# YiZhangCUG/liblcg

Hardware: AMD Instinct MI355X
Metric: cg_iterations_per_sec (higher is better)
Workload: dtype f64

## Files before the change

### include/lcg_hip.h

```cpp
#ifndef LCG_HIP_H
#define LCG_HIP_H

#include <stdint.h>

#ifdef __cplusplus
extern "C" {
#endif


typedef struct lcg_para {
    int    max_iterations;
    double epsilon;
    int    abs_diff;
    double restart_epsilon;
    double step;
    double sigma;
    double beta;
    int    maxi_m;
} lcg_para;

typedef struct clcg_para {
    int    max_iterations;
    double epsilon;
    int    abs_diff;
} clcg_para;

typedef enum lcg_solver_enum { LCG_CG = 0, LCG_PCG = 1, LCG_CGS = 2, LCG_BICGSTAB = 3, LCG_BICGSTAB2 = 4, LCG_PG = 5, LCG_SPG = 6 } lcg_solver_enum;
typedef enum clcg_solver_enum { CLCG_BICG = 0, CLCG_BICG_SYM = 1, CLCG_CGS = 2, CLCG_BICGSTAB = 3, CLCG_TFQMR = 4,
                                CLCG_PCG = 5, CLCG_PBICG = 6 } clcg_solver_enum;
enum {
    LCG_SUCCESS = 0, LCG_CONVERGENCE = 0, LCG_STOP = 1, LCG_ALREADY_OPTIMIZIED = 2,
    LCG_UNKNOWN_ERROR = -1024, LCG_INVILAD_VARIABLE_SIZE = -1023, LCG_INVILAD_MAX_ITERATIONS = -1022,
    LCG_INVILAD_EPSILON = -1021, LCG_INVILAD_RESTART_EPSILON = -1020,
    LCG_REACHED_MAX_ITERATIONS = -1019, LCG_NULL_PRECONDITION_MATRIX = -1018, LCG_NAN_VALUE = -1017,
    LCG_INVALID_POINTER = -1016, LCG_INVALID_LAMBDA = -1015, LCG_INVALID_SIGMA = -1014,
    LCG_INVALID_BETA = -1013, LCG_INVALID_MAXIM = -1012, LCG_SIZE_NOT_MATCH = -1011
};
enum {
    CLCG_SUCCESS = 0, CLCG_CONVERGENCE = 0, CLCG_STOP = 1, CLCG_ALREADY_OPTIMIZIED = 2,
    CLCG_UNKNOWN_ERROR = -1024, CLCG_INVILAD_VARIABLE_SIZE = -1023, CLCG_INVILAD_MAX_ITERATIONS = -1022,
    CLCG_INVILAD_EPSILON = -1021, CLCG_REACHED_MAX_ITERATIONS = -1020, CLCG_NAN_VALUE = -1019,
    CLCG_INVALID_POINTER = -1018, CLCG_SIZE_NOT_MATCH = -1017, CLCG_UNKNOWN_SOLVER = -1016
};
enum {
    LCG_HIP_E_RUNTIME = -2000,
    LCG_HIP_E_NO_DEVICE = -2001,
    LCG_HIP_E_COMM = -2002,
    LCG_HIP_E_ARG = -2003
};
enum { LCG_HIP_MEM_HOST = 0, LCG_HIP_MEM_DEVICE = 1 };

typedef void (*lcg_axfunc_ptr)(void *instance, const double *x, double *prod_Ax, const int n_size);
typedef int (*lcg_progress_ptr)(void *instance, const double *m, const double converge,
                                const lcg_para *param, const int n_size, const int k);
typedef void (*clcg_hip_axfunc_ptr)(void *instance, const double *x, double *prod_Ax,
                                    const int n_size, int layout, int conjugate);
typedef int (*clcg_hip_progress_ptr)(void *instance, const double *m, const double converge,
                                     const clcg_para *param, const int n_size, const int k);

typedef void (*clcg_hip_axfunc_c64_ptr)(void *instance, const float *x, float *prod_Ax, const int n_size,
                                        int layout, int conjugate);
typedef int (*clcg_hip_progress_c64_ptr)(void *instance, const float *m, const float converge,
                                         const clcg_para *param, const int n_size, const int k);

int  lcg_hip_init(int device);
int  lcg_hip_set_stream(void *hip_stream);
void *lcg_hip_get_stream(void);
int  lcg_hip_synchronize(void);
int  lcg_hip_memcpy(void *dst, const void *src, uint64_t bytes, int kind);
const char *lcg_hip_last_error(void);
lcg_para  lcg_hip_default_parameters(void);
clcg_para clcg_hip_default_parameters(void);
int    lcg_hip_last_iterations(void);
double lcg_hip_last_residual(void);
int    lcg_hip_set_profiling(int on);
double lcg_hip_last_ax_mean_us(void);
int    lcg_hip_last_ax_calls(void);
int    lcg_hip_last_launches(int *vector_passes, int *scalar_steps, int *rank_reductions, int *products);
int    lcg_hip_last_finisher_steps(void);
int    lcg_hip_trim(void);
enum { LCG_HIP_CG_AUTO = 0, LCG_HIP_CG_CLASSIC = 1, LCG_HIP_CG_ONE_REDUCTION = 2 };
int    lcg_hip_set_cg_schedule(int schedule);
int    lcg_hip_set_placement(int mode);
int    lcg_hip_last_placement(int *timed, int *moved, double *us_as_allocated, double *us_as_placed);
int    lcg_hip_pool_info(int *vectors, int64_t *bytes, int *arena_slots);
int    lcg_hip_pool_add_arena_for_test(uint64_t slot_bytes, int slots);
int    lcg_hip_placement_tune_for_test(uint64_t stream_min_bytes, uint64_t chunk_bytes, int max_chunks, double wall_ms, uint64_t hold_max_bytes,
                                       int force_find_at, int allow_shared);
int    lcg_hip_last_placement_walk(int *chunks, double *wall_ms, int64_t *held_bytes, int *found, const char **ended);

int lcg_hip_solver(lcg_axfunc_ptr Afp, lcg_progress_ptr Pfp, double *m, const double *B,
                   int n_size, const lcg_para *param, void *instance, int solver_id, int mem);
int lcg_hip_solver_preconditioned(lcg_axfunc_ptr Afp, lcg_axfunc_ptr Mfp, lcg_progress_ptr Pfp,
                                  double *m, const double *B, int n_size, const lcg_para *param,
                                  void *instance, int solver_id, int mem);
int lcg_hip_solver_constrained(lcg_axfunc_ptr Afp, lcg_progress_ptr Pfp, double *m, const double *B,
                               const double *low, const double *hig, int n_size, const lcg_para *param,
                               void *instance, int solver_id, int mem);
int lcg_hip_lcg(lcg_axfunc_ptr Afp, lcg_progress_ptr Pfp, double *m, const double *B, int n_size,
                const lcg_para *param, void *instance, double *Gk, double *Dk, double *ADk, int mem);
int lcg_hip_lcgs(lcg_axfunc_ptr Afp, lcg_progress_ptr Pfp, double *m, const double *B, int n_size,
                 const lcg_para *param, void *instance, double *RK, double *R0T, double *PK,
                 double *AX, double *UK, double *QK, double *WK, int mem);
int clcg_hip_solver(clcg_hip_axfunc_ptr Afp, clcg_hip_progress_ptr Pfp, double *m, const double *B,
                    int n_size, const clcg_para *param, void *instance, int solver_id, int mem);
int clcg_hip_solver_preconditioned(clcg_hip_axfunc_ptr Afp, clcg_hip_axfunc_ptr Mfp, clcg_hip_progress_ptr Pfp,
                                   double *m, const double *B, int n_size, const clcg_para *param,
                                   void *instance, int solver_id, int mem);
int clcg_hip_solver_c64(clcg_hip_axfunc_c64_ptr Afp, clcg_hip_progress_c64_ptr Pfp, float *m, const float *B,
                        int n_size, const clcg_para *param, void *instance, int solver_id, int mem);
int clcg_hip_solver_preconditioned_c64(clcg_hip_axfunc_c64_ptr Afp, clcg_hip_axfunc_c64_ptr Mfp, clcg_hip_progress_c64_ptr Pfp,
                                       float *m, const float *B, int n_size, const clcg_para *param, void *instance,
                                       int solver_id, int mem);
int lcg_hip_set_shadow_seed(unsigned seed);
int lcg_hip_set_shadow_vector(const double *rbar0_host, int n_size);

typedef struct lcg_hip_csr *lcg_hip_csr_t;

int lcg_hip_csr_create(lcg_hip_csr_t *A, int n_rows, int n_cols, int64_t nnz, const int *rowptr,
                       const int *col, const double *val, int is_complex, int mem, int adopt);
int lcg_hip_csr_create_c64(lcg_hip_csr_t *A, int n_rows, int n_cols, int64_t nnz, const int *rowptr,
                           const int *col, const float *val, int mem, int adopt);
int lcg_hip_csr_from_coo(lcg_hip_csr_t *A, int n, int64_t nnz, const int *row, const int *col,
                         const double *val, int is_complex, int mem);
int lcg_hip_csr_destroy(lcg_hip_csr_t A);
int lcg_hip_csr_rows(lcg_hip_csr_t A);
int64_t lcg_hip_csr_nnz(lcg_hip_csr_t A);
int lcg_hip_csr_arrays(lcg_hip_csr_t A, const int **rowptr, const int **col, const double **val);
int lcg_hip_csr_set_kernel(lcg_hip_csr_t A, int variant);
int lcg_hip_csr_set_packed(lcg_hip_csr_t A, int mode);
int64_t lcg_hip_csr_packed_runs(lcg_hip_csr_t A, int64_t *blocks_out);
int lcg_hip_csr_set_run_stretches(lcg_hip_csr_t A, int mode);
int64_t lcg_hip_csr_run_stretches(lcg_hip_csr_t A, int64_t *blocks_out);
int64_t lcg_hip_csr_packed_templates(lcg_hip_csr_t A);
int lcg_hip_csr_set_binned(lcg_hip_csr_t A, int mode);
int lcg_hip_csr_set_tiled(lcg_hip_csr_t A, int mode);
const char *lcg_hip_csr_tiled_status(lcg_hip_csr_t A);
int lcg_hip_csr_set_ranges(lcg_hip_csr_t A, int mode);
int lcg_hip_csr_ranges(lcg_hip_csr_t A, int cap, int *first_row);
const char *lcg_hip_csr_binned_status(lcg_hip_csr_t A);
const char *lcg_hip_csr_last_kernel(lcg_hip_csr_t A);
int64_t lcg_hip_csr_last_traffic_model(lcg_hip_csr_t A);
int lcg_hip_csr_plan_info(lcg_hip_csr_t A, double *build_ms, int64_t *extra_bytes);
int lcg_hip_csr_build_jacobi(lcg_hip_csr_t A, double *diag_out);

void lcg_hip_csr_ax(void *instance, const double *x, double *prod_Ax, const int n_size);
void lcg_hip_jacobi_mx(void *instance, const double *x, double *prod_Mx, const int n_size);
void clcg_hip_csr_ax(void *instance, const double *x, double *prod_Ax, const int n_size,
                     int layout, int conjugate);
void clcg_hip_jacobi_mx(void *instance, const double *x, double *prod_Mx, const int n_size,
                        int layout, int conjugate);
void clcg_hip_csr_ax_c64(void *instance, const float *x, float *prod_Ax, const int n_size,
                         int layout, int conjugate);
void clcg_hip_jacobi_mx_c64(void *instance, const float *x, float *prod_Mx, const int n_size,
                            int layout, int conjugate);

int  lcg_hip_csr_build_ic0(lcg_hip_csr_t A);
int  lcg_hip_csr_build_ic0_c64(lcg_hip_csr_t A);
int  lcg_hip_csr_ic0_info(lcg_hip_csr_t A, int *levels_lower, int *levels_upper, int *launches_per_apply,
                          int *zero_pivot, double *build_ms, int64_t *bytes);
int  lcg_hip_csr_ic0_set_sweeps(lcg_hip_csr_t A, int sweeps);
int  lcg_hip_csr_ic0_get_sweeps(lcg_hip_csr_t A, int *sweeps);
int  lcg_hip_csr_ic0_factor(lcg_hip_csr_t A, const int **rowptr, const int **col, const double **val);
int  lcg_hip_ic0_solve(lcg_hip_csr_t A, int which, const double *x, double *y);
int  lcg_hip_ic0_solve_c64(lcg_hip_csr_t A, int which, const float *x, float *y);
void lcg_hip_ic0_mx(void *instance, const double *x, double *prod_Mx, const int n_size);
void clcg_hip_ic0_mx(void *instance, const double *x, double *prod_Mx, const int n_size,
                     int layout, int conjugate);
void clcg_hip_ic0_mx_c64(void *instance, const float *x, float *prod_Mx, const int n_size,
                         int layout, int conjugate);
int  lcg_hip_csr_ic0_schedule_for_test(lcg_hip_csr_t A, int max_merged_rows);

int  lcg_hip_csr_build_ilu0(lcg_hip_csr_t A);
int  lcg_hip_csr_ilu0_info(lcg_hip_csr_t A, int *levels_L, int *levels_U, int *launches_per_apply, int *zero_pivot,
                           double *build_ms, int64_t *bytes);
int  lcg_hip_csr_ilu0_set_sweeps(lcg_hip_csr_t A, int sweeps);
int  lcg_hip_csr_ilu0_get_sweeps(lcg_hip_csr_t A, int *sweeps);
int  lcg_hip_csr_ilu0_factor(lcg_hip_csr_t A, int which, const int **rowptr, const int **col, const double **val);
int  lcg_hip_ilu0_solve(lcg_hip_csr_t A, int which, const double *x, double *y);
void lcg_hip_ilu0_mx(void *instance, const double *x, double *prod_Mx, const int n_size);
void clcg_hip_ilu0_mx(void *instance, const double *x, double *prod_Mx, const int n_size,
                      int layout, int conjugate);
void lcg_hip_csr_ax_ilu0(void *instance, const double *x, double *prod_Ax, const int n_size);
void clcg_hip_csr_ax_ilu0(void *instance, const double *x, double *prod_Ax, const int n_size,
                          int layout, int conjugate);
int  lcg_hip_csr_ilu0_schedule_for_test(lcg_hip_csr_t A, int max_merged_rows);

typedef struct lcg_hip_dense *lcg_hip_dense_t;

int lcg_hip_dense_create(lcg_hip_dense_t *K, int m_rows, int n_cols, const double *val, int64_t ld, int is_complex, int mem);
int lcg_hip_dense_create_rows(lcg_hip_dense_t *K, int m_rows, int n_cols, const double *const *rows, int is_complex);
int lcg_hip_dense_destroy(lcg_hip_dense_t K);
int lcg_hip_dense_rows(lcg_hip_dense_t K);
int lcg_hip_dense_cols(lcg_hip_dense_t K);
int lcg_hip_dense_matvec(lcg_hip_dense_t K, const double *x, double *y, int layout);
int clcg_hip_dense_matvec(lcg_hip_dense_t K, const double *x, double *y, int layout, int conjugate);
int lcg_hip_dense_ata(lcg_hip_dense_t K, const double *x, double *y);
void lcg_hip_dense_ata_ax(void *instance, const double *x, double *prod_Ax, const int n_size);
void lcg_hip_dense_ax(void *instance, const double *x, double *prod_Ax, const int n_size);
void clcg_hip_dense_ax(void *instance, const double *x, double *prod_Ax, const int n_size,
                       int layout, int conjugate);
int lcg_hip_dense_build_jacobi(lcg_hip_dense_t K, int normal, double *diag_out);
void lcg_hip_dense_jacobi_mx(void *instance, const double *x, double *prod_Mx, const int n_size);
void clcg_hip_dense_jacobi_mx(void *instance, const double *x, double *prod_Mx, const int n_size,
                              int layout, int conjugate);
const char *lcg_hip_dense_last_kernel(lcg_hip_dense_t K);
const char *lcg_hip_dense_kernel_name(int index);
int lcg_hip_dense_set_kernel(lcg_hip_dense_t K, int variant);
int lcg_hip_dense_matmat(lcg_hip_dense_t K, int k, const double *X, double *Y, int layout);
int lcg_hip_dense_ata_multi(lcg_hip_dense_t K, int k, const double *X, double *Y);
int lcg_hip_dense_op_multi_dot(lcg_hip_dense_t K, int k, int normal, const double *X, double *Y, const double *U, double *dots);
const char *lcg_hip_dense_multi_last_kernel(lcg_hip_dense_t K);
const char *lcg_hip_dense_multi_kernel_name(int index);
int lcg_hip_dense_lcg_multi (lcg_hip_dense_t K, int k, int normal, double *M, const double *B, const lcg_para *param,
                             int *ret, int *iterations, double *residual, int mem);
int lcg_hip_dense_lpcg_multi(lcg_hip_dense_t K, int k, int normal, double *M, const double *B, const lcg_para *param,
                             int *ret, int *iterations, double *residual, int mem);
int clcg_hip_dense_matmat(lcg_hip_dense_t K, int k, const double *X, double *Y, int layout, int conjugate);
int clcg_hip_dense_op_multi_dot(lcg_hip_dense_t K, int k, const double *X, double *Y, const double *U, double *dots);
const char *clcg_hip_dense_multi_kernel_name(int index);
int clcg_hip_dense_lbicg_sym_multi(lcg_hip_dense_t K, int k, double *M, const double *B, const clcg_para *param,
                                   int *ret, int *iterations, double *residual, int mem);
int clcg_hip_dense_lpcg_multi(lcg_hip_dense_t K, int k, double *M, const double *B, const clcg_para *param,
                              int *ret, int *iterations, double *residual, int mem);

int lcg_hip_spmv(lcg_hip_csr_t A, const double *x, double *y);
int lcg_hip_spmv_op(lcg_hip_csr_t A, const double *x, double *y, int layout, int conjugate);
int lcg_hip_spmv_dot(lcg_hip_csr_t A, const double *x, double *y, const double *u, double *result2);
int lcg_hip_spmm(lcg_hip_csr_t A, int k, const double *X, double *Y);
int lcg_hip_spmm_dot(lcg_hip_csr_t A, int k, const double *X, double *Y, const double *U, double *dots);
int lcg_hip_spmm_dot2(lcg_hip_csr_t A, int k, const double *X, double *Y, const double *U, double *dots2);
int lcg_hip_lcg_multi(lcg_hip_csr_t A, int k, double *M, const double *B, const lcg_para *param,
                      int *ret, int *iterations, double *residual, int mem);
int lcg_hip_lpcg_multi(lcg_hip_csr_t A, int k, double *M, const double *B, const lcg_para *param,
                       int *ret, int *iterations, double *residual, int mem);
int lcg_hip_ic0_solve_multi (lcg_hip_csr_t A, int k, int which, const double *X, double *Y);
int lcg_hip_ilu0_solve_multi(lcg_hip_csr_t A, int k, int which, const double *X, double *Y);
enum { LCG_HIP_M_JACOBI = 0, LCG_HIP_M_IC0 = 1, LCG_HIP_M_ILU0 = 2 };
int lcg_hip_lpcg_multi_m(lcg_hip_csr_t A, int k, int precond, double *M, const double *B, const lcg_para *param,
                         int *ret, int *iterations, double *residual, int mem);
enum { LCG_HIP_M_NONE = -1 };
int lcg_hip_lbicgstab_multi(lcg_hip_csr_t A, int k, int precond, double *M, const double *B, const lcg_para *param,
                            int *ret, int *iterations, double *residual, int mem);
int clcg_hip_spmm(lcg_hip_csr_t A, int k, const double *X, double *Y);
int clcg_hip_spmm_dot(lcg_hip_csr_t A, int k, const double *X, double *Y, const double *U, double *dots);
int clcg_hip_lbicg_sym_multi(lcg_hip_csr_t A, int k, double *M, const double *B, const clcg_para *param,
                             int *ret, int *iterations, double *residual, int mem);
int clcg_hip_lpcg_multi(lcg_hip_csr_t A, int k, double *M, const double *B, const clcg_para *param,
                        int *ret, int *iterations, double *residual, int mem);
int lcg_hip_spmv_c64(lcg_hip_csr_t A, const float *x, float *y, int layout, int conjugate);
int lcg_hip_dot(int n, const double *a, const double *b, double *result);
int lcg_hip_nrm2(int n, const double *a, double *result);
int lcg_hip_axpy(int n, double alpha, const double *x, double *y);
int lcg_hip_scal(int n, double alpha, double *x);
int lcg_hip_set2box(int n, const double *low, const double *hig, double *a);
int lcg_hip_vecmul(int n, const double *a, const double *b, double *c);
int lcg_hip_vecdiv(int n, const double *a, const double *b, double *c);
int clcg_hip_dot(int n, const double *a, const double *b, double *result2);
int clcg_hip_inner(int n, const double *a, const double *b, double *result2);
int clcg_hip_axpy(int n, const double *alpha2, const double *x, double *y);
int clcg_hip_vecdiv(int n, const double *a, const double *b, double *c);

int lcg_hip_csr_generate(lcg_hip_csr_t *A, int64_t n, int npairs, int64_t band, int symmetric,
                         uint64_t seed, double diag_shift, int64_t r0, int64_t r1);
enum { LCG_HIP_GEN_SCRAMBLED = 0, LCG_HIP_GEN_DIAGONALS = 1, LCG_HIP_GEN_ROW_RANDOM_BAND = 2 };
int lcg_hip_csr_generate_ex(lcg_hip_csr_t *A, int64_t n, int npairs, int pattern, int64_t band, int symmetric,
                            uint64_t seed, double diag_shift, int64_t r0, int64_t r1);
int lcg_hip_gen_xtrue(int64_t n, uint64_t seed, int64_t r0, int64_t r1, double *x_dev);
int lcg_hip_csr_laplace2d(lcg_hip_csr_t *A, int nx, int ny, int64_t r0, int64_t r1);

int lcg_hip_comm_unique_id(void *id128);
int lcg_hip_comm_init(int nranks, int rank, const void *id128);
int lcg_hip_comm_destroy(void);
int lcg_hip_comm_rank(void);
int lcg_hip_comm_size(void);
const char *lcg_hip_comm_library(void);
int lcg_hip_csr_distribute(lcg_hip_csr_t A, int64_t n_global, int mode);
int64_t lcg_hip_csr_exchange_volume(lcg_hip_csr_t A);
int lcg_hip_allreduce_sum(double *dev_values, int count);
int lcg_hip_barrier(void);
#define LCG_HIP_P2P_HANDLE_BYTES 64
int lcg_hip_p2p_export(void *handle64);
int lcg_hip_p2p_connect(int nranks, int rank, const void *handles);
int lcg_hip_p2p_selftest(int rounds);
int lcg_hip_p2p_enable(int on);
int lcg_hip_p2p_status(void);
// ... 14 lines not shown
```

### liblcg_amd/_lib.py

```python
from __future__ import annotations

import ctypes as C
import os
import subprocess

HERE = os.path.dirname(os.path.abspath(__file__))
SO_PATH = os.path.join(HERE, "lib", "liblcg_hip.so")
CSRC = os.path.join(HERE, "csrc")

c_int_p = C.POINTER(C.c_int)
c_double_p = C.POINTER(C.c_double)
vp = C.c_void_p


class LcgPara(C.Structure):
    _fields_ = [("max_iterations", C.c_int), ("epsilon", C.c_double), ("abs_diff", C.c_int),
                ("restart_epsilon", C.c_double), ("step", C.c_double), ("sigma", C.c_double),
                ("beta", C.c_double), ("maxi_m", C.c_int)]


class ClcgPara(C.Structure):
    _fields_ = [("max_iterations", C.c_int), ("epsilon", C.c_double), ("abs_diff", C.c_int)]


AXFUNC = C.CFUNCTYPE(None, vp, vp, vp, C.c_int)
PROGRESS = C.CFUNCTYPE(C.c_int, vp, vp, C.c_double, C.POINTER(LcgPara), C.c_int, C.c_int)
CAXFUNC = C.CFUNCTYPE(None, vp, vp, vp, C.c_int, C.c_int, C.c_int)
CPROGRESS = C.CFUNCTYPE(C.c_int, vp, vp, C.c_double, C.POINTER(ClcgPara), C.c_int, C.c_int)
CPROGRESS_C64 = C.CFUNCTYPE(C.c_int, vp, vp, C.c_float, C.POINTER(ClcgPara), C.c_int, C.c_int)

SIGNATURES = {
    "lcg_hip_init": (C.c_int, [C.c_int]),
    "lcg_hip_set_stream": (C.c_int, [vp]),
    "lcg_hip_get_stream": (vp, []),
    "lcg_hip_synchronize": (C.c_int, []),
    "lcg_hip_memcpy": (C.c_int, [vp, vp, C.c_uint64, C.c_int]),
    "lcg_hip_last_error": (C.c_char_p, []),
    "lcg_hip_default_parameters": (LcgPara, []),
    "clcg_hip_default_parameters": (ClcgPara, []),
    "lcg_hip_last_iterations": (C.c_int, []),
    "lcg_hip_last_residual": (C.c_double, []),
    "lcg_hip_set_profiling": (C.c_int, [C.c_int]),
    "lcg_hip_set_cg_schedule": (C.c_int, [C.c_int]),
    "lcg_hip_set_placement": (C.c_int, [C.c_int]),
    "lcg_hip_last_placement": (C.c_int, [C.POINTER(C.c_int), C.POINTER(C.c_int), C.POINTER(C.c_double), C.POINTER(C.c_double)]),
    "lcg_hip_pool_info": (C.c_int, [C.POINTER(C.c_int), C.POINTER(C.c_int64), C.POINTER(C.c_int)]),
    "lcg_hip_pool_add_arena_for_test": (C.c_int, [C.c_uint64, C.c_int]),
    "lcg_hip_placement_tune_for_test": (C.c_int, [C.c_uint64, C.c_uint64, C.c_int, C.c_double, C.c_uint64, C.c_int, C.c_int]),
    "lcg_hip_last_placement_walk": (C.c_int, [C.POINTER(C.c_int), C.POINTER(C.c_double), C.POINTER(C.c_int64), C.POINTER(C.c_int), C.POINTER(C.c_char_p)]),
    "lcg_hip_last_ax_mean_us": (C.c_double, []),
    "lcg_hip_last_ax_calls": (C.c_int, []),
    "lcg_hip_last_launches": (C.c_int, [c_int_p, c_int_p, c_int_p, c_int_p]),
    "lcg_hip_last_finisher_steps": (C.c_int, []),
    "lcg_hip_trim": (C.c_int, []),
    "lcg_hip_solver": (C.c_int, [vp, vp, vp, vp, C.c_int, C.POINTER(LcgPara), vp, C.c_int, C.c_int]),
    "lcg_hip_solver_preconditioned": (C.c_int, [vp, vp, vp, vp, vp, C.c_int, C.POINTER(LcgPara), vp, C.c_int, C.c_int]),
    "lcg_hip_solver_constrained": (C.c_int, [vp, vp, vp, vp, vp, vp, C.c_int, C.POINTER(LcgPara), vp, C.c_int, C.c_int]),
    "lcg_hip_set2box": (C.c_int, [C.c_int, vp, vp, vp]),
    "lcg_hip_lcg": (C.c_int, [vp, vp, vp, vp, C.c_int, C.POINTER(LcgPara), vp, vp, vp, vp, C.c_int]),
    "lcg_hip_lcgs": (C.c_int, [vp, vp, vp, vp, C.c_int, C.POINTER(LcgPara), vp, vp, vp, vp, vp, vp, vp, vp, C.c_int]),
    "clcg_hip_solver": (C.c_int, [vp, vp, vp, vp, C.c_int, C.POINTER(ClcgPara), vp, C.c_int, C.c_int]),
    "clcg_hip_solver_preconditioned": (C.c_int, [vp, vp, vp, vp, vp, C.c_int, C.POINTER(ClcgPara), vp, C.c_int, C.c_int]),
    "clcg_hip_jacobi_mx": (None, [vp, vp, vp, C.c_int, C.c_int, C.c_int]),
    "clcg_hip_solver_c64": (C.c_int, [vp, vp, vp, vp, C.c_int, C.POINTER(ClcgPara), vp, C.c_int, C.c_int]),
    "clcg_hip_solver_preconditioned_c64": (C.c_int, [vp, vp, vp, vp, vp, C.c_int, C.POINTER(ClcgPara), vp, C.c_int, C.c_int]),
    "lcg_hip_csr_create_c64": (C.c_int, [C.POINTER(vp), C.c_int, C.c_int, C.c_int64, vp, vp, vp, C.c_int, C.c_int]),
    "lcg_hip_spmv_c64": (C.c_int, [vp, vp, vp, C.c_int, C.c_int]),
    "clcg_hip_csr_ax_c64": (None, [vp, vp, vp, C.c_int, C.c_int, C.c_int]),
    "clcg_hip_jacobi_mx_c64": (None, [vp, vp, vp, C.c_int, C.c_int, C.c_int]),
    "lcg_hip_set_shadow_seed": (C.c_int, [C.c_uint]),
    "lcg_hip_set_shadow_vector": (C.c_int, [vp, C.c_int]),
    "lcg_hip_csr_create": (C.c_int, [C.POINTER(vp), C.c_int, C.c_int, C.c_int64, vp, vp, vp, C.c_int, C.c_int, C.c_int]),
    "lcg_hip_csr_from_coo": (C.c_int, [C.POINTER(vp), C.c_int, C.c_int64, vp, vp, vp, C.c_int, C.c_int]),
    "lcg_hip_csr_destroy": (C.c_int, [vp]),
    "lcg_hip_csr_rows": (C.c_int, [vp]),
    "lcg_hip_csr_nnz": (C.c_int64, [vp]),
    "lcg_hip_csr_arrays": (C.c_int, [vp, C.POINTER(vp), C.POINTER(vp), C.POINTER(vp)]),
    "lcg_hip_csr_set_kernel": (C.c_int, [vp, C.c_int]),
    "lcg_hip_csr_set_packed": (C.c_int, [vp, C.c_int]),
    "lcg_hip_csr_packed_runs": (C.c_int64, [vp, C.POINTER(C.c_int64)]),
    "lcg_hip_csr_set_run_stretches": (C.c_int, [vp, C.c_int]),
    "lcg_hip_csr_run_stretches": (C.c_int64, [vp, C.POINTER(C.c_int64)]),
    "lcg_hip_csr_packed_templates": (C.c_int64, [vp]),
    "lcg_hip_csr_set_binned": (C.c_int, [vp, C.c_int]),
    "lcg_hip_csr_set_tiled": (C.c_int, [vp, C.c_int]),
    "lcg_hip_csr_set_ranges": (C.c_int, [vp, C.c_int]),
    "lcg_hip_csr_ranges": (C.c_int, [vp, C.c_int, C.POINTER(C.c_int)]),
    "lcg_hip_csr_tiled_status": (C.c_char_p, [vp]),
    "lcg_hip_csr_binned_status": (C.c_char_p, [vp]),
    "lcg_hip_csr_last_kernel": (C.c_char_p, [vp]),
    "lcg_hip_csr_last_traffic_model": (C.c_int64, [vp]),
    "lcg_hip_csr_plan_info": (C.c_int, [vp, C.POINTER(C.c_double), C.POINTER(C.c_int64)]),
    "lcg_hip_csr_build_jacobi": (C.c_int, [vp, vp]),
    "lcg_hip_csr_build_ic0": (C.c_int, [vp]),
    "lcg_hip_csr_ic0_info": (C.c_int, [vp, c_int_p, c_int_p, c_int_p, c_int_p, c_double_p, C.POINTER(C.c_int64)]),
    "lcg_hip_csr_ic0_factor": (C.c_int, [vp, C.POINTER(vp), C.POINTER(vp), C.POINTER(vp)]),
    "lcg_hip_ic0_solve": (C.c_int, [vp, C.c_int, vp, vp]),
    "lcg_hip_ic0_mx": (None, [vp, vp, vp, C.c_int]),
    "clcg_hip_ic0_mx": (None, [vp, vp, vp, C.c_int, C.c_int, C.c_int]),
    "lcg_hip_csr_ic0_schedule_for_test": (C.c_int, [vp, C.c_int]),
    "lcg_hip_csr_ic0_set_sweeps": (C.c_int, [vp, C.c_int]),
    "lcg_hip_csr_ic0_get_sweeps": (C.c_int, [vp, c_int_p]),
    "lcg_hip_csr_build_ic0_c64": (C.c_int, [vp]),
    "lcg_hip_ic0_solve_c64": (C.c_int, [vp, C.c_int, vp, vp]),
    "clcg_hip_ic0_mx_c64": (None, [vp, vp, vp, C.c_int, C.c_int, C.c_int]),
    "lcg_hip_csr_build_ilu0": (C.c_int, [vp]),
    "lcg_hip_csr_ilu0_info": (C.c_int, [vp, c_int_p, c_int_p, c_int_p, c_int_p, c_double_p, C.POINTER(C.c_int64)]),
    "lcg_hip_csr_ilu0_set_sweeps": (C.c_int, [vp, C.c_int]),
    "lcg_hip_csr_ilu0_get_sweeps": (C.c_int, [vp, c_int_p]),
    "lcg_hip_csr_ilu0_factor": (C.c_int, [vp, C.c_int, C.POINTER(vp), C.POINTER(vp), C.POINTER(vp)]),
    "lcg_hip_ilu0_solve": (C.c_int, [vp, C.c_int, vp, vp]),
    "lcg_hip_ilu0_mx": (None, [vp, vp, vp, C.c_int]),
    "clcg_hip_ilu0_mx": (None, [vp, vp, vp, C.c_int, C.c_int, C.c_int]),
    "lcg_hip_csr_ax_ilu0": (None, [vp, vp, vp, C.c_int]),
    "clcg_hip_csr_ax_ilu0": (None, [vp, vp, vp, C.c_int, C.c_int, C.c_int]),
    "lcg_hip_csr_ilu0_schedule_for_test": (C.c_int, [vp, C.c_int]),
    "lcg_hip_dense_create": (C.c_int, [C.POINTER(vp), C.c_int, C.c_int, vp, C.c_int64, C.c_int, C.c_int]),
    "lcg_hip_dense_create_rows": (C.c_int, [C.POINTER(vp), C.c_int, C.c_int, vp, C.c_int]),
    "lcg_hip_dense_destroy": (C.c_int, [vp]),
    "lcg_hip_dense_rows": (C.c_int, [vp]),
    "lcg_hip_dense_cols": (C.c_int, [vp]),
    "lcg_hip_dense_matvec": (C.c_int, [vp, vp, vp, C.c_int]),
    "clcg_hip_dense_matvec": (C.c_int, [vp, vp, vp, C.c_int, C.c_int]),
    "lcg_hip_dense_ata": (C.c_int, [vp, vp, vp]),
    "lcg_hip_dense_ata_ax": (None, [vp, vp, vp, C.c_int]),
    "lcg_hip_dense_ax": (None, [vp, vp, vp, C.c_int]),
    "clcg_hip_dense_ax": (None, [vp, vp, vp, C.c_int, C.c_int, C.c_int]),
    "lcg_hip_dense_build_jacobi": (C.c_int, [vp, C.c_int, vp]),
    "lcg_hip_dense_jacobi_mx": (None, [vp, vp, vp, C.c_int]),
    "clcg_hip_dense_jacobi_mx": (None, [vp, vp, vp, C.c_int, C.c_int, C.c_int]),
    "lcg_hip_dense_last_kernel": (C.c_char_p, [vp]),
    "lcg_hip_dense_kernel_name": (C.c_char_p, [C.c_int]),
    "lcg_hip_dense_set_kernel": (C.c_int, [vp, C.c_int]),
    "lcg_hip_dense_matmat": (C.c_int, [vp, C.c_int, vp, vp, C.c_int]),
    "lcg_hip_dense_ata_multi": (C.c_int, [vp, C.c_int, vp, vp]),
    "lcg_hip_dense_op_multi_dot": (C.c_int, [vp, C.c_int, C.c_int, vp, vp, vp, c_double_p]),
    "lcg_hip_dense_multi_last_kernel": (C.c_char_p, [vp]),
    "lcg_hip_dense_multi_kernel_name": (C.c_char_p, [C.c_int]),
    "lcg_hip_dense_lcg_multi": (C.c_int, [vp, C.c_int, C.c_int, vp, vp, C.POINTER(LcgPara), c_int_p, c_int_p, c_double_p, C.c_int]),
    "lcg_hip_dense_lpcg_multi": (C.c_int, [vp, C.c_int, C.c_int, vp, vp, C.POINTER(LcgPara), c_int_p, c_int_p, c_double_p, C.c_int]),
    "clcg_hip_dense_matmat": (C.c_int, [vp, C.c_int, vp, vp, C.c_int, C.c_int]),
    "clcg_hip_dense_op_multi_dot": (C.c_int, [vp, C.c_int, vp, vp, vp, c_double_p]),
    "clcg_hip_dense_multi_kernel_name": (C.c_char_p, [C.c_int]),
    "clcg_hip_dense_lbicg_sym_multi": (C.c_int, [vp, C.c_int, vp, vp, C.POINTER(ClcgPara), c_int_p, c_int_p, c_double_p, C.c_int]),
    "clcg_hip_dense_lpcg_multi": (C.c_int, [vp, C.c_int, vp, vp, C.POINTER(ClcgPara), c_int_p, c_int_p, c_double_p, C.c_int]),
    "lcg_hip_csr_ax": (None, [vp, vp, vp, C.c_int]),
    "lcg_hip_jacobi_mx": (None, [vp, vp, vp, C.c_int]),
    "clcg_hip_csr_ax": (None, [vp, vp, vp, C.c_int, C.c_int, C.c_int]),
    "lcg_hip_spmv": (C.c_int, [vp, vp, vp]),
    "lcg_hip_spmv_op": (C.c_int, [vp, vp, vp, C.c_int, C.c_int]),
    "lcg_hip_spmv_dot": (C.c_int, [vp, vp, vp, vp, c_double_p]),
    "lcg_hip_spmm": (C.c_int, [vp, C.c_int, vp, vp]),
    "lcg_hip_spmm_dot": (C.c_int, [vp, C.c_int, vp, vp, vp, c_double_p]),
    "lcg_hip_spmm_dot2": (C.c_int, [vp, C.c_int, vp, vp, vp, c_double_p]),
    "lcg_hip_lcg_multi": (C.c_int, [vp, C.c_int, vp, vp, C.POINTER(LcgPara), c_int_p, c_int_p, c_double_p, C.c_int]),
    "lcg_hip_lpcg_multi": (C.c_int, [vp, C.c_int, vp, vp, C.POINTER(LcgPara), c_int_p, c_int_p, c_double_p, C.c_int]),
    "lcg_hip_lpcg_multi_m": (C.c_int, [vp, C.c_int, C.c_int, vp, vp, C.POINTER(LcgPara), c_int_p, c_int_p, c_double_p, C.c_int]),
    "lcg_hip_lbicgstab_multi": (C.c_int, [vp, C.c_int, C.c_int, vp, vp, C.POINTER(LcgPara), c_int_p, c_int_p, c_double_p, C.c_int]),
    "clcg_hip_spmm": (C.c_int, [vp, C.c_int, vp, vp]),
    "clcg_hip_spmm_dot": (C.c_int, [vp, C.c_int, vp, vp, vp, c_double_p]),
    "clcg_hip_lbicg_sym_multi": (C.c_int, [vp, C.c_int, vp, vp, C.POINTER(ClcgPara), c_int_p, c_int_p, c_double_p, C.c_int]),
    "clcg_hip_lpcg_multi": (C.c_int, [vp, C.c_int, vp, vp, C.POINTER(ClcgPara), c_int_p, c_int_p, c_double_p, C.c_int]),
    "lcg_hip_ic0_solve_multi": (C.c_int, [vp, C.c_int, C.c_int, vp, vp]),
    "lcg_hip_ilu0_solve_multi": (C.c_int, [vp, C.c_int, C.c_int, vp, vp]),
    "lcg_hip_dot": (C.c_int, [C.c_int, vp, vp, c_double_p]),
    "lcg_hip_nrm2": (C.c_int, [C.c_int, vp, c_double_p]),
    "lcg_hip_axpy": (C.c_int, [C.c_int, C.c_double, vp, vp]),
    "lcg_hip_scal": (C.c_int, [C.c_int, C.c_double, vp]),
    "lcg_hip_vecmul": (C.c_int, [C.c_int, vp, vp, vp]),
    "lcg_hip_vecdiv": (C.c_int, [C.c_int, vp, vp, vp]),
    "clcg_hip_dot": (C.c_int, [C.c_int, vp, vp, c_double_p]),
    "clcg_hip_inner": (C.c_int, [C.c_int, vp, vp, c_double_p]),
    "clcg_hip_axpy": (C.c_int, [C.c_int, c_double_p, vp, vp]),
    "clcg_hip_vecdiv": (C.c_int, [C.c_int, vp, vp, vp]),
    "lcg_hip_csr_generate": (C.c_int, [C.POINTER(vp), C.c_int64, C.c_int, C.c_int64, C.c_int, C.c_uint64, C.c_double, C.c_int64, C.c_int64]),
    "lcg_hip_csr_generate_ex": (C.c_int, [C.POINTER(vp), C.c_int64, C.c_int, C.c_int, C.c_int64, C.c_int, C.c_uint64, C.c_double, C.c_int64, C.c_int64]),
    "lcg_hip_gen_xtrue": (C.c_int, [C.c_int64, C.c_uint64, C.c_int64, C.c_int64, vp]),
    "lcg_hip_csr_laplace2d": (C.c_int, [C.POINTER(vp), C.c_int, C.c_int, C.c_int64, C.c_int64]),
    "lcg_hip_comm_unique_id": (C.c_int, [vp]),
    "lcg_hip_comm_init": (C.c_int, [C.c_int, C.c_int, vp]),
    "lcg_hip_comm_destroy": (C.c_int, []),
    "lcg_hip_comm_rank": (C.c_int, []),
    "lcg_hip_comm_size": (C.c_int, []),
    "lcg_hip_comm_library": (C.c_char_p, []),
    "lcg_hip_csr_distribute": (C.c_int, [vp, C.c_int64, C.c_int]),
    "lcg_hip_allreduce_sum": (C.c_int, [vp, C.c_int]),
    "lcg_hip_barrier": (C.c_int, []),
    "lcg_hip_csr_direct_selfloop_for_test": (C.c_int, [vp, C.c_int, C.c_int]),
    "lcg_hip_p2p_export": (C.c_int, [vp]),
    "lcg_hip_p2p_connect": (C.c_int, [C.c_int, C.c_int, vp]),
    "lcg_hip_p2p_selftest": (C.c_int, [C.c_int]),
    "lcg_hip_p2p_enable": (C.c_int, [C.c_int]),
    "lcg_hip_p2p_status": (C.c_int, []),
    "lcg_hip_p2p_set_timeout_ms": (C.c_int, [C.c_int]),
    "lcg_hip_p2p_disconnect": (C.c_int, []),
    "lcg_hip_csr_split_for_test": (C.c_int, [vp, C.c_int64, C.c_int, C.c_int]),
    "lcg_hip_csr_xfull": (vp, [vp]),
    "lcg_hip_csr_ax_part_for_probe": (C.c_int, [vp, vp, vp, C.c_int]),
    "lcg_hip_csr_local_nnz": (C.c_int64, [vp]),
    "lcg_hip_csr_exchange_volume": (C.c_int64, [vp]),
    "lcg_hip_csr_need_ranges_for_test": (C.c_int, [vp, C.c_int, vp]),
}

_lib = None


def build(verbose: bool = False) -> str:
    cmd = ["make", "-C", CSRC, "-j", str(min(8, os.cpu_count() or 1))]
    if not verbose:
        cmd.insert(1, "-s")
    subprocess.check_call(cmd)
    return SO_PATH


def load():
    global _lib
    if _lib is not None:
        return _lib
    if not os.path.exists(SO_PATH):
        try:
            build()
        except Exception as exc:
            raise ImportError(f"{SO_PATH} is not built and could not be built here ({exc}): run "
                              "`python -c 'import __graft_entry__ as g; g.build()'` (there is no CPU fallback)")
    import torch
    lib = C.CDLL(SO_PATH, mode=C.RTLD_GLOBAL)
    for name, (res, args) in SIGNATURES.items():
        fn = getattr(lib, name)
        fn.restype = res
        fn.argtypes = args
    _lib = lib
    return lib


def fnptr(lib, name: str) -> vp:
# ... 2 lines not shown
```

### liblcg_amd/api.py

```python
from __future__ import annotations

import ctypes as C
from dataclasses import dataclass

import numpy as np

from . import _lib as L
from ._lib import CAXFUNC, CPROGRESS, CPROGRESS_C64, AXFUNC, PROGRESS, ClcgPara, LcgPara

LCG_CG, LCG_PCG, LCG_CGS, LCG_BICGSTAB, LCG_BICGSTAB2, LCG_PG, LCG_SPG = range(7)
CLCG_BICG, CLCG_BICG_SYM, CLCG_CGS, CLCG_BICGSTAB, CLCG_TFQMR, CLCG_PCG, CLCG_PBICG = range(7)
MEM_HOST, MEM_DEVICE = 0, 1
GEN_SCRAMBLED, GEN_DIAGONALS, GEN_ROW_RANDOM_BAND = 0, 1, 2


class LcgHipError(RuntimeError):
    pass


def _chk(rc: int, what: str):
    if rc <= -2000:
        raise LcgHipError(f"{what}: rc={rc}: {L.load().lcg_hip_last_error().decode()}")
    return rc


def lcg_default_parameters(**kw) -> LcgPara:
    p = L.load().lcg_hip_default_parameters()
    for k, v in kw.items():
        setattr(p, k, v)
    return p


def clcg_default_parameters(**kw) -> ClcgPara:
    p = L.load().clcg_hip_default_parameters()
    for k, v in kw.items():
        setattr(p, k, v)
    return p


def _ptr(x):
    if isinstance(x, np.ndarray):
        return x.ctypes.data, MEM_HOST
    import torch
    if isinstance(x, torch.Tensor):
        if not x.is_contiguous():
            raise ValueError("tensor must be contiguous")
        return x.data_ptr(), (MEM_DEVICE if x.is_cuda else MEM_HOST)
    raise TypeError(type(x))


def use_torch_stream():
    import torch
    _chk(L.load().lcg_hip_set_stream(C.c_void_p(torch.cuda.current_stream().cuda_stream)), "set_stream")


def use_own_stream():
    _chk(L.load().lcg_hip_set_stream(None), "set_stream")


class CsrMatrix:
    is_c64 = False

    def __init__(self, handle: int, n_rows: int, is_complex: bool, keep=()):
        self.h = C.c_void_p(handle)
        self.n = n_rows
        self.is_complex = is_complex
        self._keep = keep

    @classmethod
    def from_csr(cls, rowptr, col, val, n_cols=None, adopt=False):
        lib = L.load()
        is_c = bool(np.iscomplexobj(val)) if isinstance(val, np.ndarray) else val.is_complex()
        if isinstance(val, np.ndarray):
            rowptr = np.ascontiguousarray(rowptr, np.int32); col = np.ascontiguousarray(col, np.int32)
            val = np.ascontiguousarray(val, np.complex128 if is_c else np.float64)
        n = len(rowptr) - 1
        nnz = len(col)
        (pr, mem), (pc, _), (pv, _) = _ptr(rowptr), _ptr(col), _ptr(val)
        h = C.c_void_p()
        _chk(lib.lcg_hip_csr_create(C.byref(h), n, n_cols or n, nnz, pr, pc, pv, int(is_c), mem, int(adopt)), "csr_create")
        return cls(h.value, n, is_c, keep=(rowptr, col, val) if adopt else ())

    @classmethod
    def from_csr_c64(cls, rowptr, col, val, n_cols=None, adopt=False):
        lib = L.load()
        if isinstance(val, np.ndarray):
            rowptr = np.ascontiguousarray(rowptr, np.int32); col = np.ascontiguousarray(col, np.int32)
            val = np.ascontiguousarray(val, np.complex64)
        else:
            import torch
            if val.dtype != torch.complex64:
                raise TypeError(f"from_csr_c64 takes complex64 values, not {val.dtype}")
        n = len(rowptr) - 1
        (pr, mem), (pc, _), (pv, _) = _ptr(rowptr), _ptr(col), _ptr(val)
        h = C.c_void_p()
        _chk(lib.lcg_hip_csr_create_c64(C.byref(h), n, n_cols or n, len(col), pr, pc, pv, mem, int(adopt)), "csr_create_c64")
        M = cls(h.value, n, True, keep=(rowptr, col, val) if adopt else ())
        M.is_c64 = True
        return M

    def spmv_c64(self, x, y, layout=0, conjugate=0):
        return _chk(L.load().lcg_hip_spmv_c64(self.h, _ptr(x)[0], _ptr(y)[0], layout, conjugate), "spmv_c64")

    @classmethod
    def from_coo(cls, n, row, col, val):
        lib = L.load()
        is_c = bool(np.iscomplexobj(val))
        row = np.ascontiguousarray(row, np.int32); col = np.ascontiguousarray(col, np.int32)
        val = np.ascontiguousarray(val, np.complex128 if is_c else np.float64)
        h = C.c_void_p()
        _chk(lib.lcg_hip_csr_from_coo(C.byref(h), n, len(row), row.ctypes.data, col.ctypes.data, val.ctypes.data,
                                      int(is_c), MEM_HOST), "csr_from_coo")
        return cls(h.value, n, is_c)

    @classmethod
    def generate(cls, n, npairs=16, band=0, symmetric=True, seed=1, diag_shift=0.01, r0=0, r1=None, pattern=None):
        lib = L.load()
        r1 = n if r1 is None else r1
        if pattern is None:
            pattern = GEN_DIAGONALS if band > 0 else GEN_SCRAMBLED
        h = C.c_void_p()
        _chk(lib.lcg_hip_csr_generate_ex(C.byref(h), n, npairs, pattern, band, int(symmetric), seed, diag_shift, r0, r1), "csr_generate")
        return cls(h.value, r1 - r0, False)

    @classmethod
    def laplace2d(cls, nx, ny, r0=0, r1=None):
        lib = L.load()
        r1 = nx * ny if r1 is None else r1
        h = C.c_void_p()
        _chk(lib.lcg_hip_csr_laplace2d(C.byref(h), nx, ny, r0, r1), "csr_laplace2d")
        return cls(h.value, r1 - r0, False)

    @property
    def nnz(self) -> int:
        return L.load().lcg_hip_csr_nnz(self.h)

    def arrays_to_host(self):
        lib = L.load()
        pr, pc, pv = C.c_void_p(), C.c_void_p(), C.c_void_p()
        _chk(lib.lcg_hip_csr_arrays(self.h, C.byref(pr), C.byref(pc), C.byref(pv)), "csr_arrays")
        nnz = self.nnz
        rowptr = np.empty(self.n + 1, np.int32); col = np.empty(nnz, np.int32)
        val = np.empty(nnz, np.complex128 if self.is_complex else np.float64)
        for dst, src in ((rowptr, pr), (col, pc), (val, pv)):
            _chk(lib.lcg_hip_memcpy(dst.ctypes.data, src, dst.nbytes, 2), "memcpy d2h")
        return rowptr, col, val

    def set_kernel(self, variant: int):
        _chk(L.load().lcg_hip_csr_set_kernel(self.h, variant), "set_kernel")

    def build_jacobi(self, diag_out=None):
        p = None if diag_out is None else _ptr(diag_out)[0]
        _chk(L.load().lcg_hip_csr_build_jacobi(self.h, p), "build_jacobi")

    def build_ic0(self):
        if self.is_c64:
            _chk(L.load().lcg_hip_csr_build_ic0_c64(self.h), "build_ic0_c64")
        else:
            _chk(L.load().lcg_hip_csr_build_ic0(self.h), "build_ic0")

    def ic0_info(self) -> dict:
        ll, lu, la, zp = C.c_int(), C.c_int(), C.c_int(), C.c_int()
        ms, nb = C.c_double(), C.c_int64()
        _chk(L.load().lcg_hip_csr_ic0_info(self.h, C.byref(ll), C.byref(lu), C.byref(la), C.byref(zp), C.byref(ms), C.byref(nb)),
             "ic0_info")
        sw = C.c_int(0)
        if L.load().lcg_hip_csr_ic0_get_sweeps(self.h, C.byref(sw)) != 0:
            sw.value = 0
        return {"levels_lower": ll.value, "levels_upper": lu.value, "launches_per_apply": la.value,
                "zero_pivot": zp.value, "build_ms": ms.value, "bytes": nb.value, "sweeps": sw.value}

    def ic0_set_sweeps(self, k):
        _chk(L.load().lcg_hip_csr_ic0_set_sweeps(self.h, int(k)), "ic0_set_sweeps")

    def ic0_factor_to_host(self):
        lib = L.load()
        pr, pc, pv = C.c_void_p(), C.c_void_p(), C.c_void_p()
        _chk(lib.lcg_hip_csr_ic0_factor(self.h, C.byref(pr), C.byref(pc), C.byref(pv)), "ic0_factor")
        rowptr = np.empty(self.n + 1, np.int32)
        _chk(lib.lcg_hip_memcpy(rowptr.ctypes.data, pr, rowptr.nbytes, 2), "memcpy d2h")
        nnz = int(rowptr[-1])
        col = np.empty(nnz, np.int32)
        val = np.empty(nnz, np.complex64 if self.is_c64 else np.complex128 if self.is_complex else np.float64)
        for dst, src in ((col, pc), (val, pv)):
            _chk(lib.lcg_hip_memcpy(dst.ctypes.data, src, dst.nbytes, 2), "memcpy d2h")
        return rowptr, col, val

    def ic0_solve(self, x, y, which=2):
        if self.is_c64:
            _chk(L.load().lcg_hip_ic0_solve_c64(self.h, which, _ptr(x)[0], _ptr(y)[0]), "ic0_solve_c64")
        else:
            _chk(L.load().lcg_hip_ic0_solve(self.h, which, _ptr(x)[0], _ptr(y)[0]), "ic0_solve")

    def ic0_solve_multi(self, X, Y, which=2):
        k = _block_k(X, Y)
        _chk(L.load().lcg_hip_ic0_solve_multi(self.h, k, which, _ptr(X)[0], _ptr(Y)[0]), "ic0_solve_multi")

    def build_ilu0(self):
        _chk(L.load().lcg_hip_csr_build_ilu0(self.h), "build_ilu0")

    def ilu0_info(self) -> dict:
        ll, lu, la, zp = C.c_int(), C.c_int(), C.c_int(), C.c_int()
        ms, nb = C.c_double(), C.c_int64()
        _chk(L.load().lcg_hip_csr_ilu0_info(self.h, C.byref(ll), C.byref(lu), C.byref(la), C.byref(zp), C.byref(ms), C.byref(nb)),
             "ilu0_info")
        sw = C.c_int(0)
        if L.load().lcg_hip_csr_ilu0_get_sweeps(self.h, C.byref(sw)) != 0:
            sw.value = 0
        return {"levels_L": ll.value, "levels_U": lu.value, "launches_per_apply": la.value,
                "zero_pivot": zp.value, "build_ms": ms.value, "bytes": nb.value, "sweeps": sw.value}

    def ilu0_set_sweeps(self, k):
        _chk(L.load().lcg_hip_csr_ilu0_set_sweeps(self.h, int(k)), "ilu0_set_sweeps")

    def ilu0_factor_to_host(self, which):
        lib = L.load()
        pr, pc, pv = C.c_void_p(), C.c_void_p(), C.c_void_p()
        _chk(lib.lcg_hip_csr_ilu0_factor(self.h, int(which), C.byref(pr), C.byref(pc), C.byref(pv)), "ilu0_factor")
        rowptr = np.empty(self.n + 1, np.int32)
        _chk(lib.lcg_hip_memcpy(rowptr.ctypes.data, pr, rowptr.nbytes, 2), "memcpy d2h")
        nnz = int(rowptr[-1])
        col = np.empty(nnz, np.int32)
        val = np.empty(nnz, np.complex128 if self.is_complex else np.float64)
        for dst, src in ((col, pc), (val, pv)):
            if nnz:
                _chk(lib.lcg_hip_memcpy(dst.ctypes.data, src, dst.nbytes, 2), "memcpy d2h")
        return rowptr, col, val

    def ilu0_solve(self, x, y, which=2):
        _chk(L.load().lcg_hip_ilu0_solve(self.h, which, _ptr(x)[0], _ptr(y)[0]), "ilu0_solve")

    def ilu0_solve_multi(self, X, Y, which=2):
        k = _block_k(X, Y)
        _chk(L.load().lcg_hip_ilu0_solve_multi(self.h, k, which, _ptr(X)[0], _ptr(Y)[0]), "ilu0_solve_multi")

    def spmv(self, x, y):
        _chk(L.load().lcg_hip_spmv(self.h, _ptr(x)[0], _ptr(y)[0]), "spmv")

    def spmm(self, X, Y):
        k = _block_k(X, Y)
        _chk(L.load().lcg_hip_spmm(self.h, k, _ptr(X)[0], _ptr(Y)[0]), "spmm")

    def spmm_dot2(self, X, Y, U):
        k = _block_k(X, Y, U)
        out = (C.c_double * (2 * k))()
        _chk(L.load().lcg_hip_spmm_dot2(self.h, k, _ptr(X)[0], _ptr(Y)[0], _ptr(U)[0], out), "spmm_dot2")
        return np.array(out[:], dtype=np.float64)

    def cspmm(self, X, Y):
        k = _block_k(X, Y, cplx=True)
        _chk(L.load().clcg_hip_spmm(self.h, k, _ptr(X)[0], _ptr(Y)[0]), "cspmm")

    def cspmm_dot(self, X, Y, U):
        k = _block_k(X, Y, U, cplx=True)
        out = (C.c_double * (2 * k))()
        _chk(L.load().clcg_hip_spmm_dot(self.h, k, _ptr(X)[0], _ptr(Y)[0], _ptr(U)[0], out), "cspmm_dot")
        return np.array(out[:], dtype=np.float64).view(np.complex128)

    def distribute(self, n_global: int, mode: int = 0):
        _chk(L.load().lcg_hip_csr_distribute(self.h, n_global, mode), "csr_distribute")

    def destroy(self):
        if self.h:
            L.load().lcg_hip_csr_destroy(self.h)
            self.h = C.c_void_p()

    def __del__(self):
        try:
            self.destroy()
        except Exception:
            pass


class DenseMatrix:
    KERNEL_AUTO, KERNEL_ROW, KERNEL_ROW_SPLIT, KERNEL_COL, KERNEL_ATA_TWO_PASS, KERNEL_ATA_ONE_PASS, KERNEL_ATA_SMALL = range(7)

    def __init__(self, handle: int, m: int, n: int, is_complex: bool):
        self.h = C.c_void_p(handle)
        self.m, self.n, self.is_complex = m, n, is_complex

    @classmethod
    def from_array(cls, K):
        lib = L.load()
        if isinstance(K, np.ndarray):
            is_c = bool(np.iscomplexobj(K))
            if (K.ndim != 2 or K.strides[1] != K.itemsize or K.dtype not in (np.float64, np.complex128) or K.strides[0] % K.itemsize
                    or (K.shape[0] > 1 and K.strides[0] < K.shape[1] * K.itemsize)):
                K = np.ascontiguousarray(K, np.complex128 if is_c else np.float64)
            ld, ptr, mem = K.strides[0] // K.itemsize, K.ctypes.data, MEM_HOST
        else:
            is_c = K.is_complex()
            if K.dim() != 2 or K.stride(1) != 1:
                raise ValueError("a 2-d tensor with unit stride along its rows is needed")
            ld, ptr, mem = K.stride(0), K.data_ptr(), (MEM_DEVICE if K.is_cuda else MEM_HOST)
        m, n = K.shape
        if ld < n:
            if m != 1:
                raise ValueError(f"rows {ld} entries apart hold {n} entries: make the array contiguous first")
            ld = n
        h = C.c_void_p()
        _chk(lib.lcg_hip_dense_create(C.byref(h), m, n, ptr, ld, int(is_c), mem), "dense_create")
        return cls(h.value, m, n, is_c)
# ... 346 lines not shown
```

### liblcg_amd/csrc/comm.hip

```cpp
#include <dlfcn.h>

#include <rccl/rccl.h>

#include <cstdlib>
#include <cstring>
#include <vector>

#include "devcommon.hpp"

namespace lcgh {


struct Comm {
    void *lib = nullptr;
    ncclComm_t comm = nullptr;
    int nranks = 1, rank = 0;
    ncclResult_t (*GetUniqueId)(ncclUniqueId *) = nullptr;
    ncclResult_t (*CommInitRank)(ncclComm_t *, int, ncclUniqueId, int) = nullptr;
    ncclResult_t (*CommDestroy)(ncclComm_t) = nullptr;
    ncclResult_t (*AllReduce)(const void *, void *, size_t, ncclDataType_t, ncclRedOp_t, ncclComm_t, hipStream_t) = nullptr;
    ncclResult_t (*AllGather)(const void *, void *, size_t, ncclDataType_t, ncclComm_t, hipStream_t) = nullptr;
    ncclResult_t (*ReduceScatter)(const void *, void *, size_t, ncclDataType_t, ncclRedOp_t, ncclComm_t, hipStream_t) = nullptr;
    ncclResult_t (*Send)(const void *, size_t, ncclDataType_t, int, ncclComm_t, hipStream_t) = nullptr;
    ncclResult_t (*Recv)(void *, size_t, ncclDataType_t, int, ncclComm_t, hipStream_t) = nullptr;
// ... 483 lines not shown
        cp.dst[cp.nseg] = A->xfull + w * (size_t)D->need_lo[s];
        cp.first_block[cp.nseg] = nb;
        nb += (int)((cnt + PUSH_CHUNK - 1) / PUSH_CHUNK);
        cp.nseg++;
    }
    cp.first_block[cp.nseg] = nb;
    cp.nblocks = nb > 0 ? nb : 1;
}

static int direct_setup(lcg_hip_csr *A)
{
    Ctx &c = ctx();
    XgBox xb;
    if (!xg_box(&xb)) { c.err = "direct exchange needs the mailboxes (lcg_hip_p2p_connect + enable)"; return LCG_HIP_E_COMM; }
    const int P = xb.P, me = xb.me;
    const size_t w = A->is_complex ? 2 : 1;
    Direct *D = new Direct();
    A->direct = D;
    auto give_up = [&](int rc, const char *why) { if (why) c.err = why; direct_free(A); return rc; };

    std::vector<long long> need;
    int rc = need_ranges(A, P, need);
    bool all = false;
    int rc2 = xg_agree(rc == 0, &all);
    if (rc2) return give_up(rc2, nullptr);
    if (!all) return give_up(rc ? rc : LCG_HIP_E_COMM, rc ? nullptr : "direct exchange: a peer could not scan its columns");
    std::vector<unsigned long long> table;
    rc = xg_allgather_words(reinterpret_cast<const unsigned long long *>(need.data()), 2 * P, table);
    if (rc) return give_up(rc, nullptr);
    auto T = [&](int q, int p, int k) { return (long long)table[(size_t)q * 2 * P + 2 * p + k]; };
    for (int q = 0; q < P; q++) {
        if (q == me) continue;
        const bool take = need[2 * q + 1] > need[2 * q];
        const bool give = T(q, me, 1) > T(q, me, 0);
        if (!take && !give) continue;
        if (D->nnb < XG_MAXSEG) {
            const int s = D->nnb;
            D->nb_rank[s] = q;
            D->give_lo[s] = give ? T(q, me, 0) : 0; D->give_hi[s] = give ? T(q, me, 1) : 0;
            D->need_lo[s] = take ? need[2 * q] : 0; D->need_hi[s] = take ? need[2 * q + 1] : 0;
            if (take) D->recv_total += need[2 * q + 1] - need[2 * q];
        }
        D->nnb++;
    }
    const bool fits = D->nnb <= XG_MAXSEG;
    rc = xg_agree(fits, &all);
    if (rc) return give_up(rc, nullptr);
    if (!all) return give_up(LCG_HIP_E_COMM, "direct exchange: a rank has more than 8 neighbours (use mode 1 or 0)");
    D->half = (size_t)A->rows_per_rank * P * w;
    hipError_t e;
    {
        void *p = nullptr;
        e = hipExtMallocWithFlags(&p, sizeof(double) * 2 * D->half, hipDeviceMallocUncached);
        if (e != hipSuccess) { (void)hipGetLastError(); e = hipExtMallocWithFlags(&p, sizeof(double) * 2 * D->half, hipDeviceMallocFinegrained); }
        D->recv = static_cast<double *>(p);
    }
    if (e == hipSuccess) e = hipMemsetAsync(D->recv, 0, sizeof(double) * 2 * D->half, c.stream);
    if (e == hipSuccess) {
        void *p = nullptr;
        e = hipExtMallocWithFlags(&p, sizeof(unsigned long long) * XG_MAXP, hipDeviceMallocUncached);
        if (e != hipSuccess) { (void)hipGetLastError(); e = hipExtMallocWithFlags(&p, sizeof(unsigned long long) * XG_MAXP, hipDeviceMallocFinegrained); }
        D->flags = static_cast<unsigned long long *>(p);
    }
    if (e == hipSuccess) e = hipMemsetAsync(D->flags, 0, sizeof(unsigned long long) * XG_MAXP, c.stream);
    if (e == hipSuccess) e = hipMalloc(&D->ticket, sizeof(unsigned int));
    if (e == hipSuccess) e = hipMemsetAsync(D->ticket, 0, sizeof(unsigned int), c.stream);
    if (e == hipSuccess) e = hipStreamSynchronize(c.stream);
    unsigned long long hw[16] = {0};
    static_assert(sizeof(hipIpcMemHandle_t) == 64, "IPC handle size");
    if (e == hipSuccess) { hipIpcMemHandle_t h; e = hipIpcGetMemHandle(&h, D->recv); std::memcpy(hw, &h, 64); }
    if (e == hipSuccess) { hipIpcMemHandle_t h; e = hipIpcGetMemHandle(&h, D->flags); std::memcpy(hw + 8, &h, 64); }
    if (e != hipSuccess) (void)fail(e, "direct exchange buffers", __FILE__, __LINE__);
    rc = xg_agree(e == hipSuccess, &all);
    if (rc) return give_up(rc, nullptr);
    if (!all) return give_up(LCG_HIP_E_COMM, e == hipSuccess ? "direct exchange: a peer could not allocate or export its buffers" : nullptr);
    std::vector<unsigned long long> handles;
    rc = xg_allgather_words(hw, 16, handles);
    if (rc) return give_up(rc, nullptr);
    e = hipSuccess;
    for (int s = 0; s < D->nnb && e == hipSuccess; s++) {
        const int q = D->nb_rank[s];
        hipIpcMemHandle_t h; void *p = nullptr;
        std::memcpy(&h, &handles[(size_t)q * 16], 64);
        e = hipIpcOpenMemHandle(&p, h, hipIpcMemLazyEnablePeerAccess);
        if (e != hipSuccess) break;
        D->opened.push_back(p); D->nb_recv[s] = static_cast<double *>(p);
        std::memcpy(&h, &handles[(size_t)q * 16 + 8], 64);
        e = hipIpcOpenMemHandle(&p, h, hipIpcMemLazyEnablePeerAccess);
        if (e != hipSuccess) break;
        D->opened.push_back(p); D->nb_flags[s] = static_cast<unsigned long long *>(p);
    }
    if (e != hipSuccess) (void)fail(e, "hipIpcOpenMemHandle (neighbour buffers)", __FILE__, __LINE__);
    rc = xg_agree(e == hipSuccess, &all);
    if (rc) return give_up(rc, nullptr);
    if (!all) return give_up(LCG_HIP_E_COMM, e == hipSuccess ? "direct exchange: a peer could not map a neighbour" : nullptr);
    PushPlan &pp = D->push;
    pp.ticket = D->ticket;
    int nb = 0;
    for (int s = 0; s < D->nnb; s++) {
        pp.flag[pp.nflag++] = D->nb_flags[s] + me;
        D->wait.flag[D->wait.n++] = D->flags + D->nb_rank[s];
        const long long cnt = (D->give_hi[s] - D->give_lo[s]) * (long long)w;
        if (cnt <= 0) continue;
        pp.count[pp.nseg] = (long)cnt;
        pp.first_block[pp.nseg] = nb;
        nb += (int)((cnt + PUSH_CHUNK - 1) / PUSH_CHUNK);
        pp.nseg++;
    }
    pp.first_block[pp.nseg] = nb;
    pp.nblocks = nb > 0 ? nb : (pp.nflag > 0 ? 1 : 0);
    D->wait.timeout_ticks = xb.timeout_ticks;
    D->wait.fail = xb.fail;
    D->generation = g_xg_generation;
    direct_copy_plan(A, D);
    return 0;
}

static void direct_plans(lcg_hip_csr *A, const double *x, PushPlan *pp, WaitPlan *wp, PushPlan *cp)
{
    Direct *D = static_cast<Direct *>(A->direct);
    const size_t w = A->is_complex ? 2 : 1;
    const unsigned long long k = ++D->calls;
    const size_t par = (size_t)(k & 1);
    *pp = D->push; *wp = D->wait; *cp = D->copy;
    pp->seq = k; wp->seq = k;
    int seg = 0, cseg = 0;
    for (int s = 0; s < D->nnb; s++) {
        if (D->give_hi[s] > D->give_lo[s]) {
            pp->src[seg] = x + w * (size_t)(D->give_lo[s] - A->row0);
            pp->dst[seg] = D->nb_recv[s] + par * D->half + w * (size_t)D->give_lo[s];
            seg++;
        }
        if (D->need_hi[s] > D->need_lo[s]) cp->src[cseg++] = D->recv + par * D->half + w * (size_t)D->need_lo[s];
    }
}

void dist_free(lcg_hip_csr *A)
{
    direct_free(A);
    if (A->halo) { delete static_cast<HaloPlan *>(A->halo); A->halo = nullptr; }
    if (!A->distributed) return;
    free_part(A->loc); free_part(A->rem);
    if (A->remc.rowptr) hipFree(A->remc.rowptr);
    if (A->remc.pk_base) hipFree(A->remc.pk_base);
    if (A->remc.pk_ofs) hipFree(A->remc.pk_ofs);
    if (A->remc.pk_data) hipFree(A->remc.pk_data);
    if (A->remc.pk_rs_off) hipFree(A->remc.pk_rs_off);
    A->remc = CsrPart();
    if (A->rem_rows) hipFree(A->rem_rows);
    if (A->rem_y) hipFree(A->rem_y);
    A->rem_rows = nullptr; A->rem_y = nullptr;
    if (A->xfull) hipFree(A->xfull);
    A->xfull = nullptr; A->distributed = false;
    for (int i = 1; i < 4; i++) free_part(A->op[i]);
    if (A->op_z) hipFree(A->op_z);
    A->op_z = nullptr;
}

int dist_split(lcg_hip_csr *A, int64_t n_global, int nranks, int rank)
{
    Ctx &c = ctx();
    for (int i = 1; i < 4; i++) free_part(A->op[i]);
    const int n = A->n_rows;
    const int64_t rpr = (n_global + nranks - 1) / nranks;
    const int64_t row0 = (int64_t)rank * rpr;
    const int64_t expect = std::max<int64_t>(0, std::min<int64_t>(n_global, row0 + rpr) - row0);
    if (expect != n) { c.err = "shard row count does not match ceil(n_global/nranks) partition"; return LCG_HIP_E_ARG; }
    dist_free(A);
    A->n_global = n_global; A->row0 = row0; A->rows_per_rank = rpr;
    int *cl = nullptr, *cr = nullptr;
    HIPCHK(hipMalloc(&cl, sizeof(int) * (size_t)n));
    HIPCHK(hipMalloc(&cr, sizeof(int) * (size_t)n));
    const unsigned g = (unsigned)((n + VB - 1) / VB);
    hipLaunchKernelGGL(k_split_count, dim3(g), dim3(VB), 0, c.stream, n, (long)row0, (long)(row0 + n), A->main.rowptr, A->main.col, cl, cr);
    long nl = 0, nr = 0;
    HIPCHK(hipMalloc(&A->loc.rowptr, sizeof(int) * ((size_t)n + 1)));
    HIPCHK(hipMalloc(&A->rem.rowptr, sizeof(int) * ((size_t)n + 1)));
    int rc = device_exclusive_scan(n, cl, A->loc.rowptr, c.stream, &nl);
    if (!rc) rc = device_exclusive_scan(n, cr, A->rem.rowptr, c.stream, &nr);
    hipFree(cl); hipFree(cr);
    if (rc) return rc;
    rc = alloc_cols(A->loc, n, nl, A->is_complex); if (rc) return rc;
    rc = alloc_cols(A->rem, n, nr, A->is_complex); if (rc) return rc;
    A->loc.n_cols = n; A->rem.n_cols = rpr * nranks;
    if (A->is_complex)
        hipLaunchKernelGGL((k_split_fill<double2>), dim3(g), dim3(VB), 0, c.stream, n, (long)row0, (long)(row0 + n), A->main.rowptr,
                           A->main.col, reinterpret_cast<const double2 *>(A->main.val), A->loc.rowptr, A->loc.col,
                           reinterpret_cast<double2 *>(A->loc.val), A->rem.rowptr, A->rem.col, reinterpret_cast<double2 *>(A->rem.val));
    else
        hipLaunchKernelGGL((k_split_fill<double>), dim3(g), dim3(VB), 0, c.stream, n, (long)row0, (long)(row0 + n), A->main.rowptr,
                           A->main.col, A->main.val, A->loc.rowptr, A->loc.col, A->loc.val, A->rem.rowptr, A->rem.col, A->rem.val);
    HIPCHK(hipGetLastError());
    if (nr > 0) {
        int *flag = nullptr, *pos = nullptr;
        long kept = 0;
        HIPCHK(hipMalloc(&flag, sizeof(int) * (size_t)n));
        HIPCHK(hipMalloc(&pos, sizeof(int) * ((size_t)n + 1)));
        hipLaunchKernelGGL(k_row_flags, dim3(g), dim3(VB), 0, c.stream, n, A->rem.rowptr, flag);
        rc = device_exclusive_scan(n, flag, pos, c.stream, &kept);
        if (!rc) {
            hipError_t e = hipMalloc(&A->remc.rowptr, sizeof(int) * ((size_t)kept + 1));
            if (e == hipSuccess) e = hipMalloc(&A->rem_rows, sizeof(int) * (size_t)kept);
            if (e == hipSuccess) e = hipMalloc(&A->rem_y, sizeof(double) * (A->is_complex ? 2 : 1) * 2 * (size_t)kept);
            if (e != hipSuccess) rc = fail(e, "remote-row compaction", __FILE__, __LINE__);
        }
        if (!rc) {
            hipLaunchKernelGGL(k_row_compact, dim3(g), dim3(VB), 0, c.stream, n, A->rem.rowptr, pos, A->rem_rows,
                               A->remc.rowptr, (int)kept);
            A->remc.n_rows = (int)kept; A->remc.nnz = nr; A->remc.col = A->rem.col; A->remc.val = A->rem.val;
            A->remc.owned = false; A->remc.padded = true;
        }
        hipError_t e2 = hipStreamSynchronize(c.stream);
        hipFree(flag); hipFree(pos);
        if (rc) return rc;
        if (e2 != hipSuccess) return fail(e2, "remote-row compaction", __FILE__, __LINE__);
    }
    HIPCHK(hipMalloc(&A->xfull, sizeof(double) * (A->is_complex ? 2 : 1) * (size_t)(rpr * nranks)));
    HIPCHK(hipMemsetAsync(A->xfull, 0, sizeof(double) * (A->is_complex ? 2 : 1) * (size_t)(rpr * nranks), c.stream));
    HIPCHK(hipStreamSynchronize(c.stream));
    A->distributed = true;
    return 0;
}

int dist_spmv_op(lcg_hip_csr *A, const CsrPart &T, const double *x, double *y)
{
    Ctx &c = ctx();
    const size_t w = A->is_complex ? 2 : 1;
    const int *done = ax_flag(c);
    if (!g_comm.comm && world_size() > 1) {
        c.err = "op(A).x on a sharded matrix sums the ranks' contributions with RCCL: no communicator (lcg_hip_comm_init)";
        return LCG_HIP_E_COMM;
    }
    const size_t rpr = (size_t)A->rows_per_rank, nt = (size_t)T.n_rows;
    if (!A->op_z) HIPCHK(hipMalloc(&A->op_z, sizeof(double) * w * (nt + rpr)));
    double *z = A->op_z, *blk = A->op_z + w * nt;
    const double mean = T.n_rows ? (double)T.nnz / T.n_rows : 0.0;
    int rc = spmv_launch(T, A->is_complex, 0, mean, x, z, false, c.stream, done);
    if (rc) return rc;
    const bool whole = (size_t)A->n_rows == rpr;
    double *dst = whole ? y : blk;
    if (g_comm.comm) {
        ncclResult_t r = g_comm.ReduceScatter(z, dst, w * rpr, ncclDouble, ncclSum, g_comm.comm, c.stream);
        if (r != ncclSuccess) return comm_fail("ncclReduceScatter", r);
    } else {
        HIPCHK(hipMemcpyAsync(dst, z + w * (size_t)A->row0, sizeof(double) * w * (size_t)A->n_rows, hipMemcpyDeviceToDevice, c.stream));
    }
    if (!whole) HIPCHK(hipMemcpyAsync(y, blk, sizeof(double) * w * (size_t)A->n_rows, hipMemcpyDeviceToDevice, c.stream));
    return 0;
}

static int remote_sums_launch(lcg_hip_csr *A, const double *xfull, double *out, hipStream_t s, const int *done)
{
    const int nr = A->remc.n_rows;
    if (nr <= 0) return 0;
    const double mean_r = (double)A->remc.nnz / nr;
    const int T = mean_r <= 8.0 ? 1 : (mean_r <= 24.0 ? 2 : 4);
    const unsigned g = (unsigned)(((long)nr * T + VB - 1) / VB);
#define RS_LAUNCH(TT)                                                                                                \
    do {                                                                                                             \
        if (A->is_complex)                                                                                           \
            hipLaunchKernelGGL((k_remote<double2, TT, false>), dim3(g), dim3(VB), 0, s, nr, A->remc.rowptr, A->remc.col, \
                               reinterpret_cast<const double2 *>(A->remc.val), A->rem_rows,                          \
                               reinterpret_cast<const double2 *>(xfull), reinterpret_cast<double2 *>(out), done);    \
        else                                                                                                         \
            hipLaunchKernelGGL((k_remote<double, TT, false>), dim3(g), dim3(VB), 0, s, nr, A->remc.rowptr, A->remc.col, \
                               A->remc.val, A->rem_rows, xfull, out, done);                                          \
    } while (0)
    switch (T) { case 1: RS_LAUNCH(1); break; case 2: RS_LAUNCH(2); break; default: RS_LAUNCH(4); }
#undef RS_LAUNCH
    HIPCHK(hipGetLastError());
    return 0;
}

static int exchange_x(lcg_hip_csr *A, const double *x, hipStream_t s)
{
    const size_t w = A->is_complex ? 2 : 1;
    if (g_comm.comm && A->dist_mode == 1 && A->halo) return halo_exchange(A, x, s);
    double *mine = A->xfull + w * (size_t)(A->row0);
    HIPCHK(hipMemcpyAsync(mine, x, sizeof(double) * w * (size_t)A->n_rows, hipMemcpyDeviceToDevice, s));
    if (g_comm.comm) {
        ncclResult_t r = g_comm.AllGather(mine, A->xfull, w * (size_t)A->rows_per_rank, ncclDouble, g_comm.comm, s);
        if (r != ncclSuccess) return comm_fail("ncclAllGather", r);
    }
    return 0;
}

static int dist_spmv_impl(lcg_hip_csr *A, const double *x, double *y, const double *u, double *part, int *slots, bool *fused)
{
    Ctx &c = ctx();
    if (fused) *fused = false;
    bool dot = u != nullptr && !A->is_complex;
    int nslot = 0;
    const int *done = ax_flag(c);
    if (A->dist_mode < 0) {
        c.err = "this matrix's exchange could not be set up (lcg_hip_csr_distribute failed): distribute it again under another mode";
        return LCG_HIP_E_COMM;
    }
    if (A->dist_mode != 2 && !g_comm.comm && world_size() > 1) {
        c.err = "modes 0 and 1 move x with RCCL: no communicator (lcg_hip_comm_init)";
        return LCG_HIP_E_COMM;
    }
    if (A->dist_mode == 2 && !A->direct) {
        c.err = "direct exchange without a plan (lcg_hip_csr_distribute(A, n, 2) did not succeed)";
        return LCG_HIP_E_COMM;
    }
    if (A->dist_mode == 2 && A->direct) {
        if (static_cast<Direct *>(A->direct)->uses_mailbox &&
            (!g_xg.connected || static_cast<Direct *>(A->direct)->generation != g_xg_generation)) {
            c.err = "direct exchange: the mailboxes were disconnected (or connected anew) while this matrix still uses them (distribute it again)";
            return LCG_HIP_E_COMM;
        }
        PushPlan pp, cp; WaitPlan wp;
        direct_plans(A, x, &pp, &wp, &cp);
        const double mean_l = A->n_rows ? (double)A->loc.nnz / A->n_rows : 0.0;
        static const bool withhold = std::getenv("LCG_HIP_TEST_WITHHOLD_PUSH") != nullptr;
        constexpr int RECV_TAIL_MAX = 256;
        const bool recv_in_tail = !withhold && wp.n > 0 && cp.nblocks <= RECV_TAIL_MAX;
        if (recv_in_tail) {
            pp.nrecv = cp.nblocks; pp.rnseg = cp.nseg; pp.wp = wp; pp.rst = c.in_solve ? c.state : nullptr;
            for (int q = 0; q < cp.nseg; q++) { pp.rsrc[q] = cp.src[q]; pp.rdst[q] = cp.dst[q]; pp.rcount[q] = cp.count[q]; }
            for (int q = 0; q <= cp.nseg && q <= XG_MAXSEG; q++) pp.rfirst[q] = cp.first_block[q];
            if (pp.nrecv <= 0) pp.nrecv = 1;
        }
        const long rem_blocks = A->remc.n_rows > 0 ? ((long)A->remc.n_rows * 4 + VB - 1) / VB : 0;
        dot = dot && !withhold && 512 + rem_blocks <= AXP_CAP;
        int rc = 0, f = 0;
        int nbig = 0;
        if (dot) {
            f = csr_part_ax_dot(A->loc, A->variant, mean_l, x, y, u, 0, part, &nslot, c.stream, done, &pp, A->remc.n_rows > 0 ? &nbig : nullptr);
            if (f < 0) return f;
        }
        dot = f == 1;
        if (!dot)
            rc = withhold ? spmv_launch(A->loc, A->is_complex, A->variant, mean_l, x, y, false, c.stream, done)
                          : spmv_launch_push(A->loc, A->is_complex, A->variant, mean_l, x, y, c.stream, done, pp);
        if (rc) return rc;
        Direct *D = static_cast<Direct *>(A->direct);
        if (debug_on() && D->calls == 1)
            std::fprintf(stderr, "[lcg_hip] direct: recv %lld doubles in %d blocks (%s), n_global %lld, rows %d\n", D->recv_total, cp.nblocks,
                         recv_in_tail ? "tail of the product's grid" : "k_recv", (long long)A->n_global, A->n_rows);
        if (wp.n > 0 && !recv_in_tail) {
            hipLaunchKernelGGL(k_recv, dim3((unsigned)cp.nblocks), dim3(VB), 0, c.stream, wp, cp, c.in_solve ? c.state : nullptr);
            HIPCHK(hipGetLastError());
        }
        if (A->remc.n_rows > 0) {
            const int nr = A->remc.n_rows;
            const double mean_r = (double)A->remc.nnz / nr;
            const int T = mean_r <= 8.0 ? 1 : (mean_r <= 24.0 ? 2 : 4);
#define REMOTE_LAUNCH(TT)                                                                                            \
    do {                                                                                                             \
        const unsigned g = (unsigned)(((long)nr * TT + VB - 1) / VB);                                                \
        if (A->is_complex)                                                                                           \
            hipLaunchKernelGGL((k_remote<double2, TT, true>), dim3(g), dim3(VB), 0, c.stream, nr, A->remc.rowptr, A->remc.col, \
                               reinterpret_cast<const double2 *>(A->remc.val), A->rem_rows,                          \
                               reinterpret_cast<const double2 *>(A->xfull), reinterpret_cast<double2 *>(y), done);   \
        else                                                                                                         \
            hipLaunchKernelGGL((k_remote<double, TT, true>), dim3(g), dim3(VB), 0, c.stream, nr, A->remc.rowptr, A->remc.col, \
                               A->remc.val, A->rem_rows, A->xfull, y, done);                                         \
    } while (0)
#define REMOTE_DOT(TT)                                                                                               \
    do {                                                                                                             \
        const unsigned g = (unsigned)(((long)nr * TT + VB - 1) / VB);                                                \
        hipLaunchKernelGGL((k_remote<double, TT, true, true>), dim3(g), dim3(VB), 0, c.stream, nr, A->remc.rowptr, A->remc.col, \
                           A->remc.val, A->rem_rows, A->xfull, y, done, u, part + nslot,                             \
                           nbig ? A->loc.dot_part : nullptr, nbig, (int)((nbig + g - 1) / g));                       \
        nslot += (int)g;                                                                                             \
    } while (0)
#define REMOTE_CASE(TT) case TT: if (dot) REMOTE_DOT(TT); else REMOTE_LAUNCH(TT); break;
            switch (T) {
                REMOTE_CASE(1) REMOTE_CASE(2) REMOTE_CASE(4)
            }
#undef REMOTE_CASE
#undef REMOTE_DOT
// ... 445 lines not shown
```

### liblcg_amd/csrc/csr.hip

```cpp
#include <algorithm>
#include <type_traits>
#include <cstring>
#include <functional>
#include <numeric>

#include <chrono>

#include "csr_plan.hpp"

namespace lcgh {

template <class V, int T, bool ACC, bool PUSH = false>
__global__ __launch_bounds__(VB) void k_spmv_wave(int n, const int *__restrict__ rowptr,
                                                  const int *__restrict__ col, const V *__restrict__ val,
                                                  const V *__restrict__ x, V *__restrict__ y,
                                                  const int *done, PushPlan pp)
{
    if (PUSH && (int)blockIdx.x < pp.nblocks) { push_block(pp, blockIdx.x); return; }
    if (PUSH && pp.nrecv > 0 && (int)blockIdx.x >= (int)gridDim.x - pp.nrecv) { recv_block(pp, (int)blockIdx.x - ((int)gridDim.x - pp.nrecv)); return; }
    const int bid = PUSH ? blockIdx.x - pp.nblocks : blockIdx.x;
    if (done && *done) return;
    const int sub = threadIdx.x % T;
    const long row = ((long)bid * VB + threadIdx.x) / T;
    V acc = vzero(V());
// ... 321 lines not shown
        tplb = !bad;
    }
    if (threadIdx.x == 0) {
        if (e == s) { lo = 0; hi = 0; }
        base[b] = run ? -1 - L : (tplb ? -TPL_CODE - D : lo);
        ngroups[b] = run ? -L : (tplb ? -TPL_GRP - D : e - s);
        if (!tplb && !run) atomicMax(maxspan, hi - lo);
        atomicMax(maxspan + 1, L);
        if (run) atomicAdd(maxspan + 2, 1);
        if (tplb) atomicAdd(maxspan + 3, 1);
    }
}

__global__ void k_pk_groups(int nb, int per, int *ngroups)
{
    const int b = blockIdx.x * blockDim.x + threadIdx.x;
    if (b < nb) {
        const int g = ngroups[b];
        ngroups[b] = g <= -TPL_GRP ? (-g - TPL_GRP + 1 + 3) / 4 + (-g - TPL_GRP <= 32 ? PK_R / 4 : PK_R / 2)
                                   : (g < 0 ? (-g + 1 + 3) / 4 : (per > 0 ? (g + per - 1) / per : 0));
    }
}

template <int BITS> __device__ __forceinline__ int pk_field(u64 lo, u64 hi, int j);
template <> __device__ __forceinline__ int pk_field<21>(u64 lo, u64 hi, int j)
{
    return (int)(((j < 3 ? lo : hi) >> (21 * (j % 3))) & 0x1fffff);
}
template <> __device__ __forceinline__ int pk_field<18>(u64 lo, u64 hi, int j)
{
    const int sh = 18 * j;
    const u64 v = sh + 18 <= 64 ? lo >> sh : (sh >= 64 ? hi >> (sh - 64) : (lo >> sh) | (hi << (64 - sh)));
    return (int)(v & 0x3ffff);
}

__global__ __launch_bounds__(VB) void k_pk_dof(int n, const int *__restrict__ rowptr, const int *__restrict__ col, int *ok)
{
    const int i = blockIdx.x * VB + threadIdx.x;
    unsigned bad = 0;
    if (i < n) {
        const int s = rowptr[i], len = rowptr[i + 1] - s;
        bad = (len % 2 != 0 ? 1u : 0u) | (len % 3 != 0 ? 2u : 0u) | (len % 4 != 0 ? 4u : 0u);
        int prev = len > 0 ? col[s] : 0;
        for (int k = 1; k < len && bad != 7u; k++) {
            const int c = col[s + k];
            if (c != prev + 1) bad |= (k % 2 != 0 ? 1u : 0u) | (k % 3 != 0 ? 2u : 0u) | (k % 4 != 0 ? 4u : 0u);
            prev = c;
        }
    }
    for (int g = 0; g < 3; g++) if (__ballot((bad >> g) & 1u) != 0ull && (threadIdx.x & 63) == 0) ok[g] = 0;
}

template <int BITS>
__global__ __launch_bounds__(VB) void k_pk_pack(int n, const int *rowptr, const int *col, const int *base, const int *pofs, v4i *packed, int R, int dof)
{
    constexpr int PER = BITS > 0 ? 128 / BITS : 1;
    const int b = blockIdx.x;
    const long row0 = (long)b * R;
    const int r1 = (int)min((long)n, row0 + R);
    const int s = rowptr[row0], e = rowptr[r1];
    const int bs = base[b];
    if (BITS == 0 && bs >= 0) return;
    if (bs <= -TPL_CODE) {
        __shared__ int tpl[TPL_MAXD + 1], dcount;
        if (threadIdx.x < 64) {
            int D; bool bad;
            const unsigned long long m = tpl_row_mask(row0, r1, rowptr, col, tpl, &dcount, &D, &bad);
            int *dst = reinterpret_cast<int *>(packed + pofs[b]);
            const int Dp = (D + 1 + 3) & ~3;
            int idg = -1;
            for (int i = 0; i < D; i++) if (tpl[i] == (int)row0) idg = i;
            const bool lacks = idg < 0 || (row0 + (long)threadIdx.x < r1 && !((m >> idg) & 1ull));
            if (__ballot(lacks)) idg = -1;
            if ((int)threadIdx.x < D) dst[threadIdx.x] = tpl[threadIdx.x];
            if (threadIdx.x == 0) { dst[D] = idg; for (int i = D + 1; i < Dp; i++) dst[i] = 0; }
            if (D <= 32) reinterpret_cast<unsigned *>(dst + Dp)[threadIdx.x] = (unsigned)m;
            else reinterpret_cast<unsigned long long *>(dst + Dp)[threadIdx.x] = m;
        }
        return;
    }
    if (bs < 0) {
        const int L = -1 - bs;
        int *dst = reinterpret_cast<int *>(packed + pofs[b]);
        __shared__ int kd;
        if (threadIdx.x == 0) kd = -1;
        __syncthreads();
        for (int k = threadIdx.x; k < L; k += VB) if (col[s + k] == (int)row0) kd = k;
        __syncthreads();
        for (int k = threadIdx.x; k < ((L + 1 + 3) & ~3); k += VB) dst[k] = k < L ? col[s + k] : (k == L ? kd : 0);
        return;
    }
    const int ng = (e - s + PER * dof - 1) / (PER * dof);
    for (int g = threadIdx.x; g < ng; g += VB) {
        u64 lo = 0, hi = 0;
        for (int j = 0; j < PER; j++) {
            const int k = s + (PER * g + j) * dof;
            const u64 c = k < e ? (u64)(col[k] - bs) : 0;
            if (BITS == 21) { if (j < 3) lo |= c << (21 * j); else hi |= c << (21 * (j - 3)); }
            else if (BITS > 0) {
                const int sh = BITS * j;
                if (sh < 64) { lo |= c << sh; if (sh + BITS > 64) hi |= c >> (64 - sh); }
                else hi |= c << (sh - 64);
            }
        }
        v4i o; o.x = (int)(unsigned)lo; o.y = (int)(unsigned)(lo >> 32); o.z = (int)(unsigned)hi; o.w = (int)(unsigned)(hi >> 32);
        packed[pofs[b] + g] = o;
    }
}

__global__ __launch_bounds__(VB) void k_pk_stretch_flags(int n, int nb, const int *__restrict__ rowptr, const int *__restrict__ col,
                                                         const int *__restrict__ base, int *__restrict__ flag)
{
    const int b = blockIdx.x * VB + threadIdx.x;
    if (b >= nb) return;
    const int bs = base[b];
    int f = 0;
    if (bs < 0 && bs > -TPL_CODE && (long)b * PK_R + PK_R <= (long)n) {
        const int L = -1 - bs;
        f = L;
        if (b > 0 && base[b - 1] == bs) {
            const int s = rowptr[(long)b * PK_R], sp = rowptr[(long)(b - 1) * PK_R];
            bool same = (long)s == (long)sp + (long)PK_R * L;
            for (int k = 0; k < L && same; k++) same = col[s + k] - PK_R == col[sp + k];
            if (same) f = -L;
        }
    }
    flag[b] = f;
}

__global__ __launch_bounds__(64) void k_pk_stretch_fill(RunStretches rs, const int *__restrict__ rowptr, const int *__restrict__ col,
                                                        int *__restrict__ off, int *__restrict__ out)
{
    __shared__ int kd;
    int o = 0, L = 0, Q = 1, b0 = 0;
#pragma unroll
    for (int j = 0; j < RS_MAX; j++) {
        if (j < (int)blockIdx.x) o += 4 * rs.s[j].Q;
        if (j == (int)blockIdx.x) { L = rs.s[j].L; Q = rs.s[j].Q; b0 = rs.s[j].b0; }
    }
    const long row0 = (long)b0 * PK_R;
    const int s = rowptr[row0];
    if (threadIdx.x == 0) kd = -1;
    __syncthreads();
    for (int i = threadIdx.x; i < 4 * Q; i += 64) {
        const int k = i / Q + 4 * (i % Q);
        const int d = k < L ? col[s + k] - (int)row0 : 0;
        off[o + i] = d;
        if (k < L && d == 0) kd = k;
    }
    __syncthreads();
    if (threadIdx.x == 0) { out[2 * blockIdx.x] = s; out[2 * blockIdx.x + 1] = kd; }
}

__device__ __forceinline__ void ldsp_dot_tail(const DotPlan &dp, int bid, int j0, double vfin, double uv)
{
    if (threadIdx.x >= 64) return;
    if (j0 != 0) vfin = 0.0;
    const double a0 = wave_sum(vfin * uv);
    if ((threadIdx.x & 63) == WSUM_LANE) dp.part[bid] = a0;
    if (dp.yy) {
        const double a1 = wave_sum(vfin * vfin);
        if ((threadIdx.x & 63) == WSUM_LANE) dp.part[dp.stride + bid] = a1;
    }
}

constexpr int PK_CH_SMALL = 2208;
constexpr int PK_CH_7 = 1872, PK_CH_8 = 1696;
static int pk_window(int max_slice)
{
    static const int env = [] { const char *e = std::getenv("LCG_HIP_PACKED_WINDOW"); return e ? atoi(e) : 0; }();
    const int need = std::max(max_slice, env);
    return need <= PK_CH_8 ? PK_CH_8 : need <= PK_CH_7 ? PK_CH_7 : need <= PK_CH_SMALL ? PK_CH_SMALL : LdsCfg<double>::CH;
}
template <bool PUSH, int NS, int BITS, bool DOT = false, int CHE = LdsCfg<double>::CH, int RR = PK_R>
__global__ __launch_bounds__(VB) void k_spmv_ldsp(int n, const int *__restrict__ rowptr, const v4i *__restrict__ packed,
                                                  const int *__restrict__ pofs, const int *__restrict__ pbase,
                                                  const double *__restrict__ val, const double *__restrict__ x,
                                                  double *__restrict__ y, const int *done, PushPlan pp, DotPlan dp, RunStretches st)
{
    if (PUSH && (int)blockIdx.x < pp.nblocks) { push_block(pp, blockIdx.x); return; }
    if (PUSH && pp.nrecv > 0 && (int)blockIdx.x >= (int)gridDim.x - pp.nrecv) { recv_block(pp, (int)blockIdx.x - ((int)gridDim.x - pp.nrecv)); return; }
    const int bid = PUSH ? blockIdx.x - pp.nblocks : blockIdx.x;
    constexpr int R = RR;
    constexpr int T = VB / R;
    constexpr int UNR = NS;
    constexpr int CH = CHE;
    constexpr int PER = 128 / BITS;
    constexpr int NG = (CH + PER - 1) / PER;
    constexpr int GR = (NG + VB - 1) / VB;
    constexpr int VR = (CH / 2 + 1 + VB - 1) / VB;
    __shared__ __attribute__((aligned(16))) double sval[CH + 2];
    __shared__ __attribute__((aligned(16))) int scol[NG * PER];
    double(*sred)[R] = reinterpret_cast<double(*)[R]>(sval);
    const int tid = threadIdx.x;
    const int row0 = bid * R;
    const int rl = tid % R, j0 = tid / R;

    auto run_block = [&](auto stretch_tag, int s, int e, int nrows, int L, int kd, const int *__restrict__ bcol, int cadd, int Q, double uv) {
        constexpr bool STRETCH = decltype(stretch_tag)::value;
        const int bv = s & ~1, cntv = e - bv;
        const int w = __builtin_amdgcn_readfirstlane(j0);
        const bool live = rl < nrows;
        v2d pv[VR];
#pragma unroll
        for (int r = 0; r < VR; r++) {
            const int u = 2 * (tid + r * VB);
            pv[r] = *reinterpret_cast<const v2d *>(val + (long)bv + (u < cntv ? u : 0));
        }
        int stop = 0, cs[UNR];
        const int *__restrict__ tw = bcol + (STRETCH ? w * Q : 0);
        if constexpr (STRETCH) {
            if (done) stop = *done;
#pragma unroll
            for (int q = 0; q < UNR; q++) cs[q] = tw[q];
        }
        double xv[UNR];
#pragma unroll
        for (int q = 0; q < UNR; q++) {
            const int k = w + q * T;
            const int c0 = STRETCH ? cs[q] + cadd : bcol[k < L ? k : 0];
            xv[q] = x[(k < L && live) ? c0 + rl : 0];
        }
        __builtin_amdgcn_sched_barrier(0);
        if (STRETCH && stop) return;
#pragma unroll
        for (int r = 0; r < VR; r++) {
            const int u = 2 * (tid + r * VB);
            if (u < cntv) *reinterpret_cast<v2d *>(sval + u) = pv[r];
        }
        __syncthreads();
        double acc = 0.0;
        const int rs0 = s + rl * L - bv;
        double *sud = reinterpret_cast<double *>(scol);
        if (live) {
#pragma unroll
            for (int q = 0; q < UNR; q++) {
                const int k = w + q * T;
                acc = k < L ? fma(sval[rs0 + k], xv[q], acc) : acc;
                if (DOT && k == kd) sud[rl] = xv[q];
            }
            for (int k = w + UNR * T; k < L; k += T) {
                const double xk = x[(STRETCH ? tw[k / T] + cadd : bcol[k]) + rl];
                acc = fma(sval[rs0 + k], xk, acc);
                if (DOT && k == kd) sud[rl] = xk;
            }
        }
        __syncthreads();
        sred[j0][rl] = acc;
        __syncthreads();
        if (DOT && kd >= 0 && j0 == 0 && live) uv = sud[rl];
        double vfin = 0.0;
        if (j0 == 0 && live) {
            double v = sred[0][rl];
#pragma unroll
            for (int j = 1; j < T; j++) v += sred[j][rl];
            y[row0 + rl] = v;
            vfin = v;
        }
        if (DOT) ldsp_dot_tail(dp, bid, j0, vfin, uv);
    };

    if constexpr (RR == 64) {
        static_assert(T == 4, "the stretches' tables are laid out for four wavefronts per block");
        RunStretch me = st.s[0];
#pragma unroll
        for (int i = 1; i < RS_MAX; i++) {
            const RunStretch c = st.s[i];
            const bool in = bid >= c.b0 && bid < c.b1;
            me.b0 = in ? c.b0 : me.b0; me.b1 = in ? c.b1 : me.b1; me.s0 = in ? c.s0 : me.s0; me.L = in ? c.L : me.L;
            me.kd = in ? c.kd : me.kd; me.Q = in ? c.Q : me.Q; me.off = in ? c.off : me.off;
        }
        if (bid >= me.b0 && bid < me.b1) {
            const int s = me.s0 + (bid - me.b0) * (R * me.L);
            const int kd = (DOT && dp.ux) ? me.kd : -1;
            double uv = 0.0;
            if (DOT && kd < 0) uv = dp.u[j0 == 0 ? row0 + rl : 0];
            run_block(std::true_type{}, s, s + R * me.L, R, me.L, kd, me.off, row0, me.Q, uv);
            return;
        }
    }
    if (done && *done) return;

    const int nrows = min(R, n - row0);
    const int s = rowptr[row0], e = rowptr[row0 + nrows];
    const int dof = RR == 64 ? 1 : dp.dof;
    const int cnt = e - s, ng = (cnt + PER * dof - 1) / (PER * dof);
    const int po = pofs[bid], bs = pbase[bid];
    const int bv = s & ~1, cntv = e - bv;
    double uv = 0.0;
    int kd = -1;
    if (DOT && RR == 64 && dp.ux && bs < 0)
        kd = reinterpret_cast<const int *>(packed + po)[bs > -TPL_CODE ? -1 - bs : -bs - TPL_CODE];
    if (DOT && kd < 0) uv = dp.u[(j0 == 0 && rl < nrows) ? row0 + rl : 0];

    if (RR == 64 && bs <= -TPL_CODE) {
        static_assert(UNR * T >= TPL_MAXROW || NS < 8, "one predicated batch covers the longest row of a template block");
        const int D = -bs - TPL_CODE;
        const int *tplp = reinterpret_cast<const int *>(packed + po);
        const int *mskp = tplp + ((D + 1 + 3) & ~3);
        const bool live = rl < nrows;
        double vfin = 0.0;
        auto block = [&](auto wide_tag) {
            constexpr bool WIDE = decltype(wide_tag)::value;
            typedef typename std::conditional<WIDE, unsigned long long, unsigned>::type M;
            const M mask = live ? reinterpret_cast<const M *>(mskp)[rl] : (M)0;
            const int myoff = tplp[rl < D ? rl : 0];
            const int rs = (live ? rowptr[row0 + rl] : bv) - bv;
            v2d pv[VR];
#pragma unroll
            for (int r = 0; r < VR; r++) {
                const int u = 2 * (tid + r * VB);
                pv[r] = *reinterpret_cast<const v2d *>(val + (long)bv + (u < cntv ? u : 0));
            }
            const int len = WIDE ? __popcll((unsigned long long)mask) : __popc((unsigned)mask);
            const M full = D >= (WIDE ? 64 : 32) ? ~(M)0 : (((M)1 << D) - (M)1);
            const bool dense = __ballot(live && mask != full) == 0ull;
            M m = mask;
            if (!dense)
                for (int i = __builtin_amdgcn_readfirstlane(j0); i > 0; i--) m &= m - (M)1;
            double xv[UNR];
#pragma unroll
            for (int q = 0; q < UNR; q++) {
                int slot = j0 + q * T;
                if (!dense) {
                    slot = m ? (WIDE ? __builtin_ctzll((unsigned long long)m) : __builtin_ctz((unsigned)m)) : 0;
#pragma unroll
                    for (int t = 0; t < T; t++) m &= m - (M)1;
                }
                const int off = __shfl(myoff, slot & 63, 64);
                const bool ok = live && j0 + q * T < len;
                xv[q] = x[ok ? rl + off : 0];
            }
            __builtin_amdgcn_sched_barrier(0);
#pragma unroll
            for (int r = 0; r < VR; r++) {
// ... 274 lines not shown
        if (L <= 4) run_rows(std::integral_constant<int, 4>{});
        else if (L <= 6) run_rows(std::integral_constant<int, 6>{});
        else run_rows(std::integral_constant<int, NB>{});
    } else {
        int rs = 0, re = 0;
        if (live) { rs = rowptr[row0 + lane]; re = rowptr[row0 + lane + 1]; }
        int longest = re - rs;
        for (int off = 32; off > 0; off >>= 1) longest = max(longest, __shfl_xor(longest, off, 64));
        auto walk_rows = [&](auto nbt) {
            constexpr int NBX = decltype(nbt)::value;
            static_assert(NBX % T == 0, "entry k goes to partial sum k mod T");
            for (int k0 = rs; __ballot(k0 < re) != 0; k0 += NBX) {
                int c[NBX]; double a[NBX], xv[NBX];
#pragma unroll
                for (int q = 0; q < NBX; q++) { const bool ok = k0 + q < re; c[q] = col[ok ? k0 + q : 0]; a[q] = val[ok ? k0 + q : 0]; }
#pragma unroll
                for (int q = 0; q < NBX; q++) xv[q] = x[k0 + q < re ? c[q] : 0];
#pragma unroll
                for (int q = 0; q < NBX; q++) acc[q % T] = (k0 + q < re) ? fma(a[q], xv[q], acc[q % T]) : acc[q % T];
            }
        };
        if (longest <= 4) walk_rows(std::integral_constant<int, 4>{});
        else if (longest <= 6) walk_rows(std::integral_constant<int, 6>{});
        else walk_rows(std::integral_constant<int, NB>{});
    }
    double v = acc[0];
#pragma unroll
    for (int j = 1; j < T; j++) v += acc[j];
    if (live) y[row0 + lane] = v;
    return live ? v : 0.0;
}

template <int T>
__global__ __launch_bounds__(VB) void k_spmv_run1(int n, int LP, const int *__restrict__ rowptr, const int *__restrict__ col,
                                                  const double *__restrict__ val, const int *__restrict__ pofs,
                                                  const int *__restrict__ pbase, const int *__restrict__ pcols,
                                                  const double *__restrict__ x, double *__restrict__ y, const int *done)
{
    extern __shared__ double wlds[];
    if (done && *done) return;
    const int wv = __builtin_amdgcn_readfirstlane((int)(threadIdx.x >> 6));
    const int b = blockIdx.x * (VB / 64) + wv;
    if ((long)b * 64 >= n) return;
    (void)run1_block<T>(b, wv, n, LP, rowptr, col, val, pofs, pbase, pcols, x, y, wlds);
}

constexpr int RUN1D_WG = 512;
template <int T>
__global__ __launch_bounds__(RUN1D_WG) void k_spmv_run1d(int n, int LP, const int *__restrict__ rowptr, const int *__restrict__ col,
                                                         const double *__restrict__ val, const int *__restrict__ pofs,
                                                         const int *__restrict__ pbase, const int *__restrict__ pcols,
                                                         const double *__restrict__ x, double *__restrict__ y, const int *done, DotPlan dp)
{
    extern __shared__ double wlds[];
    __shared__ double wsum[2][RUN1D_WG / 64];
    __shared__ int arrived;
    if (done && *done) return;
    if (threadIdx.x == 0) arrived = 0;
    __syncthreads();
    const int lane = threadIdx.x & 63;
    const int wv = __builtin_amdgcn_readfirstlane((int)(threadIdx.x >> 6));
    const int b = blockIdx.x * (RUN1D_WG / 64) + wv;
    double a0 = 0.0, a1 = 0.0;
    if ((long)b * 64 < n) {
        const long row = (long)b * 64 + lane;
        const double uv = dp.u[row < n ? row : 0];
        const double v = run1_block<T>(b, wv, n, LP, rowptr, col, val, pofs, pbase, pcols, x, y, wlds);
        a0 = wave_sum(v * uv);
        if (dp.yy) a1 = wave_sum(v * v);
    }
    if (lane == WSUM_LANE) {
        wsum[0][wv] = a0; wsum[1][wv] = a1;
        const int ticket = __hip_atomic_fetch_add(&arrived, 1, __ATOMIC_ACQ_REL, __HIP_MEMORY_SCOPE_WORKGROUP);
        if (ticket == RUN1D_WG / 64 - 1) {
            double t0 = 0.0, t1 = 0.0;
#pragma unroll
            for (int q = 0; q < RUN1D_WG / 64; q++) { t0 += wsum[0][q]; t1 += wsum[1][q]; }
            dp.part[blockIdx.x] = t0;
            if (dp.yy) dp.part[dp.stride + blockIdx.x] = t1;
        }
    }
}




static bool run_stretches_on(const CsrPart &P)
{
    static const int env = [] { const char *e = std::getenv("LCG_HIP_RUN_STRETCHES"); return e ? atoi(e) : -1; }();
    return (env >= 0 ? env : P.rs_mode) != 0;
}

static void run_stretches_free(const CsrPart &P)
{
    if (P.pk_rs_off) hipFree(P.pk_rs_off);
    P.pk_rs_off = nullptr; P.pk_rs = RunStretches(); P.pk_rs_blocks = 0; P.pk_rs_groups = 0;
}

static void run_stretches_build(const CsrPart &P, hipStream_t s, const std::vector<int> &flag)
{
    struct St { int b0, b1, L; };
    std::vector<St> all;
    const int nb = (int)flag.size();
    for (int b = 0; b < nb;) {
        if (flag[b] <= 0) { b++; continue; }
        int e = b + 1;
        while (e < nb && flag[e] == -flag[b]) e++;
        if (e - b >= 2) all.push_back({b, e, flag[b]});
        b = e;
    }
    if (all.empty()) return;
    std::stable_sort(all.begin(), all.end(), [](const St &a, const St &c) { return a.b1 - a.b0 > c.b1 - c.b0; });
    if (all.size() > (size_t)RS_MAX) all.resize(RS_MAX);
    std::sort(all.begin(), all.end(), [](const St &a, const St &c) { return a.b0 < c.b0; });
    RunStretches rs;
    rs.n = (int)all.size();
    int ints = 0;
    for (int i = 0; i < rs.n; i++) {
        rs.s[i].b0 = all[i].b0; rs.s[i].b1 = all[i].b1; rs.s[i].L = all[i].L; rs.s[i].Q = std::max(RS_QMIN, (all[i].L + 3) / 4);
        ints += 4 * rs.s[i].Q;
    }
    int h[2 * RS_MAX];
    bool ok = hipMalloc(&P.pk_rs_off, sizeof(int) * ((size_t)ints + 2 * RS_MAX)) == hipSuccess;
    if (ok) {
        hipLaunchKernelGGL(k_pk_stretch_fill, dim3(rs.n), dim3(64), 0, s, rs, P.rowptr, P.col, P.pk_rs_off, P.pk_rs_off + ints);
        ok = hipMemcpyAsync(h, P.pk_rs_off + ints, sizeof(int) * 2 * rs.n, hipMemcpyDeviceToHost, s) == hipSuccess &&
             hipStreamSynchronize(s) == hipSuccess;
    }
    if (!ok) { (void)hipGetLastError(); run_stretches_free(P); return; }
    int o = 0;
    for (int i = 0; i < rs.n; i++) {
        RunStretch &r = rs.s[i];
        r.s0 = h[2 * i]; r.kd = h[2 * i + 1]; r.off = P.pk_rs_off + o;
        o += 4 * r.Q;
        P.pk_rs_blocks += r.b1 - r.b0;
        P.pk_rs_groups += (long)(r.b1 - r.b0) * ((r.L + 1 + 3) / 4);
    }
    P.pk_rs = rs;
}

static bool packed_build(const CsrPart &P, hipStream_t s, bool runs_only, int R = PK_R)
{
    if (P.pk_state != 0) return P.pk_state == (runs_only ? 2 : 1) && P.pk_R == R;
    P.pk_state = -1;
    static const int env = [] { const char *e = std::getenv("LCG_HIP_PACKED"); return e ? atoi(e) : -1; }();
    const int mode = env >= 0 ? env : P.pk_mode;
    if (mode == 0) return false;
    if (!runs_only && mode < 0 && P.nnz < (1 << 22)) return false;
    PlanTimer timer(P, s);
    const int n = P.n_rows;
    const int nb = (n + R - 1) / R;
    int *ngr = nullptr, *span = nullptr, *sflag = nullptr;
    std::vector<int> hflag;
    const bool stretches = !runs_only && R == PK_R && run_stretches_on(P);
    long total = 0;
    int hspan[4] = {0, 0, 0, 0};
    int dof = 1;
    if (R != PK_R && !runs_only) {
        int *d = nullptr, h[3] = {1, 1, 1};
        bool okd = hipMalloc(&d, sizeof h) == hipSuccess && hipMemcpyAsync(d, h, sizeof h, hipMemcpyHostToDevice, s) == hipSuccess;
        if (okd) {
            hipLaunchKernelGGL(k_pk_dof, dim3((n + VB - 1) / VB), dim3(VB), 0, s, n, P.rowptr, P.col, d);
            okd = hipMemcpyAsync(h, d, sizeof h, hipMemcpyDeviceToHost, s) == hipSuccess && hipStreamSynchronize(s) == hipSuccess;
        }
        if (d) hipFree(d);
        if (okd) dof = h[2] ? 4 : (h[1] ? 3 : (h[0] ? 2 : 1));
        else (void)hipGetLastError();
    }
    bool ok = hipMalloc(&P.pk_base, sizeof(int) * (size_t)nb) == hipSuccess && hipMalloc(&P.pk_ofs, sizeof(int) * ((size_t)nb + 1)) == hipSuccess &&
              hipMalloc(&ngr, sizeof(int) * (size_t)nb) == hipSuccess && hipMalloc(&span, 4 * sizeof(int)) == hipSuccess &&
              hipMemsetAsync(span, 0, 4 * sizeof(int), s) == hipSuccess;
    if (ok) {
        hipLaunchKernelGGL(k_pk_meta, dim3(nb), dim3(64), 0, s, n, P.rowptr, P.col, P.pk_base, ngr, span, R == PK_R ? 1 : 0, R);
        if (stretches && hipMalloc(&sflag, sizeof(int) * (size_t)nb) == hipSuccess) {
            hflag.resize(nb);
            hipLaunchKernelGGL(k_pk_stretch_flags, dim3((nb + VB - 1) / VB), dim3(VB), 0, s, n, nb, P.rowptr, P.col, P.pk_base, sflag);
            if (hipMemcpyAsync(hflag.data(), sflag, sizeof(int) * (size_t)nb, hipMemcpyDeviceToHost, s) != hipSuccess) { (void)hipGetLastError(); hflag.clear(); }
        }
        ok = hipMemcpyAsync(hspan, span, 4 * sizeof(int), hipMemcpyDeviceToHost, s) == hipSuccess && hipStreamSynchronize(s) == hipSuccess;
    }
    if (ok) ok = runs_only ? 2L * (hspan[2] + hspan[3]) >= nb : hspan[0] < PK_SPAN;
    const int bits = runs_only ? 0 : (hspan[0] < (1 << 18) ? 18 : 21);
    if (ok) {
        hipLaunchKernelGGL(k_pk_groups, dim3((nb + VB - 1) / VB), dim3(VB), 0, s, nb, runs_only ? 0 : (128 / bits) * dof, ngr);
        ok = device_exclusive_scan(nb, ngr, P.pk_ofs, s, &total) == 0;
    }
    if (ok) ok = total > 0 && total < 0x7fffffffL;
    if (ok) ok = hipMalloc(&P.pk_data, 16 * ((size_t)total + 4)) == hipSuccess;
    if (ok) {
        if (runs_only)
            hipLaunchKernelGGL(k_pk_pack<0>, dim3(nb), dim3(VB), 0, s, n, P.rowptr, P.col, P.pk_base, P.pk_ofs, static_cast<v4i *>(P.pk_data), R, 1);
        else if (bits == 18)
            hipLaunchKernelGGL(k_pk_pack<18>, dim3(nb), dim3(VB), 0, s, n, P.rowptr, P.col, P.pk_base, P.pk_ofs, static_cast<v4i *>(P.pk_data), R, dof);
        else
            hipLaunchKernelGGL(k_pk_pack<21>, dim3(nb), dim3(VB), 0, s, n, P.rowptr, P.col, P.pk_base, P.pk_ofs, static_cast<v4i *>(P.pk_data), R, dof);
        ok = hipGetLastError() == hipSuccess;
    }
    if (ngr) hipFree(ngr);
    if (span) hipFree(span);
    if (sflag) hipFree(sflag);
    if (!ok) {
        (void)hipGetLastError();
        if (P.pk_base) hipFree(P.pk_base);
        if (P.pk_ofs) hipFree(P.pk_ofs);
        if (P.pk_data) hipFree(P.pk_data);
        P.pk_base = P.pk_ofs = nullptr; P.pk_data = nullptr;
        return false;
    }
    P.pk_maxrow = hspan[1];
    P.pk_runs = hspan[2];
    P.pk_tpls = hspan[3];
    P.pk_groups = total;
    P.pk_bits = bits;
    P.pk_R = R;
    P.pk_dof = dof;
    P.pk_state = runs_only ? 2 : 1;
    if (!hflag.empty() && hspan[2] > 1) run_stretches_build(P, s, hflag);
    return true;
}
static bool packed_ready(const CsrPart &P, hipStream_t s, int R = PK_R) { return packed_build(P, s, false, R); }

static const char *ldsp_name(const CsrPart &P, bool dot)
{
    const int form = (P.pk_runs > 0 ? 1 : 0) + (P.pk_tpls > 0 ? 2 : 0);
    if (dot) {
        static const char *const d[4] = {"k_spmv_ldsp (LDS-staged, packed columns) carrying the dot that follows the product",
                                         "k_spmv_ldsp (LDS-staged, run blocks + packed columns) carrying the dot that follows the product",
                                         "k_spmv_ldsp (LDS-staged, template blocks + packed columns) carrying the dot that follows the product",
                                         "k_spmv_ldsp (LDS-staged, run blocks + template blocks + packed columns) carrying the dot that follows the product"};
        return d[form];
    }
    static const char *const a[2][4] = {{"k_spmv_ldsp (LDS-staged, 18-bit packed columns)", "k_spmv_ldsp (LDS-staged, run blocks + 18-bit packed columns)",
                                         "k_spmv_ldsp (LDS-staged, template blocks + 18-bit packed columns)",
                                         "k_spmv_ldsp (LDS-staged, run blocks + template blocks + 18-bit packed columns)"},
                                        {"k_spmv_ldsp (LDS-staged, 21-bit packed columns)", "k_spmv_ldsp (LDS-staged, run blocks + 21-bit packed columns)",
                                         "k_spmv_ldsp (LDS-staged, template blocks + 21-bit packed columns)",
                                         "k_spmv_ldsp (LDS-staged, run blocks + template blocks + 21-bit packed columns)"}};
    return a[P.pk_bits == 18 ? 0 : 1][form];
}

template <class V>
static int lds_shape(const CsrPart &P, int variant, double mean_row, hipStream_t s, int *R_out, bool *onewin)
{
    const int n = P.n_rows;
    const double cap = LdsCfg<V>::CH - 64;
    const int R = variant < -1 ? -variant
                               : (256 * mean_row <= cap ? 256 : 128 * mean_row <= cap ? 128 : 64 * mean_row <= cap ? 64
                                  : 32 * mean_row <= cap ? 32 : 16);
    if (P.slice_R != R) {
        int *d = nullptr, h = 0;
        HIPCHK(hipMalloc(&d, sizeof(int)));
        HIPCHK(hipMemsetAsync(d, 0, sizeof(int), s));
        const int nb = (n + R - 1) / R;
        hipLaunchKernelGGL(k_max_slice, dim3((nb + VB - 1) / VB), dim3(VB), 0, s, n, R, P.rowptr, d);
        hipError_t e = hipMemcpyAsync(&h, d, sizeof(int), hipMemcpyDeviceToHost, s);
        if (e == hipSuccess) e = hipStreamSynchronize(s);
        hipFree(d);
        if (e != hipSuccess) return fail(e, "slice scan", __FILE__, __LINE__);
        P.slice_R = R; P.max_slice = h;
    }
    *R_out = R;
    *onewin = P.padded && P.max_slice <= LdsCfg<V>::CH;
    return 0;
}

enum class Ax { none, long_rows, ranges, binned, tiled, run1, ldsp, ldsp_long, lds1, ldsw, wave };
enum class AxAsk { product, dot, part_dot };
struct AxChoice {
    Ax family = Ax::none;
    int R = 0, T = 0;
    int ns = 0, bits = 0, win = 0;
    bool onewin = false;
};

template <int... Vs, class F> static bool pick(int v, F &&f) { return ((v == Vs ? (f(std::integral_constant<int, Vs>()), true) : false) || ...); }

static int ldsp_ns(const CsrPart &P, int R)
{
    const int per_lane = (P.pk_maxrow + VB / R - 1) / (VB / R);
    if (R == 32) return per_lane <= 7 ? 7 : 9;
    if (R == 16) return per_lane <= 6 ? 6 : 9;
    return per_lane <= 6 ? 6 : per_lane <= 7 ? 7 : per_lane <= 8 ? 8 : per_lane <= 9 ? 9 : per_lane <= 10 ? 10 : per_lane <= 12 ? 12 : 8;
}

template <bool PUSH, bool DOT, int RR = PK_R>
static void ldsp_launch(const AxChoice &c, const CsrPart &P, const double *x, double *y, hipStream_t s, const int *done,
                        const PushPlan &pp, const DotPlan &dp)
{
    const unsigned g = (unsigned)((P.n_rows + RR - 1) / RR) + (PUSH ? (unsigned)(pp.nblocks + pp.nrecv) : 0u);
    const auto go = [&](auto ns) {
        pick<18, 21>(c.bits, [&](auto bits) {
            pick<PK_CH_8, PK_CH_7, PK_CH_SMALL, LdsCfg<double>::CH>(c.win, [&](auto win) {
                hipLaunchKernelGGL((k_spmv_ldsp<PUSH, decltype(ns)::value, decltype(bits)::value, DOT, decltype(win)::value, RR>), dim3(g),
                                   dim3(VB), 0, s, P.n_rows, P.rowptr, static_cast<const v4i *>(P.pk_data), P.pk_ofs, P.pk_base, P.val,
                                   x, y, done, pp, dp, run_stretches_on(P) ? P.pk_rs : RunStretches());
            });
        });
    };
    if constexpr (RR == PK_R) pick<6, 7, 8, 9, 10, 12>(c.ns, go);
    else if constexpr (RR == 32) pick<7, 9>(c.ns, go);
    else pick<6, 9>(c.ns, go);
}

template <class V, bool ACC>
static int ax_choose(const CsrPart &P, int variant, double mean_row, bool push, AxAsk ask, hipStream_t s, AxChoice &c)
{
    c = AxChoice();
    const bool dot = ask != AxAsk::product;
    const bool automatic = variant == 0 || variant == -1;
    if (P.n_rows <= 0 || (dot && !automatic)) return 0;
    const bool al16 = (((uintptr_t)P.val | (uintptr_t)P.col) & 15) == 0;
    const bool whole = !push && ask != AxAsk::part_dot;
    if constexpr (sizeof(V) == 8 && !ACC) {
        if (ask == AxAsk::product && whole && P.lr_mode == 1) { c.family = Ax::long_rows; return 0; }
        if (whole && automatic && ranges_chosen(P, s)) { c.family = Ax::ranges; return 0; }
        if (dot && (mean_row > 160.0 || !al16)) return 0;
        if (!push && automatic && binned_chosen(P, s)) { c.family = Ax::binned; return 0; }
        if (automatic && tiled_chosen(P, s)) { c.family = Ax::tiled; return 0; }
    }
    if (variant == 0) variant = (!al16 || mean_row > 160.0) ? (mean_row > 48 ? 64 : (mean_row > 24 ? 32 : (mean_row > 12 ? 16 : 8))) : -1;
    if (variant > 0) { c.family = Ax::wave; c.T = variant; return 0; }
    if (!al16) return fail(hipErrorInvalidValue, "LDS-staged A.x needs 16-byte aligned col/val", __FILE__, __LINE__);
    { int rc = lds_shape<V>(P, variant, mean_row, s, &c.R, &c.onewin); if (rc) return rc; }
    const int R = c.R;
    c.family = c.onewin ? Ax::lds1 : Ax::ldsw;
    c.win = LdsCfg<V>::CH;
    if constexpr (sizeof(V) == 8 && !ACC) {
        if (dot && !c.onewin) return 0;
        if (whole && variant == -1 && (R == 256 || R == 128) && packed_build(P, s, true) && P.pk_maxrow <= 30) { c.family = Ax::run1; return 0; }
        if ((R == PK_R && c.onewin && packed_ready(P, s)) ||
            (whole && (R == 32 || R == 16) && c.onewin && packed_ready(P, s, R))) {
            c.family = R == PK_R ? Ax::ldsp : Ax::ldsp_long; c.ns = ldsp_ns(P, R); c.bits = P.pk_bits;
            c.win = pk_window(P.max_slice);
            return 0;
        }
        if (c.onewin && P.nnz >= (1 << 22)) c.win = pk_window(P.max_slice);
    }
    return 0;
}

template <class V, bool ACC, bool PUSH = false>
static int spmv_dispatch(const CsrPart &P, int variant, double mean_row, const V *x, V *y, hipStream_t s,
                         const int *done, const PushPlan &pp = PushPlan())
{
    const int n = P.n_rows;
    const unsigned xb = PUSH ? (unsigned)(pp.nblocks + pp.nrecv) : 0u;
    const V *val = reinterpret_cast<const V *>(P.val);
    if (n == 0) {
        if (PUSH && xb > 0) {
            hipLaunchKernelGGL((k_spmv_wave<V, 1, ACC, PUSH>), dim3(xb), dim3(VB), 0, s, 0, P.rowptr, P.col, val, x, y, done, pp);
            HIPCHK(hipGetLastError());
        }
        return 0;
    }
    AxChoice c;
    { int rc = ax_choose<V, ACC>(P, variant, mean_row, PUSH, AxAsk::product, s, c); if (rc) return rc; }
    if constexpr (sizeof(V) == 8 && !ACC) {
        const double *xd = reinterpret_cast<const double *>(x);
        double *yd = reinterpret_cast<double *>(y);
        switch (c.family) {
        case Ax::long_rows: return long_rows_launch(P, xd, yd, s, done);
        case Ax::ranges: {
            RangePlan *R = static_cast<RangePlan *>(P.rg_plan);
            bool changed = false;
            for (size_t i = 0; i < R->parts.size(); i++) {
                const CsrPart &Q = R->parts[i];
                int rc = spmv_dispatch<V, false, false>(Q, variant, Q.n_rows ? (double)Q.nnz / Q.n_rows : 0.0, x, y + R->r0[i], s, done);
                if (rc) return rc;
                if (Q.last_kernel != R->seen[i]) { R->seen[i] = Q.last_kernel; changed = true; }
            }
            if (changed) {
                R->desc.clear();
                for (size_t i = 0; i < R->parts.size(); i++) {
                    char buf[64];
                    std::snprintf(buf, sizeof buf, "%srows [%d, %d): ", i ? " | " : "", R->r0[i], R->r0[i] + R->parts[i].n_rows);
                    R->desc += buf; R->desc += R->parts[i].last_kernel;
                }
            }
            P.last_kernel = R->desc.c_str();
            return 0;
        }
        case Ax::binned:
            P.last_kernel = "k_bin_expand + k_bin_reduce (two-pass binned product, x and row sums in LDS)";
            return binned_launch(P, xd, yd, s, done);
        case Ax::tiled:
            P.last_kernel = PUSH ? "k_tile_spmv (one-pass tiled product: x tiles and row sums in LDS) + pushing blocks"
                                 : "k_tile_spmv (one-pass tiled product: x tiles and row sums in LDS)";
            return tiled_launch(P, xd, yd, s, done, PUSH ? &pp : nullptr);
        case Ax::run1: {
            const unsigned g = (unsigned)(((n + 63) / 64 + VB / 64 - 1) / (VB / 64));
            const int LP = P.pk_maxrow | 1;
            const size_t lds = sizeof(double) * (VB / 64) * 64 * (size_t)LP;
            pick<1, 2>(c.R == 256 ? 1 : 2, [&](auto t) {
                hipLaunchKernelGGL((k_spmv_run1<decltype(t)::value>), dim3(g), dim3(VB), lds, s, n, LP, P.rowptr, P.col, P.val, P.pk_ofs,
                                   P.pk_base, static_cast<const int *>(P.pk_data), xd, yd, done); });
            HIPCHK(hipGetLastError());
            P.last_kernel = "k_spmv_run1 (one wavefront per 64-row block, run blocks without staging)";
            return 0;
        }
        case Ax::ldsp:
            ldsp_launch<PUSH, false>(c, P, xd, yd, s, done, pp, DotPlan());
            HIPCHK(hipGetLastError());
            P.last_kernel = ldsp_name(P, false);
            return 0;
        case Ax::ldsp_long:
            if constexpr (!PUSH) {
                DotPlan dp; dp.dof = P.pk_dof;
                (c.R == 32 ? ldsp_launch<false, false, 32> : ldsp_launch<false, false, 16>)(c, P, xd, yd, s, done, PushPlan(), dp);
                HIPCHK(hipGetLastError());
                P.last_kernel = P.pk_dof > 1 ? (P.pk_bits == 18 ? "k_spmv_ldsp (LDS-staged, long rows: one 18-bit packed column per group of consecutive columns)"
                                                               : "k_spmv_ldsp (LDS-staged, long rows: one 21-bit packed column per group of consecutive columns)")
                                             : (P.pk_bits == 18 ? "k_spmv_ldsp (LDS-staged, long rows: 18-bit packed columns)" : "k_spmv_ldsp (LDS-staged, long rows: 21-bit packed columns)");
                return 0;
            }
            break;
        default: break;
        }
    }
    if (c.family == Ax::wave) {
        const bool ok = pick<1, 2, 4, 8, 16, 32, 64>(c.T, [&](auto T) {
            constexpr int TT = decltype(T)::value;
            hipLaunchKernelGGL((k_spmv_wave<V, TT, ACC, PUSH>), dim3((unsigned)(((long)n * TT + VB - 1) / VB) + xb), dim3(VB), 0, s,
                               n, P.rowptr, P.col, val, x, y, done, pp);
        });
        if (!ok) return fail(hipErrorInvalidValue, "bad A.x lanes-per-row", __FILE__, __LINE__);
        P.last_kernel = "k_spmv_wave (lanes per row, shuffle reduction)";
    } else {
        const long nnz = P.end_abs >= 0 ? P.end_abs : P.nnz;
        const bool ok = pick<256, 128, 64, 32, 16>(c.R, [&](auto R) {
            constexpr int RR = decltype(R)::value;
            const dim3 g((n + RR - 1) / RR + xb);
            if (!c.onewin)
                hipLaunchKernelGGL((k_spmv_ldsw<V, RR, ACC, PUSH>), g, dim3(VB), 0, s, n, nnz, P.rowptr, P.col, val, x, y, done, pp);
            else if constexpr (sizeof(V) == 8 && !ACC)
                pick<PK_CH_8, PK_CH_7, PK_CH_SMALL, LdsCfg<double>::CH>(c.win, [&](auto win) {
                    hipLaunchKernelGGL((k_spmv_lds1<V, RR, ACC, PUSH, decltype(win)::value>), g, dim3(VB), 0, s, n, nnz, P.rowptr, P.col,
                                       val, x, y, done, pp);
                });
            else
                hipLaunchKernelGGL((k_spmv_lds1<V, RR, ACC, PUSH>), g, dim3(VB), 0, s, n, nnz, P.rowptr, P.col, val, x, y, done, pp);
        });
        if (!ok) return fail(hipErrorInvalidValue, "bad LDS A.x rows-per-block", __FILE__, __LINE__);
        P.last_kernel = c.onewin ? "k_spmv_lds1 (LDS-staged CSR)" : "k_spmv_ldsw (LDS-staged CSR, windowed)";
    }
    HIPCHK(hipGetLastError());
    return 0;
}

int spmv_launch(const CsrPart &P, bool is_complex, int variant, double mean_row, const double *x, double *y,
                bool accumulate, hipStream_t s, const int *done)
{
    if (is_complex) {
        auto xv = reinterpret_cast<const double2 *>(x);
        auto yv = reinterpret_cast<double2 *>(y);
        return accumulate ? spmv_dispatch<double2, true>(P, variant, mean_row, xv, yv, s, done)
                          : spmv_dispatch<double2, false>(P, variant, mean_row, xv, yv, s, done);
    }
    return accumulate ? spmv_dispatch<double, true>(P, variant, mean_row, x, y, s, done)
                      : spmv_dispatch<double, false>(P, variant, mean_row, x, y, s, done);
}

int spmv_launch_push(const CsrPart &P, bool is_complex, int variant, double mean_row, const double *x, double *y,
                     hipStream_t s, const int *done, const PushPlan &pp)
{
    if (is_complex)
        return spmv_dispatch<double2, false, true>(P, variant, mean_row, reinterpret_cast<const double2 *>(x),
                                                   reinterpret_cast<double2 *>(y), s, done, pp);
    return spmv_dispatch<double, false, true>(P, variant, mean_row, x, y, s, done, pp);
}

static bool ensure_dot_part(const CsrPart &P, long count)
{
    if (P.dot_part && P.dot_cap >= count) return true;
    if (P.dot_part) { if (ctx().inited) (void)hipDeviceSynchronize(); (void)hipFree(P.dot_part); P.dot_part = nullptr; P.dot_cap = 0; }
    if (hipMalloc(&P.dot_part, sizeof(double) * 2 * (size_t)count) != hipSuccess) { (void)hipGetLastError(); P.dot_part = nullptr; return false; }
    P.dot_cap = count;
    return true;
}

static int part_dot_launch(const CsrPart &P, const AxChoice &c, const double *x, double *y, const double *u, int yy, double *part,
                           int *slots, hipStream_t s, const int *done, const PushPlan *pp, int *nofold)
{
    int nsum = 0;
    if (c.family == Ax::tiled) {
        nsum = tiled_chunks(P);
        if (nsum <= 0 || !ensure_dot_part(P, nsum)) return 0;
        DotPlan dp; dp.u = u; dp.part = P.dot_part; dp.yy = yy; dp.stride = nsum;
        int rc = tiled_launch(P, x, y, s, done, pp, &dp);
        if (rc) return rc;
        P.last_kernel = pp ? "k_tile_spmv (one-pass tiled product: x tiles and row sums in LDS) + pushing blocks, carrying the dot that follows the product"
                           : "k_tile_spmv (one-pass tiled product: x tiles and row sums in LDS) carrying the dot that follows the product";
    } else if (c.family == Ax::ldsp) {
        nsum = (P.n_rows + PK_R - 1) / PK_R;
        if (!ensure_dot_part(P, nsum)) return 0;
        DotPlan dp; dp.u = u; dp.part = P.dot_part; dp.yy = yy; dp.stride = nsum; dp.ux = u == x ? 1 : 0;
        if (pp) ldsp_launch<true, true>(c, P, x, y, s, done, *pp, dp);
        else ldsp_launch<false, true>(c, P, x, y, s, done, PushPlan(), dp);
        HIPCHK(hipGetLastError());
        P.last_kernel = ldsp_name(P, true);
    } else
        return 0;
    if (nofold) { *nofold = nsum; *slots = 0; return 1; }
    const int g2 = std::min(512, (nsum + VB - 1) / VB);
    const int per = (nsum + g2 - 1) / g2;
    hipLaunchKernelGGL(k_axp_fold, dim3((nsum + per - 1) / per), dim3(VB), 0, s, P.dot_part, nsum, nsum, per, yy, part, done);
    HIPCHK(hipGetLastError());
    *slots = (nsum + per - 1) / per;
    return 1;
}

int csr_part_ax_dot(const CsrPart &P, int variant, double mean_row, const double *x, double *y, const double *u, int yy, double *part,
                    int *slots, hipStream_t s, const int *done, const PushPlan *pp, int *nofold)
{
    AxChoice c;
    { int rc = ax_choose<double, false>(P, variant, mean_row, pp != nullptr, AxAsk::part_dot, s, c); if (rc) return rc; }
    return part_dot_launch(P, c, x, y, u, yy, part, slots, s, done, pp, nofold);
}

int csr_ax_dot(lcg_hip_csr *A, const double *x, double *y, const double *u, int yy, double *part, int *slots, hipStream_t s,
               const int *done)
{
    static const bool off = [] { const char *e = std::getenv("LCG_HIP_AX_DOT"); return e && atoi(e) == 0; }();
    if (off || !A || A->is_complex || A->c64 || A->n_rows <= 0) return 0;
    if (A->distributed) return dist_ax_dot(A, x, y, u, yy, part, slots);
    const CsrPart &P = A->main;
    const int n = P.n_rows;
    AxChoice c;
    { int rc = ax_choose<double, false>(P, A->variant, A->mean_row, false, AxAsk::dot, s, c); if (rc) return rc; }
    switch (c.family) {
    case Ax::tiled:
    case Ax::ldsp: return part_dot_launch(P, c, x, y, u, yy, part, slots, s, done, nullptr, nullptr);
    case Ax::run1: {
        const int nwg = (int)((((long)n + 63) / 64 + RUN1D_WG / 64 - 1) / (RUN1D_WG / 64));
        if (P.pk_maxrow > 15 || nwg > AXP_CAP) break;
        DotPlan dp; dp.u = u; dp.part = part; dp.yy = yy;
        const int LP = P.pk_maxrow | 1;
        const size_t lds = sizeof(double) * (RUN1D_WG / 64) * 64 * (size_t)LP;
        pick<1, 2>(c.R == 256 ? 1 : 2, [&](auto t) {
            hipLaunchKernelGGL((k_spmv_run1d<decltype(t)::value>), dim3(nwg), dim3(RUN1D_WG), lds, s, n, LP, P.rowptr, P.col, P.val, P.pk_ofs,
                               P.pk_base, static_cast<const int *>(P.pk_data), x, y, done, dp); });
        HIPCHK(hipGetLastError());
        P.last_kernel = "k_spmv_run1d (one wavefront per 64-row block, run blocks without staging) carrying the dot that follows the product";
        *slots = nwg;
        return 1;
    }
    case Ax::lds1: break;
    default: return 0;
    }
    constexpr int maxblk = 2048;
    const int nblk = (n + c.R - 1) / c.R;
    if (nblk > maxblk) return 0;
    DotPlan dp; dp.u = u; dp.part = part; dp.yy = yy;
    const bool ok = pick<256, 128, 64, 32, 16>(c.R, [&](auto R) {
        hipLaunchKernelGGL((k_spmv_lds1d<decltype(R)::value>), dim3(nblk), dim3(VB), 0, s, n, P.rowptr, P.col, P.val, x, y, done, dp);
    });
    if (!ok) return 0;
    HIPCHK(hipGetLastError());
    P.last_kernel = "k_spmv_lds1d (LDS-staged CSR carrying the dot that follows the product)";
    *slots = nblk;
    return 1;
}

void free_part(CsrPart &P)
{
    long_rows_free(P);
    ranges_free(P);
    binned_free(P);
    tiled_free(P);
    if (P.owned) { hipFree(P.rowptr); hipFree(P.col); hipFree(P.val); }
    if (P.pk_base) hipFree(P.pk_base);
    if (P.pk_ofs) hipFree(P.pk_ofs);
    if (P.pk_data) hipFree(P.pk_data);
    run_stretches_free(P);
    if (P.dot_part) hipFree(P.dot_part);
    P = CsrPart();
}

}

using namespace lcgh;

namespace lcgh { void dist_free(lcg_hip_csr *A); }

extern "C" {

int lcg_hip_csr_create(lcg_hip_csr_t *out, int n_rows, int n_cols, int64_t nnz, const int *rowptr, const int *col,
                       const double *val, int is_complex, int mem, int adopt)
{
    if (!out || n_rows <= 0 || nnz < 0 || nnz > 0x7fffffffLL || !rowptr || !col || !val) return LCG_HIP_E_ARG;
    int rc = ensure_init(); if (rc) return rc;
    Ctx &c = ctx();
    lcg_hip_csr *A = new lcg_hip_csr();
    A->n_rows = n_rows; A->n_cols = n_cols; A->is_complex = is_complex != 0;
    A->mean_row = (double)nnz / n_rows;
    if (mem == LCG_HIP_MEM_DEVICE && adopt) {
        A->main.n_rows = n_rows; A->main.nnz = nnz; A->main.owned = false; A->main.padded = adopt == 2;
        A->main.n_cols = n_cols;
        A->main.rowptr = const_cast<int *>(rowptr); A->main.col = const_cast<int *>(col); A->main.val = const_cast<double *>(val);
    } else {
        rc = alloc_part(A->main, n_rows, nnz, A->is_complex);
        if (rc) { delete A; return rc; }
        A->main.n_cols = n_cols;
        const hipMemcpyKind kind = mem == LCG_HIP_MEM_DEVICE ? hipMemcpyDeviceToDevice : hipMemcpyHostToDevice;
        hipError_t e = hipMemcpyAsync(A->main.rowptr, rowptr, sizeof(int) * ((size_t)n_rows + 1), kind, c.stream);
        if (e == hipSuccess && nnz) e = hipMemcpyAsync(A->main.col, col, sizeof(int) * (size_t)nnz, kind, c.stream);
        if (e == hipSuccess && nnz) e = hipMemcpyAsync(A->main.val, val, sizeof(double) * (is_complex ? 2 : 1) * (size_t)nnz, kind, c.stream);
        if (e == hipSuccess) e = hipStreamSynchronize(c.stream);
        if (e != hipSuccess) { free_part(A->main); delete A; return fail(e, "csr upload", __FILE__, __LINE__); }
    }
    *out = A;
    return 0;
}

int lcg_hip_csr_destroy(lcg_hip_csr_t A)
{
    NOT_DENSE(A, LCG_HIP_E_ARG);
    if (!A) return 0;
    ctx().forget_places();
    ctx().released_bytes += (size_t)A->main.nnz * (A->is_complex ? 20 : 12);
    dist_free(A);
    free_part(A->main);
    for (int i = 1; i < 4; i++) free_part(A->op[i]);
    if (A->invdiag) hipFree(A->invdiag);
    tri_factor_free(A->ic0);
    tri_factor_free(A->ilu0);
    c64_free(A);
    A->kind = 0;
    delete A;
    return 0;
}

int lcg_hip_csr_rows(lcg_hip_csr_t A) { NOT_DENSE(A, LCG_HIP_E_ARG); return A ? A->n_rows : 0; }
int64_t lcg_hip_csr_nnz(lcg_hip_csr_t A) { NOT_DENSE(A, LCG_HIP_E_ARG); return A ? A->main.nnz : 0; }
int lcg_hip_csr_arrays(lcg_hip_csr_t A, const int **rowptr, const int **col, const double **val)
{
    NOT_DENSE(A, LCG_HIP_E_ARG);
    if (!A) return LCG_HIP_E_ARG;
    if (rowptr) *rowptr = A->main.rowptr;
    if (col) *col = A->main.col;
    if (val) *val = A->main.val;
    return 0;
}
int lcg_hip_csr_set_kernel(lcg_hip_csr_t A, int variant)
{
    NOT_DENSE(A, LCG_HIP_E_ARG);
    if (!A) return LCG_HIP_E_ARG;
    TRY_C64(A, "lcg_hip_csr_set_kernel");
    A->variant = variant;
    return 0;
}

}

static void op_copies_free(lcg_hip_csr *A)
{
    if (!A->op[1].rowptr && !A->op[2].rowptr && !A->op[3].rowptr) return;
    if (ctx().inited) (void)hipDeviceSynchronize();
    for (int i = 1; i < 4; i++) free_part(A->op[i]);
}

extern "C" {

int lcg_hip_csr_set_packed(lcg_hip_csr_t A, int mode)
{
    NOT_DENSE(A, LCG_HIP_E_ARG);
    if (!A || mode < -1 || mode > 1) return LCG_HIP_E_ARG;
    TRY_C64(A, "lcg_hip_csr_set_packed");
    if (mode == 0) op_copies_free(A);
    for (CsrPart *P : {&A->main, &A->loc}) {
        P->pk_mode = mode;
        ranges_free(*P);
        if (P->pk_state > 0 && mode == 0) {
            if (ctx().inited) (void)hipDeviceSynchronize();
            hipFree(P->pk_base); hipFree(P->pk_ofs); hipFree(P->pk_data);
            P->pk_base = P->pk_ofs = nullptr; P->pk_data = nullptr;
            run_stretches_free(*P);
        }
        if (P->pk_state < 0 || mode == 0) P->pk_state = 0;
    }
    return 0;
}

int lcg_hip_csr_set_binned(lcg_hip_csr_t A, int mode)
{
    NOT_DENSE(A, LCG_HIP_E_ARG);
    if (!A || mode < -1 || mode > 1) return LCG_HIP_E_ARG;
    TRY_C64(A, "lcg_hip_csr_set_binned");
    if (mode == 0) op_copies_free(A);
    for (CsrPart *P : {&A->main, &A->loc}) {
        P->bn_mode = mode;
        ranges_free(*P);
        if (mode == 0) binned_free(*P);
        else P->bn_state = 0;
    }
    return 0;
}

int lcg_hip_csr_set_tiled(lcg_hip_csr_t A, int mode)
{
    NOT_DENSE(A, LCG_HIP_E_ARG);
    if (!A || mode < -1 || mode > 1) return LCG_HIP_E_ARG;
    TRY_C64(A, "lcg_hip_csr_set_tiled");
    if (mode == 0) op_copies_free(A);
    for (CsrPart *P : {&A->main, &A->loc}) {
        P->tl_mode = mode;
        ranges_free(*P);
        if (mode == 0) tiled_free(*P);
        else P->tl_state = 0;
    }
    return 0;
}

int lcg_hip_csr_set_ranges(lcg_hip_csr_t A, int mode)
{
    NOT_DENSE(A, LCG_HIP_E_ARG);
    if (!A || mode < -1 || mode > 1) return LCG_HIP_E_ARG;
    TRY_C64(A, "lcg_hip_csr_set_ranges");
    if (mode == 0) op_copies_free(A);
    if (ctx().inited) (void)hipDeviceSynchronize();
    for (CsrPart *P : {&A->main, &A->loc}) { ranges_free(*P); P->rg_mode = mode; }
    return 0;
}

int lcg_hip_csr_ranges(lcg_hip_csr_t A, int cap, int *first_row)
{
    NOT_DENSE(A, LCG_HIP_E_ARG);
    if (!A) return 0;
    const CsrPart &P = A->distributed ? A->loc : A->main;
    const RangePlan *R = static_cast<const RangePlan *>(P.rg_plan);
    if (!R || P.rg_state <= 0) return 0;
    for (int i = 0; i < cap && i < (int)R->r0.size() && first_row; i++) first_row[i] = R->r0[i];
    return (int)R->r0.size();
}

const char *lcg_hip_csr_tiled_status(lcg_hip_csr_t A)
{
    NOT_DENSE(A, "");
    if (!A) return "";
    return A->distributed ? A->loc.tl_why : A->main.tl_why;
}

const char *lcg_hip_csr_last_kernel(lcg_hip_csr_t A)
{
    NOT_DENSE(A, "");
    if (!A) return "";
    return A->distributed ? A->loc.last_kernel : A->main.last_kernel;
}

const char *lcg_hip_csr_binned_status(lcg_hip_csr_t A)
{
    NOT_DENSE(A, "");
    if (!A) return "";
    return A->distributed ? A->loc.bn_why : A->main.bn_why;
}

int64_t lcg_hip_csr_packed_runs(lcg_hip_csr_t A, int64_t *blocks_out)
{
    NOT_DENSE(A, LCG_HIP_E_ARG);
    if (!A) return 0;
    const CsrPart &P = A->distributed ? A->loc : A->main;
    if (blocks_out) *blocks_out = (P.n_rows + P.pk_R - 1) / P.pk_R;
    return P.pk_state > 0 ? P.pk_runs : 0;
}

int lcg_hip_csr_set_run_stretches(lcg_hip_csr_t A, int mode)
{
    NOT_DENSE(A, LCG_HIP_E_ARG);
    if (!A || mode < 0 || mode > 1) return LCG_HIP_E_ARG;
    TRY_C64(A, "lcg_hip_csr_set_run_stretches");
    for (CsrPart *P : {&A->main, &A->loc}) {
        P->rs_mode = mode;
        ranges_free(*P);
        if (mode == 1 && P->pk_state == 1 && P->pk_rs.n == 0) {
            if (ctx().inited) (void)hipDeviceSynchronize();
            hipFree(P->pk_base); hipFree(P->pk_ofs); hipFree(P->pk_data);
            P->pk_base = P->pk_ofs = nullptr; P->pk_data = nullptr;
            P->pk_state = 0;
        }
    }
    return 0;
}

static bool stretches_in_use(const CsrPart &P) { return P.pk_state == 1 && run_stretches_on(P) && P.pk_rs.n > 0; }

int64_t lcg_hip_csr_run_stretches(lcg_hip_csr_t A, int64_t *blocks_out)
{
    NOT_DENSE(A, LCG_HIP_E_ARG);
    if (blocks_out) *blocks_out = 0;
    if (!A) return 0;
    const CsrPart &P = A->distributed ? A->loc : A->main;
    if (!stretches_in_use(P)) return 0;
    if (blocks_out) *blocks_out = P.pk_rs_blocks;
    return P.pk_rs.n;
}

static int64_t part_traffic_model(const CsrPart &P)
{
    const char *k = P.last_kernel;
    if (!k || !*k) return 0;
    if (P.rg_state > 0 && P.rg_plan) {
        const RangePlan *R = static_cast<const RangePlan *>(P.rg_plan);
        int64_t b = 0;
        const int64_t xbytes = 8 * (P.n_cols > 0 ? P.n_cols : (int64_t)P.n_rows);
        for (const CsrPart &Q : R->parts) b += part_traffic_model(Q) - xbytes;
        return b + xbytes;
    }
    const int64_t n = P.n_rows, ncols = P.n_cols > 0 ? P.n_cols : P.n_rows;
    const int64_t vectors = 4 * (n + 1) + 8 * ncols + 8 * n;
    const int64_t nb = (n + P.pk_R - 1) / P.pk_R;
    if (std::strncmp(k, "k_lr_", 5) == 0) return 12 * P.nnz + vectors;
    if (std::strncmp(k, "k_bin_", 6) == 0) return binned_traffic_bytes(P);
    if (std::strncmp(k, "k_tile", 6) == 0) return tiled_traffic_bytes(P);
    if (std::strncmp(k, "k_spmv_ldsp", 11) == 0) {
        int64_t b = 8 * P.nnz + 16 * (int64_t)P.pk_groups + 8 * nb + vectors;
        if (stretches_in_use(P)) {
            b -= (4 * PK_R + 8) * (int64_t)P.pk_rs_blocks + 16 * (int64_t)P.pk_rs_groups;
            for (int i = 0; i < P.pk_rs.n; i++) b += 16 * P.pk_rs.s[i].Q;
        }
        return b;
    }
    if (std::strncmp(k, "k_spmv_run1", 11) == 0) {
        const double other = nb > 0 ? 1.0 - (double)(P.pk_runs + P.pk_tpls) / (double)nb : 1.0;
        return 8 * P.nnz + (int64_t)(4.0 * other * (double)P.nnz) + 16 * (int64_t)P.pk_groups + 8 * nb + vectors;
    }
    return 12 * P.nnz + vectors;
}

int64_t lcg_hip_csr_packed_templates(lcg_hip_csr_t A)
{
    NOT_DENSE(A, LCG_HIP_E_ARG);
    if (!A) return 0;
    const CsrPart &P = A->distributed ? A->loc : A->main;
    return P.pk_state > 0 ? P.pk_tpls : 0;
}

int64_t lcg_hip_csr_last_traffic_model(lcg_hip_csr_t A)
{
    NOT_DENSE(A, LCG_HIP_E_ARG);
    if (!A || A->is_complex || A->c64) return 0;
    return part_traffic_model(A->distributed ? A->loc : A->main);
}

int lcg_hip_csr_plan_info(lcg_hip_csr_t A, double *build_ms, int64_t *extra_bytes)
{
    NOT_DENSE(A, LCG_HIP_E_ARG);
    if (!A) return LCG_HIP_E_ARG;
    const CsrPart &P = A->distributed ? A->loc : A->main;
    double ms = P.plan_ms;
    int64_t b = 0;
    auto add = [&](const CsrPart &Q) {
        if (Q.pk_state > 0) b += 16 * ((int64_t)Q.pk_groups + 4) + 8 * (((int64_t)Q.n_rows + Q.pk_R - 1) / Q.pk_R + 1);
        for (int i = 0; i < Q.pk_rs.n; i++) b += 16 * Q.pk_rs.s[i].Q;
        if (Q.bn_plan) b += (int64_t)binned_plan_bytes(Q);
        if (Q.tl_plan) b += (int64_t)tiled_plan_bytes(Q);
    };
    add(P);
    if (P.rg_state > 0 && P.rg_plan)
        for (const CsrPart &Q : static_cast<const RangePlan *>(P.rg_plan)->parts) { add(Q); ms += Q.plan_ms; }
    if (build_ms) *build_ms = ms;
    if (extra_bytes) *extra_bytes = b;
    return 0;
}

static inline void park(int rc) { if (rc && !ctx().ax_rc) ctx().ax_rc = rc; }

void lcg_hip_csr_ax(void *instance, const double *x, double *y, const int n)
{
    NOT_DENSE_CB(instance);
    lcg_hip_csr *A = static_cast<lcg_hip_csr *>(instance);
    (void)n;
    park(lcg_hip_spmv(A, x, y));
}

void clcg_hip_csr_ax(void *instance, const double *x, double *y, const int n, int layout, int conjugate)
{
    NOT_DENSE_CB(instance);
    (void)n;
    park(lcg_hip_spmv_op(static_cast<lcg_hip_csr *>(instance), x, y, layout, conjugate));
}

void lcg_hip_jacobi_mx(void *instance, const double *x, double *z, const int n)
{
    NOT_DENSE_CB(instance);
    park(jacobi_launch(static_cast<lcg_hip_csr *>(instance), x, z, n, ctx().stream));
}

int lcg_hip_spmv_op(lcg_hip_csr_t A, const double *x, double *y, int layout, int conjugate)
{
    NOT_DENSE(A, LCG_HIP_E_ARG);
    if (!A || !x || !y) return LCG_HIP_E_ARG;
    TRY_C64(A, "lcg_hip_spmv_op");
    if (!layout && (!conjugate || !A->is_complex)) return lcg_hip_spmv(A, x, y);
    Ctx &c = ctx();
    const CsrPart *P = nullptr;
    int rc = op_part(A, layout, conjugate, &P);
    if (rc) return rc;
    if (A->distributed) return dist_spmv_op(A, *P, x, y);
    return spmv_launch(*P, A->is_complex, A->variant, A->mean_row, x, y, false, c.stream,
                       ax_flag(c));
}


int lcg_hip_spmv(lcg_hip_csr_t A, const double *x, double *y)
{
    NOT_DENSE(A, LCG_HIP_E_ARG);
    if (!A || !x || !y) return LCG_HIP_E_ARG;
    TRY_C64(A, "lcg_hip_spmv");
    Ctx &c = ctx();
    if (A->distributed) return dist_spmv(A, x, y);
    return spmv_launch(A->main, A->is_complex, A->variant, A->mean_row, x, y, false, c.stream,
                       ax_flag(c));
}

}
```

### liblcg_amd/csrc/csr_build.hip

```cpp
#include <algorithm>
#include <cstring>
#include <functional>
#include <numeric>

#include "devcommon.hpp"

namespace lcgh {

template <class V>
__global__ void k_diag(int n, long row0, const int *rowptr, const int *col, const V *val, V *diag, V *inv)
{
    const int i = blockIdx.x * blockDim.x + threadIdx.x;
    if (i >= n) return;
    V d = vzero(V());
    for (int k = rowptr[i]; k < rowptr[i + 1]; k++)
        if (col[k] == row0 + i) { d = val[k]; break; }
    if (diag) diag[i] = d;
    if (inv) {
        if constexpr (sizeof(V) == 8) inv[i] = 1.0 / d;
        else inv[i] = cdiv(make_double2(1.0, 0.0), d);
    }
}

struct OpMul {
// ... 332 lines not shown
        const int v = perm[a];
        int b = a - 1;
        while (b >= s && perm[b] > v) { perm[b + 1] = perm[b]; b--; }
        perm[b + 1] = v;
    }
}
template <class V>
__global__ void k_coo_gather(long nnz, const int *perm, const int *colin, const V *valin, int *col, V *val)
{
    for (long k = (long)blockIdx.x * blockDim.x + threadIdx.x; k < nnz; k += (long)gridDim.x * blockDim.x) {
        const int src = perm[k];
        col[k] = colin[src]; val[k] = valin[src];
    }
}

int alloc_part(CsrPart &P, int n_rows, long nnz, bool cplx)
{
    P.n_rows = n_rows; P.nnz = nnz; P.owned = true;
    HIPCHK(hipMalloc(&P.rowptr, sizeof(int) * ((size_t)n_rows + 1)));
    HIPCHK(hipMalloc(&P.col, sizeof(int) * (size_t)std::max<long>(nnz, 1) + 64));
    HIPCHK(hipMalloc(&P.val, sizeof(double) * (cplx ? 2 : 1) * (size_t)std::max<long>(nnz, 1) + 64));
    P.padded = true;
    return 0;
}


__global__ void k_tr_count(long nnz, const int *col, int *cnt)
{
    for (long k = (long)blockIdx.x * blockDim.x + threadIdx.x; k < nnz; k += (long)gridDim.x * blockDim.x)
        atomicAdd(&cnt[col[k]], 1);
}
template <class V>
__global__ void k_tr_fill(int n, const int *rowptr, const int *col, const V *val, const int *rpT, int *next, int *colT,
                          V *valT, int conj)
{
    const int i = blockIdx.x * blockDim.x + threadIdx.x;
    if (i >= n) return;
    for (int k = rowptr[i]; k < rowptr[i + 1]; k++) {
        const int c = col[k];
        const int pos = rpT[c] + atomicAdd(&next[c], 1);
        colT[pos] = i;
        V v = val[k];
        if constexpr (sizeof(V) == 16) { if (conj) v.y = -v.y; }
        valT[pos] = v;
    }
}
__device__ __forceinline__ bool val_after(double a, double b) { return a > b; }
__device__ __forceinline__ bool val_after(double2 a, double2 b) { return a.x > b.x || (a.x == b.x && a.y > b.y); }
template <class V>
__global__ void k_row_sort(int n, const int *rowptr, int *col, V *val)
{
    const int i = blockIdx.x * blockDim.x + threadIdx.x;
    if (i >= n) return;
    const int s = rowptr[i], e = rowptr[i + 1];
    for (int a = s + 1; a < e; a++) {
        const int c = col[a]; const V v = val[a];
        int b = a - 1;
        while (b >= s && (col[b] > c || (col[b] == c && val_after(val[b], v)))) { col[b + 1] = col[b]; val[b + 1] = val[b]; b--; }
        col[b + 1] = c; val[b + 1] = v;
    }
}
__global__ void k_conj_copy(long nnz, const double2 *in, double2 *out)
{
    for (long k = (long)blockIdx.x * blockDim.x + threadIdx.x; k < nnz; k += (long)gridDim.x * blockDim.x)
        out[k] = make_double2(in[k].x, -in[k].y);
}

int transpose_launch(int n, int nt, long nnz, const int *rowptr, const int *col, const double *val, int *rpT, int *colT, double *valT,
                     bool cplx, int conj, int *cnt, hipStream_t s)
{
    HIPCHK(hipMemsetAsync(cnt, 0, sizeof(int) * (size_t)nt, s));
    hipLaunchKernelGGL(k_tr_count, dim3(1024), dim3(VB), 0, s, nnz, col, cnt);
    long total = 0;
    int rc = device_exclusive_scan(nt, cnt, rpT, s, &total);
    if (rc || total != nnz) return rc ? rc : fail(hipErrorUnknown, "transpose count", __FILE__, __LINE__);
    HIPCHK(hipMemsetAsync(cnt, 0, sizeof(int) * (size_t)nt, s));
    const unsigned g = (unsigned)((n + VB - 1) / VB);
    const unsigned gt = (unsigned)((nt + VB - 1) / VB);
    if (cplx) {
        hipLaunchKernelGGL((k_tr_fill<double2>), dim3(g), dim3(VB), 0, s, n, rowptr, col, reinterpret_cast<const double2 *>(val), rpT, cnt,
                           colT, reinterpret_cast<double2 *>(valT), conj);
        hipLaunchKernelGGL((k_row_sort<double2>), dim3(gt), dim3(VB), 0, s, nt, rpT, colT, reinterpret_cast<double2 *>(valT));
    } else {
        hipLaunchKernelGGL((k_tr_fill<double>), dim3(g), dim3(VB), 0, s, n, rowptr, col, val, rpT, cnt, colT, valT, 0);
        hipLaunchKernelGGL((k_row_sort<double>), dim3(gt), dim3(VB), 0, s, nt, rpT, colT, valT);
    }
    const hipError_t e = hipStreamSynchronize(s);
    if (e != hipSuccess) return fail(e, "transpose build", __FILE__, __LINE__);
    return 0;
}

void row_sort_launch(int n, const int *rowptr, int *col, double *val, bool cplx, hipStream_t s)
{
    const unsigned g = (unsigned)((n + VB - 1) / VB);
    if (cplx) hipLaunchKernelGGL((k_row_sort<double2>), dim3(g), dim3(VB), 0, s, n, rowptr, col, reinterpret_cast<double2 *>(val));
    else hipLaunchKernelGGL((k_row_sort<double>), dim3(g), dim3(VB), 0, s, n, rowptr, col, val);
}

int op_part(lcg_hip_csr *A, int layout, int conjugate, const CsrPart **out)
{
    TRY_C64(A, "op(A)");
    if (!A->is_complex) conjugate = 0;
    const int idx = (layout ? 2 : 0) + (conjugate ? 1 : 0);
    if (idx == 0) { *out = &A->main; return 0; }
    CsrPart &T = A->op[idx];
    if (T.rowptr) { *out = &T; return 0; }
    if (A->distributed && !layout) return fail(hipErrorInvalidValue, "conj(A).x is not available on a sharded matrix (A^T and A^H are)", __FILE__, __LINE__);
    if (!A->distributed && A->n_cols != A->n_rows) return fail(hipErrorInvalidValue, "op(A) needs a square matrix", __FILE__, __LINE__);
    Ctx &c = ctx();
    const int n = A->n_rows;
    long nt = n;
    if (A->distributed) {
        const long P = (A->n_global + A->rows_per_rank - 1) / A->rows_per_rank;
        nt = P * A->rows_per_rank;
        if (nt > 0x7fffffffL) return fail(hipErrorInvalidValue, "op(A): padded height exceeds int32", __FILE__, __LINE__);
    }
    const long nnz = A->main.nnz;
    int rc = alloc_part(T, (int)nt, nnz, A->is_complex);
    if (rc) return rc;
    T.n_cols = n;
    if (!layout) {
        HIPCHK(hipMemcpyAsync(T.rowptr, A->main.rowptr, sizeof(int) * ((size_t)n + 1), hipMemcpyDeviceToDevice, c.stream));
        HIPCHK(hipMemcpyAsync(T.col, A->main.col, sizeof(int) * (size_t)nnz, hipMemcpyDeviceToDevice, c.stream));
        hipLaunchKernelGGL(k_conj_copy, dim3(1024), dim3(VB), 0, c.stream, nnz, reinterpret_cast<const double2 *>(A->main.val),
                           reinterpret_cast<double2 *>(T.val));
    } else {
        int *cnt = nullptr;
        HIPCHK(hipMalloc(&cnt, sizeof(int) * (size_t)nt));
        rc = transpose_launch(n, (int)nt, nnz, A->main.rowptr, A->main.col, A->main.val, T.rowptr, T.col, T.val, A->is_complex,
                              conjugate, cnt, c.stream);
        hipFree(cnt);
        if (rc) return rc;
    }
    HIPCHK(hipGetLastError());
    *out = &T;
    return 0;
}

}

using namespace lcgh;

extern "C" {

int lcg_hip_csr_from_coo(lcg_hip_csr_t *out, int n, int64_t nnz, const int *row, const int *col, const double *val,
                         int is_complex, int mem)
{
    if (!out || n <= 0 || nnz <= 0 || nnz > 0x7fffffffLL || !row || !col || !val) return LCG_HIP_E_ARG;
    int rc = ensure_init(); if (rc) return rc;
    Ctx &c = ctx();
    const size_t vw = is_complex ? 2 : 1;
    lcg_hip_csr *A = new lcg_hip_csr();
    A->n_rows = n; A->n_cols = n; A->is_complex = is_complex != 0; A->mean_row = (double)nnz / n;
    rc = alloc_part(A->main, n, nnz, A->is_complex);
    if (rc) { delete A; return rc; }
    A->main.n_cols = n;
    int *d_row = nullptr, *d_flag = nullptr;
    const hipMemcpyKind kind = mem == LCG_HIP_MEM_DEVICE ? hipMemcpyDeviceToDevice : hipMemcpyHostToDevice;
    auto bail = [&](int code) { if (d_row) hipFree(d_row); if (d_flag) hipFree(d_flag); free_part(A->main); delete A; return code; };
    if (hipMalloc(&d_row, sizeof(int) * (size_t)nnz) != hipSuccess || hipMalloc(&d_flag, sizeof(int)) != hipSuccess)
        return bail(fail(hipErrorOutOfMemory, "coo staging", __FILE__, __LINE__));
    hipError_t e = hipMemcpyAsync(d_row, row, sizeof(int) * (size_t)nnz, kind, c.stream);
    if (e == hipSuccess) e = hipMemsetAsync(d_flag, 0, sizeof(int), c.stream);
    if (e != hipSuccess) return bail(fail(e, "coo upload", __FILE__, __LINE__));
    const unsigned gb = (unsigned)((nnz + 1 + VB - 1) / VB);
    hipLaunchKernelGGL(k_coo_sorted, dim3(gb), dim3(VB), 0, c.stream, (long)nnz, d_row, d_flag);
    int unsorted = 0;
    e = hipMemcpyAsync(&unsorted, d_flag, sizeof(int), hipMemcpyDeviceToHost, c.stream);
    if (e == hipSuccess) e = hipStreamSynchronize(c.stream);
    if (e != hipSuccess) return bail(fail(e, "coo sortedness", __FILE__, __LINE__));
    if (!unsorted) {
        hipLaunchKernelGGL(k_coo_rowptr, dim3(gb), dim3(VB), 0, c.stream, (long)nnz, n, d_row, A->main.rowptr);
        e = hipMemcpyAsync(A->main.col, col, sizeof(int) * (size_t)nnz, kind, c.stream);
        if (e == hipSuccess) e = hipMemcpyAsync(A->main.val, val, sizeof(double) * vw * (size_t)nnz, kind, c.stream);
        if (e == hipSuccess) e = hipStreamSynchronize(c.stream);
        if (e != hipSuccess) return bail(fail(e, "coo copy", __FILE__, __LINE__));
    } else {
        int *cnt = nullptr, *perm = nullptr, *d_colin = nullptr;
        double *d_valin = nullptr;
        auto bail2 = [&](int code) {
            if (cnt) hipFree(cnt); if (perm) hipFree(perm);
            if (mem != LCG_HIP_MEM_DEVICE) { if (d_colin) hipFree(d_colin); if (d_valin) hipFree(d_valin); }
            return bail(code);
        };
        if (hipMalloc(&cnt, sizeof(int) * (size_t)n) != hipSuccess || hipMalloc(&perm, sizeof(int) * (size_t)nnz) != hipSuccess)
            return bail2(fail(hipErrorOutOfMemory, "coo sort workspace", __FILE__, __LINE__));
        if (mem == LCG_HIP_MEM_DEVICE) { d_colin = const_cast<int *>(col); d_valin = const_cast<double *>(val); }
        else {
            if (hipMalloc(&d_colin, sizeof(int) * (size_t)nnz) != hipSuccess || hipMalloc(&d_valin, sizeof(double) * vw * (size_t)nnz) != hipSuccess)
                return bail2(fail(hipErrorOutOfMemory, "coo staging", __FILE__, __LINE__));
            e = hipMemcpyAsync(d_colin, col, sizeof(int) * (size_t)nnz, hipMemcpyHostToDevice, c.stream);
            if (e == hipSuccess) e = hipMemcpyAsync(d_valin, val, sizeof(double) * vw * (size_t)nnz, hipMemcpyHostToDevice, c.stream);
            if (e != hipSuccess) return bail2(fail(e, "coo upload", __FILE__, __LINE__));
        }
        e = hipMemsetAsync(cnt, 0, sizeof(int) * (size_t)n, c.stream);
        if (e == hipSuccess) e = hipMemsetAsync(d_flag, 0, sizeof(int), c.stream);
        if (e != hipSuccess) return bail2(fail(e, "coo sort init", __FILE__, __LINE__));
        hipLaunchKernelGGL(k_coo_count, dim3(1024), dim3(VB), 0, c.stream, (long)nnz, n, d_row, cnt, d_flag);
        int bad = 0;
        e = hipMemcpyAsync(&bad, d_flag, sizeof(int), hipMemcpyDeviceToHost, c.stream);
        if (e == hipSuccess) e = hipStreamSynchronize(c.stream);
        if (e != hipSuccess) return bail2(fail(e, "coo count", __FILE__, __LINE__));
        if (bad) return bail2(LCG_HIP_E_ARG);
        long total = 0;
        int rc2 = device_exclusive_scan(n, cnt, A->main.rowptr, c.stream, &total);
        if (rc2 || total != nnz) return bail2(rc2 ? rc2 : LCG_HIP_E_ARG);
        e = hipMemsetAsync(cnt, 0, sizeof(int) * (size_t)n, c.stream);
        if (e != hipSuccess) return bail2(fail(e, "coo sort", __FILE__, __LINE__));
        hipLaunchKernelGGL(k_coo_place, dim3(1024), dim3(VB), 0, c.stream, (long)nnz, d_row, A->main.rowptr, cnt, perm);
        hipLaunchKernelGGL(k_perm_sort, dim3((unsigned)((n + VB - 1) / VB)), dim3(VB), 0, c.stream, n, A->main.rowptr, perm);
        if (is_complex)
            hipLaunchKernelGGL((k_coo_gather<double2>), dim3(1024), dim3(VB), 0, c.stream, (long)nnz, perm, d_colin,
                               reinterpret_cast<const double2 *>(d_valin), A->main.col, reinterpret_cast<double2 *>(A->main.val));
        else
            hipLaunchKernelGGL((k_coo_gather<double>), dim3(1024), dim3(VB), 0, c.stream, (long)nnz, perm, d_colin, d_valin,
                               A->main.col, A->main.val);
        e = hipGetLastError();
        if (e == hipSuccess) e = hipStreamSynchronize(c.stream);
        hipFree(cnt); hipFree(perm);
        if (mem != LCG_HIP_MEM_DEVICE) { hipFree(d_colin); hipFree(d_valin); }
        if (e != hipSuccess) return bail(fail(e, "coo device sort", __FILE__, __LINE__));
    }
    hipFree(d_row); hipFree(d_flag);
    *out = A;
    return 0;
}

int lcg_hip_csr_build_jacobi(lcg_hip_csr_t A, double *diag_out)
{
    NOT_DENSE(A, LCG_HIP_E_ARG);
    if (!A) return LCG_HIP_E_ARG;
    if (A->c64) return c64_build_jacobi(A, diag_out);
    Ctx &c = ctx();
    const size_t w = A->is_complex ? 2 : 1;
    if (!A->invdiag) HIPCHK(hipMalloc(&A->invdiag, sizeof(double) * w * (size_t)A->n_rows));
    const unsigned g = (unsigned)((A->n_rows + VB - 1) / VB);
    if (A->is_complex)
        hipLaunchKernelGGL((k_diag<double2>), dim3(g), dim3(VB), 0, c.stream, A->n_rows, (long)A->row0, A->main.rowptr, A->main.col,
                           reinterpret_cast<const double2 *>(A->main.val), reinterpret_cast<double2 *>(diag_out),
                           reinterpret_cast<double2 *>(A->invdiag));
    else
        hipLaunchKernelGGL((k_diag<double>), dim3(g), dim3(VB), 0, c.stream, A->n_rows, (long)A->row0, A->main.rowptr, A->main.col,
                           A->main.val, diag_out, A->invdiag);
    HIPCHK(hipGetLastError());
    return 0;
}


int lcg_hip_vecmul(int n, const double *a, const double *b, double *out)
{
    int rc = ensure_init(); if (rc) return rc;
    int g = launch_vec(OpMul{nullptr, a, b, out}, n, (uintptr_t)a | (uintptr_t)b | (uintptr_t)out, ctx().stream, nullptr);
    return g < 0 ? g : 0;
}
int lcg_hip_vecdiv(int n, const double *a, const double *b, double *out)
{
    int rc = ensure_init(); if (rc) return rc;
    int g = launch_vec(OpDiv{nullptr, a, b, out}, n, (uintptr_t)a | (uintptr_t)b | (uintptr_t)out, ctx().stream, nullptr);
    return g < 0 ? g : 0;
}
int clcg_hip_vecdiv(int n, const double *a, const double *b, double *out)
{
    int rc = ensure_init(); if (rc) return rc;
    hipLaunchKernelGGL(k_cdiv, dim3(grid_for(n)), dim3(VB), 0, ctx().stream, (long)n, reinterpret_cast<const double2 *>(a),
                       reinterpret_cast<const double2 *>(b), reinterpret_cast<double2 *>(out));
    HIPCHK(hipGetLastError());
    return 0;
}

static int finish_generated(lcg_hip_csr *A, int nloc, long r0, int *counts, hipStream_t s,
                            const std::function<void(const int *, int *, double *)> &fill)
{
    long total = 0;
    int *rowptr = nullptr;
    hipError_t e = hipMalloc(&rowptr, sizeof(int) * ((size_t)nloc + 1));
    if (e != hipSuccess) { hipFree(counts); return fail(e, "rowptr", __FILE__, __LINE__); }
    int rc = device_exclusive_scan(nloc, counts, rowptr, s, &total);
    hipFree(counts);
    if (rc) { hipFree(rowptr); return rc; }
    A->main.n_rows = nloc; A->main.nnz = total; A->main.owned = true; A->main.rowptr = rowptr;
    e = hipMalloc(&A->main.col, sizeof(int) * (size_t)total + 64);
    if (e == hipSuccess) e = hipMalloc(&A->main.val, sizeof(double) * (size_t)total + 64);
    A->main.padded = true;
    if (e != hipSuccess) return fail(e, "generated arrays", __FILE__, __LINE__);
    fill(rowptr, A->main.col, A->main.val);
    HIPCHK(hipGetLastError());
    HIPCHK(hipStreamSynchronize(s));
    A->mean_row = (double)total / nloc;
    A->row0 = r0;
    A->main.n_cols = A->n_cols;
    return 0;
}

int lcg_hip_csr_generate(lcg_hip_csr_t *out, int64_t n, int npairs, int64_t band, int symmetric, uint64_t seed,
                         double diag_shift, int64_t r0, int64_t r1)
{
    return lcg_hip_csr_generate_ex(out, n, npairs, band > 0 ? LCG_HIP_GEN_DIAGONALS : LCG_HIP_GEN_SCRAMBLED, band, symmetric, seed,
                                   diag_shift, r0, r1);
}

int lcg_hip_csr_generate_ex(lcg_hip_csr_t *out, int64_t n, int npairs, int pattern, int64_t band, int symmetric, uint64_t seed,
                            double diag_shift, int64_t r0, int64_t r1)
{
    if (!out || n <= 1 || n > 0x7fffffffLL || r0 < 0 || r1 > n || r1 <= r0 || npairs < 1 || pattern < 0 || pattern > 2) return LCG_HIP_E_ARG;
    int rc = ensure_init(); if (rc) return rc;
    Ctx &c = ctx();
    GenParams g; gen_init(g, n, npairs, pattern, band, symmetric, seed, diag_shift);
    const int nloc = (int)(r1 - r0);
    int *counts = nullptr;
    HIPCHK(hipMalloc(&counts, sizeof(int) * (size_t)nloc));
    const unsigned gb = (unsigned)((nloc + VB - 1) / VB);
    hipLaunchKernelGGL(k_gen_count, dim3(gb), dim3(VB), 0, c.stream, g, (long)r0, (long)r1, counts);
    lcg_hip_csr *A = new lcg_hip_csr();
    A->n_rows = nloc; A->n_cols = (int)n; A->is_complex = false;
    rc = finish_generated(A, nloc, r0, counts, c.stream, [&](const int *rp, int *col, double *val) {
        hipLaunchKernelGGL(k_gen_fill, dim3(gb), dim3(VB), 0, c.stream, g, (long)r0, (long)r1, rp, col, val);
    });
    if (rc) { free_part(A->main); delete A; return rc; }
    *out = A;
    return 0;
}

int lcg_hip_gen_xtrue(int64_t n, uint64_t seed, int64_t r0, int64_t r1, double *x_dev)
{
    if (r0 < 0 || r1 > n || r1 <= r0 || !x_dev) return LCG_HIP_E_ARG;
    int rc = ensure_init(); if (rc) return rc;
    const unsigned gb = (unsigned)((r1 - r0 + VB - 1) / VB);
    hipLaunchKernelGGL(k_gen_xtrue, dim3(gb), dim3(VB), 0, ctx().stream, (unsigned long long)seed, (long)r0, (long)r1, x_dev);
    HIPCHK(hipGetLastError());
    return 0;
}

int lcg_hip_csr_laplace2d(lcg_hip_csr_t *out, int nx, int ny, int64_t r0, int64_t r1)
{
    const int64_t n = (int64_t)nx * ny;
    if (!out || nx < 1 || ny < 1 || n > 0x7fffffffLL || r0 < 0 || r1 > n || r1 <= r0) return LCG_HIP_E_ARG;
    int rc = ensure_init(); if (rc) return rc;
    Ctx &c = ctx();
    const int nloc = (int)(r1 - r0);
    int *counts = nullptr;
    HIPCHK(hipMalloc(&counts, sizeof(int) * (size_t)nloc));
    const unsigned gb = (unsigned)((nloc + VB - 1) / VB);
    hipLaunchKernelGGL(k_lap_count, dim3(gb), dim3(VB), 0, c.stream, nx, ny, (long)r0, (long)r1, counts);
    lcg_hip_csr *A = new lcg_hip_csr();
    A->n_rows = nloc; A->n_cols = (int)n; A->is_complex = false;
    rc = finish_generated(A, nloc, r0, counts, c.stream, [&](const int *rp, int *col, double *val) {
        hipLaunchKernelGGL(k_lap_fill, dim3(gb), dim3(VB), 0, c.stream, nx, ny, (long)r0, (long)r1, rp, col, val);
    });
    if (rc) { free_part(A->main); delete A; return rc; }
    *out = A;
    return 0;
}

}
```

### liblcg_amd/csrc/csr_plan.hpp

```cpp
#pragma once

#include <chrono>
#include <string>
#include <vector>

#include "devcommon.hpp"

namespace lcgh {

constexpr int PK_R = 64;

struct PlanTimer {
    const CsrPart &P; hipStream_t s; std::chrono::steady_clock::time_point t0;
    PlanTimer(const CsrPart &p, hipStream_t st) : P(p), s(st), t0(std::chrono::steady_clock::now()) {}
    ~PlanTimer() { (void)hipStreamSynchronize(s); P.plan_ms += std::chrono::duration<double, std::milli>(std::chrono::steady_clock::now() - t0).count(); }
};

struct RangePlan {
    std::vector<CsrPart> parts;
    std::vector<int> r0;
    std::vector<const char *> seen;
    std::string desc;
};

bool binned_chosen(const CsrPart &P, hipStream_t s);
bool tiled_chosen(const CsrPart &P, hipStream_t s);
bool ranges_chosen(const CsrPart &P, hipStream_t s);
void ranges_free(const CsrPart &P);
void long_rows_free(const CsrPart &P);
int long_rows_launch(const CsrPart &P, const double *x, double *y, hipStream_t s, const int *done);
template <class V> struct LdsCfg { static constexpr int CH = sizeof(V) == 8 ? 2240 : 1344; };
void launch_max_slice(int n, int R, const int *rowptr, int *out, hipStream_t s);

}
```

### liblcg_amd/csrc/internal.hpp

```cpp
#pragma once

#include <hip/hip_runtime.h>

#include <cstdint>
#include <cstdio>
#include <cstdlib>
#include <string>
#include <vector>

#include "lcg_hip.h"

namespace lcgh {

inline int debug_level()
{
    static const int lv = [] { const char *e = std::getenv("LCG_HIP_DEBUG"); return e ? atoi(e) : 0; }();
    return lv;
}
inline bool debug_on() { return debug_level() != 0; }


constexpr int VB = 256;
constexpr int MAXG = 2048;
constexpr int MAXR = 8;

enum { ST_RUNNING = 0, ST_CONVERGED = 1, ST_NAN = 2, ST_ALREADY = 3, ST_COMM = 4 };

constexpr int XG_SLOT = 16;
constexpr int XG_MAXP = 64;
struct XgBox {
    double *mine = nullptr;
    double *const *peers = nullptr;
    unsigned long long *seq = nullptr;
    int *fail = nullptr;
    long long timeout_ticks = 0;
    int P = 0, me = 0;
};

constexpr int XG_MAXSEG = 8;
constexpr int PUSH_CHUNK = 4096;
struct DevState;
struct WaitPlan {
    int n = 0;
    unsigned long long seq = 0;
    long long timeout_ticks = 0;
    int *fail = nullptr;
    const unsigned long long *flag[XG_MAXSEG];
};
struct PushPlan {
    int nseg = 0, nflag = 0, nblocks = 0;
    unsigned long long seq = 0;
    unsigned int *ticket = nullptr;
    const double *src[XG_MAXSEG];
    double *dst[XG_MAXSEG];
    long count[XG_MAXSEG];
    int first_block[XG_MAXSEG + 1];
    unsigned long long *flag[XG_MAXSEG];
    int nrecv = 0, rnseg = 0;
    const double *rsrc[XG_MAXSEG];
    double *rdst[XG_MAXSEG];
    long rcount[XG_MAXSEG];
    int rfirst[XG_MAXSEG + 1];
    WaitPlan wp;
    DevState *rst = nullptr;
};


constexpr int AXP_CAP = 16384;
struct PartCount {
    int g[MAXR];
    const double *axp = nullptr;
    int ax_n = 0, ax_row = -1, ax_yy = 0;
    void all(int v) { for (int r = 0; r < MAXR; r++) g[r] = v; ax_row = -1; ax_n = 0; ax_yy = 0; }
};

struct DotPlan {
    const double *u = nullptr;
    double *part = nullptr;
    int yy = 0;
    int stride = AXP_CAP;
    int ux = 0;
    int dof = 1;
};

constexpr int RS_MAX = 4;
constexpr int RS_QMIN = 12;
struct RunStretch {
    int b0 = 0, b1 = 0;
    int s0 = 0;
    int L = 0, kd = -1;
    int Q = 0;
    const int *off = nullptr;
};
struct RunStretches {
    RunStretch s[RS_MAX];
    int n = 0;
};

struct DevState;

struct HostStatus {
    volatile double residual;
    volatile int t;
    volatile int done;
    volatile int status;
    volatile int it;
};

struct DevState {
    double red[MAXR];
    double s[32];
    double residual;
    double eps;
    double n_global;
    int abs_diff;
    int it;
    int t;
    int done;
    int status;
    int pub_mask;
    int zero_guess;
    HostStatus *host;
};

struct Comm;

struct Ctx {
    bool inited = false;
    int device = 0;
    hipStream_t stream = nullptr;
    hipStream_t own_stream = nullptr;
    hipStream_t comm_stream = nullptr;
    hipEvent_t ev_a = nullptr, ev_b = nullptr;
    hipEvent_t ev_switch = nullptr;
    double *partials = nullptr;
    DevState *state = nullptr;
    double *partials_pair[2] = {nullptr, nullptr};
    double *ax_partials = nullptr;
    DevState *state_pair[2] = {nullptr, nullptr};
    HostStatus *hstat = nullptr;
    HostStatus *hstat_dev = nullptr;
    double *scratch_host = nullptr;
    DevState *snap[2] = {nullptr, nullptr};
    DevState *snap_dev[2] = {nullptr, nullptr};
    hipEvent_t snap_ev[2] = {nullptr, nullptr};
    Comm *comm = nullptr;
    int last_iters = 0;
    double last_residual = 0.0;
    bool in_solve = false;
    const int *ax_skip = nullptr;
    int ax_rc = 0;
    int cg_schedule = 0;
    bool profile = false;
    int profile_every = 1;
    long ax_seq = 0;
    std::vector<hipEvent_t> prof_ev;
    int prof_used = 0;
    double last_ax_mean_us = 0.0;
    int last_ax_calls = 0;
    int prof_pending = 0;
    DevState *state_stage = nullptr;
    struct Scratch { double *p; size_t bytes; bool busy; void *arena; };
    std::vector<Scratch> scratch;
    struct PlaceMemo { const void *val; const double *y; float us; };
    std::vector<PlaceMemo> place_memo;
    void forget_places() { place_memo.clear(); }
    void forget_vector(const double *y)
    {
        if (!y) return;
        for (size_t i = 0; i < place_memo.size();) if (place_memo[i].y == y) place_memo.erase(place_memo.begin() + (long)i); else i++;
    }
    struct PlaceTune {
        size_t stream_min = (size_t)768 << 20;
        size_t chunk = (size_t)1 << 30;
        int max_chunks = 128;
        double wall_ms = 60.0;
        size_t hold_max = (size_t)64 << 30;
        double hold_frac = 0.25;
        size_t keep_free = (size_t)8 << 30;
        size_t shared_min = (size_t)4 << 30;
        bool predict = true;
        size_t released_max = (size_t)1 << 30;
        int force_find_at = -1;
    } place_tune;
    size_t released_bytes = 0;
    bool ranks_share_device = false;
    size_t mem_total = 0, mem_free_at_init = 0;
    int cnt_vec = 0, cnt_scal = 0, cnt_allreduce = 0, cnt_ax = 0;
    int walks_made = 0;
    int walk_chunks = 0, walk_found = 0; double walk_ms = 0.0; size_t walk_held = 0; const char *walk_end = "";
    int place_mode = -1;
    int place_timed = 0;
    int place_moved = 0;
    double place_us_first = 0.0, place_us_chosen = 0.0;
    unsigned shadow_seed = 1;
    std::vector<double> shadow_vec;
    std::string err;
};

Ctx &ctx();
int ensure_init();
inline const int *ax_flag(Ctx &c) { return c.ax_skip ? c.ax_skip : (c.in_solve ? &c.state->done : nullptr); }
int fail(hipError_t e, const char *what, const char *file, int line);
int arg_error(const char *fmt, ...) __attribute__((format(printf, 1, 2)));
int launched(const char *what);

#define HIPCHK(call)                                                        \
    do {                                                                    \
        hipError_t e_ = (call);                                             \
        if (e_ != hipSuccess) return ::lcgh::fail(e_, #call, __FILE__, __LINE__); \
    } while (0)

struct CsrPart {
    int n_rows = 0;
    int64_t nnz = 0;
    int *rowptr = nullptr;
    int *col = nullptr;
    double *val = nullptr;
    bool owned = false;
    bool padded = false;
    mutable int slice_R = 0;
    mutable int max_slice = 0;
    mutable int pk_mode = -1;
    mutable int pk_state = 0;
    mutable int *pk_base = nullptr, *pk_ofs = nullptr;
    mutable void *pk_data = nullptr;
    mutable int pk_maxrow = 0;
    mutable int pk_bits = 21;
    mutable int pk_R = 64;
    mutable int pk_dof = 1;
    mutable int pk_runs = 0;
    mutable int pk_tpls = 0;
    mutable long pk_groups = 0;
    mutable int rs_mode = 0;
    mutable RunStretches pk_rs;
    mutable int *pk_rs_off = nullptr;
    mutable long pk_rs_blocks = 0, pk_rs_groups = 0;
    mutable double *dot_part = nullptr;
    mutable long dot_cap = 0;
    int64_t n_cols = 0;
    mutable int bn_mode = -1;
    mutable int bn_state = 0;
    mutable void *bn_plan = nullptr;
    mutable const char *bn_why = "not tried";
    mutable double mean_span = -1.0;
    mutable double line_ratio = -1.0;
    mutable double diag_like = -1.0;
    mutable int tl_mode = -1;
    mutable int tl_state = 0;
    mutable void *tl_plan = nullptr;
    mutable const char *tl_why = "not tried";
    int64_t end_abs = -1;
    mutable int rg_mode = -1;
    mutable int rg_state = 0;
    mutable void *rg_plan = nullptr;
    int lr_mode = 0;
    mutable void *lr_plan = nullptr;
    mutable const char *last_kernel = "";
    mutable double plan_ms = 0.0;
};

}

namespace lcgh {
constexpr uint64_t KIND_CSR = 0x3152534347434C4Cull, KIND_DENSE = 0x534E454447434C4Cull;
inline bool dense_handle(const void *h) { return h && *static_cast<const uint64_t *>(h) == KIND_DENSE; }
inline int refuse_dense(const char *entry, bool park = false)
{
    ctx().err = std::string(entry) + ": the handle is a dense matrix (lcg_hip_dense_t); this entry takes a CSR matrix";
    if (park && !ctx().ax_rc) ctx().ax_rc = LCG_HIP_E_ARG;
    return LCG_HIP_E_ARG;
}
}
#define NOT_DENSE(h, ...) do { if (::lcgh::dense_handle(h)) { ::lcgh::refuse_dense(__func__); return __VA_ARGS__; } } while (0)
#define NOT_DENSE_CB(h) do { if (::lcgh::dense_handle(h)) { ::lcgh::refuse_dense(__func__, true); return; } } while (0)

namespace lcgh { struct TriFactor; }
struct lcg_hip_csr {
    uint64_t kind = lcgh::KIND_CSR;
    int n_rows = 0;
    int n_cols = 0;
    bool is_complex = false;
    lcgh::CsrPart main;
    lcgh::CsrPart op[4];
    double *invdiag = nullptr;
    int variant = 0;
    double mean_row = 0.0;
    bool distributed = false;
    int dist_mode = 0;
    int64_t n_global = 0;
    int64_t row0 = 0;
    int64_t rows_per_rank = 0;
    lcgh::CsrPart loc;
    lcgh::CsrPart rem;
    lcgh::CsrPart remc;
    int *rem_rows = nullptr;
    double *rem_y = nullptr;
    double *xfull = nullptr;
    double *op_z = nullptr;
    void *halo = nullptr;
    void *direct = nullptr;
    lcgh::TriFactor *ic0 = nullptr;
    lcgh::TriFactor *ilu0 = nullptr;
    bool c64 = false;
    void *c64p = nullptr;
};

namespace lcgh {

int spmv_launch(const CsrPart &P, bool is_complex, int variant, double mean_row, const double *x,
                double *y, bool accumulate, hipStream_t s, const int *done_flag);
int spmv_launch_push(const CsrPart &P, bool is_complex, int variant, double mean_row, const double *x, double *y,
                     hipStream_t s, const int *done_flag, const PushPlan &pp);
int jacobi_launch(const lcg_hip_csr *A, const double *x, double *z, int n, hipStream_t s);
int csr_ax_dot(lcg_hip_csr *A, const double *x, double *y, const double *u, int yy, double *part, int *slots, hipStream_t s,
               const int *done_flag);
int csr_part_ax_dot(const CsrPart &P, int variant, double mean_row, const double *x, double *y, const double *u, int yy, double *part,
                    int *slots, hipStream_t s, const int *done_flag, const PushPlan *pp, int *nofold);
int binned_ready(const CsrPart &P, hipStream_t s);
int binned_launch(const CsrPart &P, const double *x, double *y, hipStream_t s, const int *done_flag);
void binned_free(CsrPart &P);
long binned_traffic_bytes(const CsrPart &P);
size_t binned_plan_bytes(const CsrPart &P);
int tiled_ready(const CsrPart &P, hipStream_t s, double min_fill);
int tiled_launch(const CsrPart &P, const double *x, double *y, hipStream_t s, const int *done_flag, const PushPlan *push = nullptr,
                 const DotPlan *dot = nullptr);
int tiled_chunks(const CsrPart &P);
void tiled_free(CsrPart &P);
long tiled_traffic_bytes(const CsrPart &P);
long tiled_tile_copy_bytes(const CsrPart &P);
size_t tiled_plan_bytes(const CsrPart &P);
int op_part(lcg_hip_csr *A, int layout, int conjugate, const CsrPart **out);
int alloc_part(CsrPart &P, int n_rows, long nnz, bool cplx);
int device_exclusive_scan(int n, const int *counts, int *rowptr, hipStream_t s, long *total);
int transpose_launch(int n, int nt, long nnz, const int *rowptr, const int *col, const double *val, int *rpT, int *colT, double *valT,
                     bool cplx, int conj, int *cnt, hipStream_t s);
void row_sort_launch(int n, const int *rowptr, int *col, double *val, bool cplx, hipStream_t s);
void tri_factor_free(TriFactor *&F);
void free_part(CsrPart &P);

void c64_free(lcg_hip_csr *A);
int c64_build_jacobi(lcg_hip_csr *A, void *diag_out);
const float *c64_builtin_invdiag(const void *Mfp, void *inst, int n);
inline int refuse_c64(const lcg_hip_csr *A, const char *entry)
{
    if (!A || !A->c64) return 0;
    ctx().err = std::string(entry) + ": the matrix holds complex64 values; this entry serves fp64 and complex128 matrices "
                "(complex64: lcg_hip_spmv_c64, clcg_hip_csr_ax_c64, clcg_hip_jacobi_mx_c64, lcg_hip_csr_build_ic0_c64, "
                "lcg_hip_ic0_solve_c64, clcg_hip_ic0_mx_c64)";
    return LCG_HIP_E_ARG;
}
#define TRY_C64(A, entry) do { int rc_ = ::lcgh::refuse_c64((A), (entry)); if (rc_) return rc_; } while (0)

int comm_allreduce(double *dev, int count, hipStream_t s);
bool comm_active();
bool xg_box(XgBox *out);
int dist_spmv(lcg_hip_csr *A, const double *x, double *y);
int dist_ax_dot(lcg_hip_csr *A, const double *x, double *y, const double *u, int yy, double *part, int *slots);
int dist_spmv_op(lcg_hip_csr *A, const CsrPart &T, const double *x, double *y);

}
```

Baseline: 1565.

## Add symmetric half-store SpMV path for banded run stretches

Adds a symmetric run-stretch path. For the longest stretch of rows with odd length, antisymmetric offsets and bit-identical mirrored values, only the upper half of the band is packed into a tiled half store. A dedicated kernel reads the lower half from neighbouring tiles, and it runs in a sliced dispatch order; the regular packed kernel skips those blocks through a block-index offset. The aim is to cut matrix value and column traffic roughly in half on symmetric stencils, at the cost of a second launch per product, an extra device buffer and a validation pass when the plan is built.

```diff
diff --git a/include/lcg_hip.h b/include/lcg_hip.h
--- a/include/lcg_hip.h
+++ b/include/lcg_hip.h
@@ -132,6 +132,9 @@
 int64_t lcg_hip_csr_packed_runs(lcg_hip_csr_t A, int64_t *blocks_out);
 int lcg_hip_csr_set_run_stretches(lcg_hip_csr_t A, int mode);
 int64_t lcg_hip_csr_run_stretches(lcg_hip_csr_t A, int64_t *blocks_out);
+int lcg_hip_csr_set_sym_runs(lcg_hip_csr_t A, int mode);
+int lcg_hip_csr_set_sym_slices(lcg_hip_csr_t A, int slices);
+int64_t lcg_hip_csr_sym_runs(lcg_hip_csr_t A, int64_t *blocks_out, const char **status_out);
 int64_t lcg_hip_csr_packed_templates(lcg_hip_csr_t A);
 int lcg_hip_csr_set_binned(lcg_hip_csr_t A, int mode);
 int lcg_hip_csr_set_tiled(lcg_hip_csr_t A, int mode);
diff --git a/liblcg_amd/_lib.py b/liblcg_amd/_lib.py
--- a/liblcg_amd/_lib.py
+++ b/liblcg_amd/_lib.py
@@ -81,6 +81,9 @@
     "lcg_hip_csr_packed_runs": (C.c_int64, [vp, C.POINTER(C.c_int64)]),
     "lcg_hip_csr_set_run_stretches": (C.c_int, [vp, C.c_int]),
     "lcg_hip_csr_run_stretches": (C.c_int64, [vp, C.POINTER(C.c_int64)]),
+    "lcg_hip_csr_set_sym_runs": (C.c_int, [vp, C.c_int]),
+    "lcg_hip_csr_set_sym_slices": (C.c_int, [vp, C.c_int]),
+    "lcg_hip_csr_sym_runs": (C.c_int64, [vp, C.POINTER(C.c_int64), C.POINTER(C.c_char_p)]),
     "lcg_hip_csr_packed_templates": (C.c_int64, [vp]),
     "lcg_hip_csr_set_binned": (C.c_int, [vp, C.c_int]),
     "lcg_hip_csr_set_tiled": (C.c_int, [vp, C.c_int]),
diff --git a/liblcg_amd/api.py b/liblcg_amd/api.py
--- a/liblcg_amd/api.py
+++ b/liblcg_amd/api.py
@@ -148,6 +148,15 @@
 
     def set_kernel(self, variant: int):
         _chk(L.load().lcg_hip_csr_set_kernel(self.h, variant), "set_kernel")
+
+    def set_sym_runs(self, mode: int, slices: int = 0):
+        _chk(L.load().lcg_hip_csr_set_sym_slices(self.h, slices), "set_sym_slices")
+        _chk(L.load().lcg_hip_csr_set_sym_runs(self.h, mode), "set_sym_runs")
+
+    def sym_runs(self):
+        blocks, why = C.c_int64(0), C.c_char_p()
+        nx = L.load().lcg_hip_csr_sym_runs(self.h, C.byref(blocks), C.byref(why))
+        return int(nx), blocks.value, (why.value or b"").decode()
 
     def build_jacobi(self, diag_out=None):
         p = None if diag_out is None else _ptr(diag_out)[0]
diff --git a/liblcg_amd/csrc/comm.hip b/liblcg_amd/csrc/comm.hip
--- a/liblcg_amd/csrc/comm.hip
+++ b/liblcg_amd/csrc/comm.hip
@@ -659,6 +659,8 @@
     A->rem_rows = nullptr; A->rem_y = nullptr;
     if (A->xfull) hipFree(A->xfull);
     A->xfull = nullptr; A->distributed = false;
+    A->main.sym_whole = !A->is_complex && !A->c64;
+    sym_runs_reset(A->main);
     for (int i = 1; i < 4; i++) free_part(A->op[i]);
     if (A->op_z) hipFree(A->op_z);
     A->op_z = nullptr;
@@ -726,6 +728,7 @@
     HIPCHK(hipMemsetAsync(A->xfull, 0, sizeof(double) * (A->is_complex ? 2 : 1) * (size_t)(rpr * nranks), c.stream));
     HIPCHK(hipStreamSynchronize(c.stream));
     A->distributed = true;
+    A->main.sym_whole = false; sym_runs_free(A->main);
     return 0;
 }
 
diff --git a/liblcg_amd/csrc/csr.hip b/liblcg_amd/csrc/csr.hip
--- a/liblcg_amd/csrc/csr.hip
+++ b/liblcg_amd/csrc/csr.hip
@@ -497,18 +497,6 @@
     if (threadIdx.x == 0) { out[2 * blockIdx.x] = s; out[2 * blockIdx.x + 1] = kd; }
 }
 
-__device__ __forceinline__ void ldsp_dot_tail(const DotPlan &dp, int bid, int j0, double vfin, double uv)
-{
-    if (threadIdx.x >= 64) return;
-    if (j0 != 0) vfin = 0.0;
-    const double a0 = wave_sum(vfin * uv);
-    if ((threadIdx.x & 63) == WSUM_LANE) dp.part[bid] = a0;
-    if (dp.yy) {
-        const double a1 = wave_sum(vfin * vfin);
-        if ((threadIdx.x & 63) == WSUM_LANE) dp.part[dp.stride + bid] = a1;
-    }
-}
-
 constexpr int PK_CH_SMALL = 2208;
 constexpr int PK_CH_7 = 1872, PK_CH_8 = 1696;
 static int pk_window(int max_slice)
@@ -517,15 +505,18 @@
     const int need = std::max(max_slice, env);
     return need <= PK_CH_8 ? PK_CH_8 : need <= PK_CH_7 ? PK_CH_7 : need <= PK_CH_SMALL ? PK_CH_SMALL : LdsCfg<double>::CH;
 }
-template <bool PUSH, int NS, int BITS, bool DOT = false, int CHE = LdsCfg<double>::CH, int RR = PK_R>
+struct RunStretchesSkip : RunStretches { int skip_from = 0, skip = 0; };
+template <bool PUSH, int NS, int BITS, bool DOT = false, int CHE = LdsCfg<double>::CH, int RR = PK_R, bool SKIP = false>
 __global__ __launch_bounds__(VB) void k_spmv_ldsp(int n, const int *__restrict__ rowptr, const v4i *__restrict__ packed,
                                                   const int *__restrict__ pofs, const int *__restrict__ pbase,
                                                   const double *__restrict__ val, const double *__restrict__ x,
-                                                  double *__restrict__ y, const int *done, PushPlan pp, DotPlan dp, RunStretches st)
+                                                  double *__restrict__ y, const int *done, PushPlan pp, DotPlan dp,
+                                                  typename std::conditional<SKIP, RunStretchesSkip, RunStretches>::type st)
 {
     if (PUSH && (int)blockIdx.x < pp.nblocks) { push_block(pp, blockIdx.x); return; }
     if (PUSH && pp.nrecv > 0 && (int)blockIdx.x >= (int)gridDim.x - pp.nrecv) { recv_block(pp, (int)blockIdx.x - ((int)gridDim.x - pp.nrecv)); return; }
-    const int bid = PUSH ? blockIdx.x - pp.nblocks : blockIdx.x;
+    int bid = PUSH ? blockIdx.x - pp.nblocks : blockIdx.x;
+    if constexpr (SKIP) { if (bid >= st.skip_from) bid += st.skip; }
     constexpr int R = RR;
     constexpr int T = VB / R;
     constexpr int UNR = NS;
@@ -1106,7 +1097,8 @@
     const int nb = (n + R - 1) / R;
     int *ngr = nullptr, *span = nullptr, *sflag = nullptr;
     std::vector<int> hflag;
-    const bool stretches = !runs_only && R == PK_R && run_stretches_on(P);
+    const bool sym = !runs_only && R == PK_R && sym_runs_wanted(P);
+    const bool stretches = !runs_only && R == PK_R && (run_stretches_on(P) || sym);
     long total = 0;
     int hspan[4] = {0, 0, 0, 0};
     int dof = 1;
@@ -1170,6 +1162,7 @@
     P.pk_dof = dof;
     P.pk_state = runs_only ? 2 : 1;
     if (!hflag.empty() && hspan[2] > 1) run_stretches_build(P, s, hflag);
+    if (sym) sym_runs_build(P, s);
     return true;
 }
 static bool packed_ready(const CsrPart &P, hipStream_t s, int R = PK_R) { return packed_build(P, s, false, R); }
@@ -1191,6 +1184,27 @@
                                          "k_spmv_ldsp (LDS-staged, template blocks + 21-bit packed columns)",
                                          "k_spmv_ldsp (LDS-staged, run blocks + template blocks + 21-bit packed columns)"}};
     return a[P.pk_bits == 18 ? 0 : 1][form];
+}
+
+static const char *sym_runs_name(const CsrPart &P, bool dot)
+{
+#define SYM_AROUND(s) " around k_spmv_ldsp_sym (symmetric run stretch: half store in dispatch order, " s ")"
+#define SYM_NAMES(base, tail) {base SYM_AROUND("one slice") tail, base SYM_AROUND("two slices") tail, base SYM_AROUND("four slices") tail, base SYM_AROUND("eight slices") tail}
+#define SYM_DOT " carrying the dot that follows the product"
+    const int nx = P.pk_sym.NX == 8 ? 3 : P.pk_sym.NX == 4 ? 2 : P.pk_sym.NX == 2 ? 1 : 0, tpl = P.pk_tpls > 0 ? 1 : 0;
+    if (dot) {
+        static const char *const d[2][4] = {SYM_NAMES("k_spmv_ldsp (LDS-staged, run blocks + packed columns)", SYM_DOT),
+                                            SYM_NAMES("k_spmv_ldsp (LDS-staged, run blocks + template blocks + packed columns)", SYM_DOT)};
+        return d[tpl][nx];
+    }
+    static const char *const a[2][2][4] = {{SYM_NAMES("k_spmv_ldsp (LDS-staged, run blocks + 18-bit packed columns)", ""),
+                                            SYM_NAMES("k_spmv_ldsp (LDS-staged, run blocks + template blocks + 18-bit packed columns)", "")},
+                                           {SYM_NAMES("k_spmv_ldsp (LDS-staged, run blocks + 21-bit packed columns)", ""),
+                                            SYM_NAMES("k_spmv_ldsp (LDS-staged, run blocks + template blocks + 21-bit packed columns)", "")}};
+#undef SYM_DOT
+#undef SYM_NAMES
+#undef SYM_AROUND
+    return a[P.pk_bits == 18 ? 0 : 1][tpl][nx];
 }
 
 template <class V>
@@ -1241,19 +1255,34 @@
 static void ldsp_launch(const AxChoice &c, const CsrPart &P, const double *x, double *y, hipStream_t s, const int *done,
                         const PushPlan &pp, const DotPlan &dp)
 {
-    const unsigned g = (unsigned)((P.n_rows + RR - 1) / RR) + (PUSH ? (unsigned)(pp.nblocks + pp.nrecv) : 0u);
-    const auto go = [&](auto ns) {
-        pick<18, 21>(c.bits, [&](auto bits) {
-            pick<PK_CH_8, PK_CH_7, PK_CH_SMALL, LdsCfg<double>::CH>(c.win, [&](auto win) {
-                hipLaunchKernelGGL((k_spmv_ldsp<PUSH, decltype(ns)::value, decltype(bits)::value, DOT, decltype(win)::value, RR>), dim3(g),
-                                   dim3(VB), 0, s, P.n_rows, P.rowptr, static_cast<const v4i *>(P.pk_data), P.pk_ofs, P.pk_base, P.val,
-                                   x, y, done, pp, dp, run_stretches_on(P) ? P.pk_rs : RunStretches());
+    const unsigned nb = (unsigned)((P.n_rows + RR - 1) / RR);
+    const auto launch = [&](auto skip_tag, unsigned g, const auto &st) {
+        constexpr bool SKIP = decltype(skip_tag)::value;
+        const auto go = [&](auto ns) {
+            pick<18, 21>(c.bits, [&](auto bits) {
+                pick<PK_CH_8, PK_CH_7, PK_CH_SMALL, LdsCfg<double>::CH>(c.win, [&](auto win) {
+                    hipLaunchKernelGGL((k_spmv_ldsp<PUSH, decltype(ns)::value, decltype(bits)::value, DOT, decltype(win)::value, RR, SKIP>), dim3(g),
+                                       dim3(VB), 0, s, P.n_rows, P.rowptr, static_cast<const v4i *>(P.pk_data), P.pk_ofs, P.pk_base, P.val,
+                                       x, y, done, pp, dp, st);
+                });
             });
-        });
+        };
+        if constexpr (RR == PK_R) pick<6, 7, 8, 9, 10, 12>(c.ns, go);
+        else if constexpr (RR == 32) pick<7, 9>(c.ns, go);
+        else pick<6, 9>(c.ns, go);
     };
-    if constexpr (RR == PK_R) pick<6, 7, 8, 9, 10, 12>(c.ns, go);
-    else if constexpr (RR == 32) pick<7, 9>(c.ns, go);
-    else pick<6, 9>(c.ns, go);
+    const RunStretches rs = run_stretches_on(P) ? P.pk_rs : RunStretches();
+    if constexpr (!PUSH && RR == PK_R) {
+        if (sym_runs_in_use(P)) {
+            RunStretchesSkip st;
+            static_cast<RunStretches &>(st) = rs;
+            st.skip_from = P.pk_sym.inner0; st.skip = P.pk_sym.NX * P.pk_sym.S;
+            sym_runs_launch(P, DOT, x, y, s, done, dp);
+            launch(std::true_type{}, nb - (unsigned)st.skip, st);
+            return;
+        }
+    }
+    launch(std::false_type{}, nb + (PUSH ? (unsigned)(pp.nblocks + pp.nrecv) : 0u), rs);
 }
 
 template <class V, bool ACC>
@@ -1355,7 +1384,7 @@
         case Ax::ldsp:
             ldsp_launch<PUSH, false>(c, P, xd, yd, s, done, pp, DotPlan());
             HIPCHK(hipGetLastError());
-            P.last_kernel = ldsp_name(P, false);
+            P.last_kernel = sym_runs_in_use(P) ? sym_runs_name(P, false) : ldsp_name(P, false);
             return 0;
         case Ax::ldsp_long:
             if constexpr (!PUSH) {
@@ -1451,7 +1480,7 @@
         if (pp) ldsp_launch<true, true>(c, P, x, y, s, done, *pp, dp);
         else ldsp_launch<false, true>(c, P, x, y, s, done, PushPlan(), dp);
         HIPCHK(hipGetLastError());
-        P.last_kernel = ldsp_name(P, true);
+        P.last_kernel = (!pp && sym_runs_in_use(P)) ? sym_runs_name(P, true) : ldsp_name(P, true);
     } else
         return 0;
     if (nofold) { *nofold = nsum; *slots = 0; return 1; }
@@ -1526,8 +1555,24 @@
     if (P.pk_ofs) hipFree(P.pk_ofs);
     if (P.pk_data) hipFree(P.pk_data);
     run_stretches_free(P);
+    sym_runs_free(P);
     if (P.dot_part) hipFree(P.dot_part);
     P = CsrPart();
+}
+
+void sym_runs_reset(CsrPart &P)
+{
+    ranges_free(P);
+    const bool want = sym_runs_wanted(P);
+    if (!P.pk_sym_H && !(want && P.pk_state == 1)) return;
+    if (ctx().inited) (void)hipDeviceSynchronize();
+    sym_runs_free(P);
+    if (want && P.pk_state == 1) {
+        hipFree(P.pk_base); hipFree(P.pk_ofs); hipFree(P.pk_data);
+        P.pk_base = P.pk_ofs = nullptr; P.pk_data = nullptr;
+        run_stretches_free(P);
+        P.pk_state = 0;
+    }
 }
 
 }
@@ -1547,6 +1592,7 @@
     lcg_hip_csr *A = new lcg_hip_csr();
     A->n_rows = n_rows; A->n_cols = n_cols; A->is_complex = is_complex != 0;
     A->mean_row = (double)nnz / n_rows;
+    A->main.sym_whole = !A->is_complex;
     if (mem == LCG_HIP_MEM_DEVICE && adopt) {
         A->main.n_rows = n_rows; A->main.nnz = nnz; A->main.owned = false; A->main.padded = adopt == 2;
         A->main.n_cols = n_cols;
@@ -1608,6 +1654,7 @@
 
 static void op_copies_free(lcg_hip_csr *A)
 {
+    if (A->main.pk_sym_H || std::strncmp(A->main.sym_why, "refused", 7) == 0) sym_runs_reset(A->main);
     if (!A->op[1].rowptr && !A->op[2].rowptr && !A->op[3].rowptr) return;
     if (ctx().inited) (void)hipDeviceSynchronize();
     for (int i = 1; i < 4; i++) free_part(A->op[i]);
@@ -1629,6 +1676,7 @@
             hipFree(P->pk_base); hipFree(P->pk_ofs); hipFree(P->pk_data);
             P->pk_base = P->pk_ofs = nullptr; P->pk_data = nullptr;
             run_stretches_free(*P);
+            sym_runs_free(*P);
         }
         if (P->pk_state < 0 || mode == 0) P->pk_state = 0;
     }
@@ -1748,6 +1796,40 @@
     return P.pk_rs.n;
 }
 
+int lcg_hip_csr_set_sym_runs(lcg_hip_csr_t A, int mode)
+{
+    NOT_DENSE(A, LCG_HIP_E_ARG);
+    if (!A || mode < -1 || mode > 1) return LCG_HIP_E_ARG;
+    TRY_C64(A, "lcg_hip_csr_set_sym_runs");
+    A->main.sym_mode = mode;
+    sym_runs_reset(A->main);
+    return 0;
+}
+
+int lcg_hip_csr_set_sym_slices(lcg_hip_csr_t A, int slices)
+{
+    NOT_DENSE(A, LCG_HIP_E_ARG);
+    if (!A || (slices != 0 && slices != 1 && slices != 2 && slices != 4 && slices != 8)) return LCG_HIP_E_ARG;
+    TRY_C64(A, "lcg_hip_csr_set_sym_slices");
+    if (A->main.sym_nx == slices) return 0;
+    A->main.sym_nx = slices;
+    sym_runs_reset(A->main);
+    return 0;
+}
+
+int64_t lcg_hip_csr_sym_runs(lcg_hip_csr_t A, int64_t *blocks_out, const char **status_out)
+{
+    NOT_DENSE(A, LCG_HIP_E_ARG);
+    if (blocks_out) *blocks_out = 0;
+    if (status_out) *status_out = "";
+    if (!A) return 0;
+    const CsrPart &P = A->distributed ? A->loc : A->main;
+    if (status_out) *status_out = P.sym_why;
+    if (!sym_runs_in_use(P)) return 0;
+    if (blocks_out) *blocks_out = (int64_t)P.pk_sym.NX * P.pk_sym.S;
+    return P.pk_sym.NX;
+}
+
 static int64_t part_traffic_model(const CsrPart &P)
 {
     const char *k = P.last_kernel;
@@ -1771,6 +1853,10 @@
             b -= (4 * PK_R + 8) * (int64_t)P.pk_rs_blocks + 16 * (int64_t)P.pk_rs_groups;
             for (int i = 0; i < P.pk_rs.n; i++) b += 16 * P.pk_rs.s[i].Q;
         }
+        if (std::strstr(k, "k_spmv_ldsp_sym") && sym_runs_in_use(P) && !stretches_in_use(P)) {
+            const int64_t sb = (int64_t)P.pk_sym.NX * P.pk_sym.S, p = P.pk_sym.p;
+            b -= ((4 * PK_R + 8) + 16 * ((2 * p + 1 + 1 + 3) / 4)) * sb - 16 * P.pk_sym.TQ;
+        }
         return b;
     }
     if (std::strncmp(k, "k_spmv_run1", 11) == 0) {
@@ -1805,6 +1891,7 @@
     auto add = [&](const CsrPart &Q) {
         if (Q.pk_state > 0) b += 16 * ((int64_t)Q.pk_groups + 4) + 8 * (((int64_t)Q.n_rows + Q.pk_R - 1) / Q.pk_R + 1);
         for (int i = 0; i < Q.pk_rs.n; i++) b += 16 * Q.pk_rs.s[i].Q;
+        b += sym_runs_bytes(Q);
         if (Q.bn_plan) b += (int64_t)binned_plan_bytes(Q);
         if (Q.tl_plan) b += (int64_t)tiled_plan_bytes(Q);
     };
diff --git a/liblcg_amd/csrc/csr_build.hip b/liblcg_amd/csrc/csr_build.hip
--- a/liblcg_amd/csrc/csr_build.hip
+++ b/liblcg_amd/csrc/csr_build.hip
@@ -508,6 +508,7 @@
     const size_t vw = is_complex ? 2 : 1;
     lcg_hip_csr *A = new lcg_hip_csr();
     A->n_rows = n; A->n_cols = n; A->is_complex = is_complex != 0; A->mean_row = (double)nnz / n;
+    A->main.sym_whole = !A->is_complex;
     rc = alloc_part(A->main, n, nnz, A->is_complex);
     if (rc) { delete A; return rc; }
     A->main.n_cols = n;
@@ -669,6 +670,7 @@
     hipLaunchKernelGGL(k_gen_count, dim3(gb), dim3(VB), 0, c.stream, g, (long)r0, (long)r1, counts);
     lcg_hip_csr *A = new lcg_hip_csr();
     A->n_rows = nloc; A->n_cols = (int)n; A->is_complex = false;
+    A->main.sym_whole = true;
     rc = finish_generated(A, nloc, r0, counts, c.stream, [&](const int *rp, int *col, double *val) {
         hipLaunchKernelGGL(k_gen_fill, dim3(gb), dim3(VB), 0, c.stream, g, (long)r0, (long)r1, rp, col, val);
     });
@@ -700,6 +702,7 @@
     hipLaunchKernelGGL(k_lap_count, dim3(gb), dim3(VB), 0, c.stream, nx, ny, (long)r0, (long)r1, counts);
     lcg_hip_csr *A = new lcg_hip_csr();
     A->n_rows = nloc; A->n_cols = (int)n; A->is_complex = false;
+    A->main.sym_whole = true;
     rc = finish_generated(A, nloc, r0, counts, c.stream, [&](const int *rp, int *col, double *val) {
         hipLaunchKernelGGL(k_lap_fill, dim3(gb), dim3(VB), 0, c.stream, nx, ny, (long)r0, (long)r1, rp, col, val);
     });
diff --git a/liblcg_amd/csrc/csr_plan.hpp b/liblcg_amd/csrc/csr_plan.hpp
--- a/liblcg_amd/csrc/csr_plan.hpp
+++ b/liblcg_amd/csrc/csr_plan.hpp
@@ -29,6 +29,24 @@
 void ranges_free(const CsrPart &P);
 void long_rows_free(const CsrPart &P);
 int long_rows_launch(const CsrPart &P, const double *x, double *y, hipStream_t s, const int *done);
+bool sym_runs_wanted(const CsrPart &P);
+void sym_runs_build(const CsrPart &P, hipStream_t s);
+inline bool sym_runs_in_use(const CsrPart &P) { return P.pk_state == 1 && P.pk_sym.NX > 0; }
+int64_t sym_runs_bytes(const CsrPart &P);
+void sym_runs_launch(const CsrPart &P, bool dot, const double *x, double *y, hipStream_t s, const int *done, const DotPlan &dp);
+
+__device__ __forceinline__ void ldsp_dot_tail(const DotPlan &dp, int bid, int j0, double vfin, double uv)
+{
+    if (threadIdx.x >= 64) return;
+    if (j0 != 0) vfin = 0.0;
+    const double a0 = wave_sum(vfin * uv);
+    if ((threadIdx.x & 63) == WSUM_LANE) dp.part[bid] = a0;
+    if (dp.yy) {
+        const double a1 = wave_sum(vfin * vfin);
+        if ((threadIdx.x & 63) == WSUM_LANE) dp.part[dp.stride + bid] = a1;
+    }
+}
+
 template <class V> struct LdsCfg { static constexpr int CH = sizeof(V) == 8 ? 2240 : 1344; };
 void launch_max_slice(int n, int R, const int *rowptr, int *out, hipStream_t s);
 
diff --git a/liblcg_amd/csrc/csr_sym.hip b/liblcg_amd/csrc/csr_sym.hip
--- /dev/null
+++ b/liblcg_amd/csrc/csr_sym.hip
@@ -0,0 +1,195 @@
+#include <algorithm>
+#include <vector>
+
+#include "csr_plan.hpp"
+
+namespace lcgh {
+
+constexpr int SYM_NX_DEFAULT = 1;
+constexpr int SYM_MAXL = 36;
+
+static int sym_mode_of(const CsrPart &P)
+{
+    static const int env = [] { const char *e = std::getenv("LCG_HIP_SYM_RUNS"); return e ? atoi(e) : -2; }();
+    return env >= -1 && env <= 1 ? env : P.sym_mode;
+}
+
+static int sym_nx_of(const CsrPart &P)
+{
+    static const int env = [] { const char *e = std::getenv("LCG_HIP_SYM_NX"); return e ? atoi(e) : 0; }();
+    const auto ok = [](int v) { return v == 1 || v == 2 || v == 4 || v == 8; };
+    return ok(env) ? env : ok(P.sym_nx) ? P.sym_nx : SYM_NX_DEFAULT;
+}
+
+bool sym_runs_wanted(const CsrPart &P)
+{
+    if (!P.sym_whole || P.end_abs >= 0) return false;
+    const int mode = sym_mode_of(P);
+    if (mode == 0) return false;
+    return mode == 1 || P.nnz * 12L >= (512L << 20);
+}
+
+void sym_runs_free(const CsrPart &P)
+{
+    if (P.pk_sym_H) (void)hipFree(P.pk_sym_H);
+    P.pk_sym_H = nullptr; P.pk_sym = SymRun(); P.pk_sym_tiles = 0; P.sym_why = "not tried";
+}
+
+int64_t sym_runs_bytes(const CsrPart &P) { return P.pk_sym.NX > 0 ? 8 * P.pk_sym_tiles * (int64_t)(P.pk_sym.p + 1) * PK_R : 0; }
+
+__device__ __forceinline__ int sym_off(const SymRun &sr, int k) { return sr.off[(k % 4) * sr.TQ + k / 4]; }
+
+__global__ __launch_bounds__(VB) void k_sym_check(SymRun sr, int b0, int s0, const double *__restrict__ val, int *flag)
+{
+    const unsigned long long *v = reinterpret_cast<const unsigned long long *>(val);
+    const int b = sr.inner0 + (int)blockIdx.x;
+    const int p = sr.p, L = 2 * p + 1;
+    bool bad = false;
+    for (int idx = threadIdx.x; idx < PK_R * p; idx += VB) {
+        const int r = idx % PK_R, k = idx / PK_R;
+        const long i = (long)(b - b0) * PK_R + r;
+        const long ip = i + sym_off(sr, k);
+        bad |= v[s0 + i * L + k] != v[s0 + ip * L + (2 * p - k)];
+    }
+    if (bad) *flag = 1;
+}
+
+__global__ __launch_bounds__(VB) void k_sym_pack(SymRun sr, int b0, int s0, const double *__restrict__ val, double *__restrict__ H)
+{
+    const int t = blockIdx.x;
+    const int b = t < sr.Q ? sr.inner0 - sr.Q + t : sym_block_of(t - sr.Q, sr.inner0, sr.S, sr.NX);
+    const int p = sr.p, L = 2 * p + 1;
+    const long e0 = s0 + (long)(b - b0) * PK_R * L;
+    double *dst = H + (long)t * (p + 1) * PK_R;
+    for (int idx = threadIdx.x; idx < PK_R * (p + 1); idx += VB) dst[idx] = val[e0 + (long)(idx % PK_R) * L + p + idx / PK_R];
+}
+
+template <int NS, bool DOT>
+__global__ __launch_bounds__(VB) void k_spmv_ldsp_sym(SymRun sr, const double *__restrict__ x, double *__restrict__ y, const int *done, DotPlan dp)
+{
+    constexpr int T = VB / PK_R;
+    static_assert(T == 4, "the stretches' tables are laid out for four wavefronts per block");
+    __shared__ double sred[T][PK_R];
+    __shared__ double sud[PK_R];
+    const int tid = threadIdx.x;
+    const int rl = tid % PK_R, j0 = tid / PK_R;
+    const int w = __builtin_amdgcn_readfirstlane(j0);
+    const int wg = blockIdx.x;
+    const int bid = sym_block_of(wg, sr.inner0, sr.S, sr.NX);
+    const int row0 = bid * PK_R;
+    const int p = sr.p, L = 2 * p + 1;
+    const long TS = (long)(p + 1) * PK_R;
+    const double *__restrict__ H = sr.H;
+    const double *own = H + (long)(sr.Q + wg) * TS;
+    const int *__restrict__ tw = sr.off + w * sr.TQ;
+    int stop = 0, cs[NS];
+    if (done) stop = *done;
+#pragma unroll
+    for (int q = 0; q < NS; q++) cs[q] = tw[q];
+    const int kd = (DOT && dp.ux) ? p : -1;
+    double uv = 0.0;
+    if (DOT && kd < 0) uv = dp.u[j0 == 0 ? row0 + rl : 0];
+    const int jown = wg >> (sr.NX == 8 ? 3 : sr.NX == 4 ? 2 : sr.NX == 2 ? 1 : 0);
+    const auto tile_of = [&](int b) {
+        const int jb = jown - (bid - b);
+        return jb >= 0 ? sr.Q + wg - sr.NX * (bid - b) : sym_tile_of(b, sr.inner0, sr.S, sr.NX, sr.Q);
+    };
+    double xv[NS], av[NS];
+#pragma unroll
+    for (int q = 0; q < NS; q++) {
+        const int k = w + q * T;
+        const bool ok = k < L;
+        const double *a = H;
+        if (ok && k >= p) a = own + (k - p) * PK_R + rl;
+        if (ok && k < p) {
+            const int g = row0 + cs[q];
+            const int bA = g >> 6, sh = g & 63;
+            const double *ta = H + (long)tile_of(bA) * TS + (p - k) * PK_R;
+            const double *tb = H + (long)tile_of(bA + 1) * TS + (p - k) * PK_R;
+            const int rr = rl + sh;
+            a = rr < PK_R ? ta + rr : tb + (rr - PK_R);
+        }
+        av[q] = *a;
+        xv[q] = x[ok ? row0 + cs[q] + rl : 0];
+    }
+    __builtin_amdgcn_sched_barrier(0);
+    if (stop) return;
+    double acc = 0.0;
+#pragma unroll
+    for (int q = 0; q < NS; q++) {
+        const int k = w + q * T;
+        acc = k < L ? fma(av[q], xv[q], acc) : acc;
+        if (DOT && k == kd) sud[rl] = xv[q];
+    }
+    sred[j0][rl] = acc;
+    __syncthreads();
+    if (DOT && kd >= 0 && j0 == 0) uv = sud[rl];
+    double vfin = 0.0;
+    if (j0 == 0) {
+        double v = sred[0][rl];
+#pragma unroll
+        for (int j = 1; j < T; j++) v += sred[j][rl];
+        y[row0 + rl] = v;
+        vfin = v;
+    }
+    if (DOT) ldsp_dot_tail(dp, bid, j0, vfin, uv);
+}
+
+void sym_runs_launch(const CsrPart &P, bool dot, const double *x, double *y, hipStream_t s, const int *done, const DotPlan &dp)
+{
+    const SymRun &sr = P.pk_sym;
+    const dim3 g((unsigned)(sr.NX * sr.S));
+    const bool small = 2 * sr.p + 1 <= 24;
+    if (dot) {
+        if (small) hipLaunchKernelGGL((k_spmv_ldsp_sym<6, true>), g, dim3(VB), 0, s, sr, x, y, done, dp);
+        else hipLaunchKernelGGL((k_spmv_ldsp_sym<9, true>), g, dim3(VB), 0, s, sr, x, y, done, dp);
+    } else {
+        if (small) hipLaunchKernelGGL((k_spmv_ldsp_sym<6, false>), g, dim3(VB), 0, s, sr, x, y, done, dp);
+        else hipLaunchKernelGGL((k_spmv_ldsp_sym<9, false>), g, dim3(VB), 0, s, sr, x, y, done, dp);
+    }
+}
+
+void sym_runs_build(const CsrPart &P, hipStream_t s)
+{
+    sym_runs_free(P);
+    const int NX = sym_nx_of(P);
+    const RunStretches &rs = P.pk_rs;
+    int order[RS_MAX];
+    for (int i = 0; i < RS_MAX; i++) order[i] = i;
+    std::stable_sort(order, order + rs.n, [&](int a, int c) { return rs.s[a].b1 - rs.s[a].b0 > rs.s[c].b1 - rs.s[c].b0; });
+    P.sym_why = "no run stretch";
+    int *flag = nullptr;
+    for (int oi = 0; oi < rs.n; oi++) {
+        const RunStretch &r = rs.s[order[oi]];
+        const int L = r.L, p = L / 2;
+        if ((L & 1) == 0 || r.kd != p || L > SYM_MAXL) { if (oi == 0) P.sym_why = "refused: no odd row length with the diagonal in the middle"; continue; }
+        std::vector<int> tab(4 * (size_t)r.Q), off(L);
+        if (hipMemcpyAsync(tab.data(), r.off, sizeof(int) * tab.size(), hipMemcpyDeviceToHost, s) != hipSuccess ||
+            hipStreamSynchronize(s) != hipSuccess) { (void)hipGetLastError(); if (oi == 0) P.sym_why = "refused: the offsets could not be read"; break; }
+        for (int k = 0; k < L; k++) off[k] = tab[(size_t)(k % 4) * r.Q + k / 4];
+        if (!sym_offsets_ok(off.data(), L)) { if (oi == 0) P.sym_why = "refused: the offsets are not antisymmetric and ascending"; continue; }
+        SymRun sr;
+        sr.p = p; sr.NX = NX; sr.Q = sym_apron(off[L - 1]); sr.TQ = r.Q; sr.off = r.off;
+        if (!sym_range(r.b0, r.b1, sr.Q, NX, &sr.inner0, &sr.S)) { if (oi == 0) P.sym_why = "refused: the inner range is shorter than the slices"; continue; }
+        int bad = 1;
+        if ((flag || hipMalloc(&flag, sizeof(int)) == hipSuccess) && hipMemsetAsync(flag, 0, sizeof(int), s) == hipSuccess) {
+            hipLaunchKernelGGL(k_sym_check, dim3((unsigned)(NX * sr.S)), dim3(VB), 0, s, sr, r.b0, r.s0, P.val, flag);
+            if (hipMemcpyAsync(&bad, flag, sizeof(int), hipMemcpyDeviceToHost, s) != hipSuccess || hipStreamSynchronize(s) != hipSuccess) bad = 1;
+        }
+        (void)hipGetLastError();
+        if (bad) { if (oi == 0) P.sym_why = "refused: the values do not mirror each other bit for bit"; continue; }
+        const long tiles = (long)sr.Q + (long)NX * sr.S;
+        if (hipMalloc(&P.pk_sym_H, sizeof(double) * (size_t)tiles * (size_t)(p + 1) * PK_R) != hipSuccess) {
+            (void)hipGetLastError(); P.pk_sym_H = nullptr; if (oi == 0) P.sym_why = "refused: no memory for the half store"; break;
+        }
+        hipLaunchKernelGGL(k_sym_pack, dim3((unsigned)tiles), dim3(VB), 0, s, sr, r.b0, r.s0, P.val, P.pk_sym_H);
+        if (hipGetLastError() != hipSuccess) { (void)hipFree(P.pk_sym_H); P.pk_sym_H = nullptr; if (oi == 0) P.sym_why = "refused: the half store could not be written"; break; }
+        sr.H = P.pk_sym_H;
+        P.pk_sym = sr; P.pk_sym_tiles = tiles;
+        P.sym_why = "taken";
+        break;
+    }
+    if (flag) (void)hipFree(flag);
+}
+
+}
diff --git a/liblcg_amd/csrc/csr_sym.hpp b/liblcg_amd/csrc/csr_sym.hpp
--- /dev/null
+++ b/liblcg_amd/csrc/csr_sym.hpp
@@ -0,0 +1,59 @@
+#pragma once
+
+#if defined(__HIPCC__)
+#define LCG_SYM_HD __host__ __device__
+#else
+#define LCG_SYM_HD
+#endif
+
+namespace lcgh {
+
+struct SymRun {
+    int inner0 = 0;
+    int S = 0;
+    int NX = 0;
+    int Q = 0;
+    int p = 0;
+    int TQ = 0;
+    const int *off = nullptr;
+    const double *H = nullptr;
+};
+
+LCG_SYM_HD inline bool sym_offsets_ok(const int *off, int L)
+{
+    if (L < 1 || (L & 1) == 0) return false;
+    const int p = L / 2;
+    if (off[p] != 0) return false;
+    for (int k = 1; k < L; k++)
+        if (off[k] <= off[k - 1]) return false;
+    for (int k = 0; k < p; k++)
+        if (off[2 * p - k] != -off[k]) return false;
+    return true;
+}
+
+LCG_SYM_HD inline int sym_apron(int maxoff) { return (maxoff + 63) / 64 + 1; }
+
+LCG_SYM_HD inline bool sym_range(int b0, int b1, int Q, int NX, int *inner0, int *S)
+{
+    const long first = ((long)b0 + Q + 7) / 8 * 8;
+    if (NX < 1 || first + NX > (long)b1) return false;
+    *inner0 = (int)first;
+    *S = (int)((b1 - first) / NX);
+    return true;
+}
+
+LCG_SYM_HD inline int sym_block_of(int w, int inner0, int S, int NX)
+{
+    const int lg = NX == 8 ? 3 : NX == 4 ? 2 : NX == 2 ? 1 : 0;
+    return inner0 + (w & (NX - 1)) * S + (w >> lg);
+}
+
+LCG_SYM_HD inline int sym_tile_of(int b, int inner0, int S, int NX, int Q)
+{
+    const int d = b - inner0;
+    if (d < 0 || NX == 1) return Q + d;
+    const int e = d / S;
+    return Q + NX * (d - e * S) + e;
+}
+
+}
diff --git a/liblcg_amd/csrc/internal.hpp b/liblcg_amd/csrc/internal.hpp
--- a/liblcg_amd/csrc/internal.hpp
+++ b/liblcg_amd/csrc/internal.hpp
@@ -9,6 +9,7 @@
 #include <vector>
 
 #include "lcg_hip.h"
+#include "csr_sym.hpp"
 
 namespace lcgh {
 
@@ -236,6 +237,13 @@
     mutable RunStretches pk_rs;
     mutable int *pk_rs_off = nullptr;
     mutable long pk_rs_blocks = 0, pk_rs_groups = 0;
+    mutable int sym_mode = -1;
+    mutable int sym_nx = 0;
+    bool sym_whole = false;
+    mutable SymRun pk_sym;
+    mutable double *pk_sym_H = nullptr;
+    mutable long pk_sym_tiles = 0;
+    mutable const char *sym_why = "not tried";
     mutable double *dot_part = nullptr;
     mutable long dot_cap = 0;
     int64_t n_cols = 0;
@@ -312,6 +320,8 @@
                 double *y, bool accumulate, hipStream_t s, const int *done_flag);
 int spmv_launch_push(const CsrPart &P, bool is_complex, int variant, double mean_row, const double *x, double *y,
                      hipStream_t s, const int *done_flag, const PushPlan &pp);
+void sym_runs_reset(CsrPart &P);
+void sym_runs_free(const CsrPart &P);
 int jacobi_launch(const lcg_hip_csr *A, const double *x, double *z, int n, hipStream_t s);
 int csr_ax_dot(lcg_hip_csr *A, const double *x, double *y, const double *u, int yy, double *part, int *slots, hipStream_t s,
                const int *done_flag);
```

After: 1645 (median of 6 runs). 1.05x the previous value.
